# muonium-ai/Qwen3-TTS-C

Hardware: AMD Instinct MI355X
Metric: audio-sec/wall-sec (RTF^-1) + first-packet ms, Qwen3-TTS-1.7B @ 1 & 8 GPU (higher is better)
Workload: dtype fp32 activations x bf16 weights (fp32 accumulate); 1 GPU; Qwen3-TTS-1.7b synthetic, P128 prompt, fixed 128 frames (10.24 s audio), default sampling, batch 1 per GPU; global_batch=1, frames=128, parallelism=dp1 (independent replicas, no collective in the data path)

## Files before the change

### include/qtts_hip.h

```cpp
#ifndef QTTS_HIP_H
#define QTTS_HIP_H

#include <stddef.h>
#include <stdint.h>

#ifdef __cplusplus
extern "C" {
#endif

typedef struct qtts_dev qtts_dev_t;

typedef struct {
    int H, I, L, NH, KV, HD, TH, TV, V, G;
    int Hs, Is, Ls, NHs, KVs, HDs, Vs;
    float eps, theta;
    int cq, ccb, ccbdim, chid, clat, clayers, cheads, ckv, cinter, cwin, cdec;
    int rates[4], ratios[2];
    float ceps;
    int pad_id, bos_id, eos_id;
} qtts_dims_t;

typedef struct {
    int mel_dim, enc_dim, n_ch;
    int ch[8], ks[8], dil[8];
// ... 65 lines not shown
int qtts_dev_codec_stream_begin_ex(qtts_dev_t *dev, int max_frames, int chunk_frames);
int qtts_dev_codec_stream_prime(qtts_dev_t *dev, const int *codes, int T);
int qtts_dev_codec_stream_push_slot(qtts_dev_t *dev, int b, int frame0, int T, float *host_out);
int qtts_dev_codec_stream_push_host(qtts_dev_t *dev, const int *codes, int T, float *host_out);

int qtts_dev_codec_mstream_begin(qtts_dev_t *dev, int n_streams, int max_frames, int chunk_frames);
int qtts_dev_codec_mstream_push_slots(qtts_dev_t *dev, int n, const int *streams, const int *slots, int frame0, int T,
                                      float *const *host_out);
int qtts_dev_codec_mstream_push_host(qtts_dev_t *dev, int n, const int *streams, const int *codes, int T,
                                     float *const *host_out);
int qtts_dev_codec_mstream_pos(qtts_dev_t *dev, int stream);
int qtts_dev_codec_mstream_push_slots_at(qtts_dev_t *dev, int n, const int *streams, const int *slots,
                                         const int *frame0, int T, float *const *host_out);
int qtts_dev_codec_mstream_push_host_any(qtts_dev_t *dev, int n, const int *streams, const int *codes, int T,
                                         float *const *host_out);
int qtts_dev_codec_mstream_reset(qtts_dev_t *dev, int stream);
int qtts_dev_codec_mstream_push_host_ragged(qtts_dev_t *dev, int n, const int *streams, const int *codes,
                                            const int *counts, int ld_frames, float *const *host_out);
int qtts_dev_codec_mstream_push_slots_ragged(qtts_dev_t *dev, int n, const int *streams, const int *slots,
                                             const int *frame0, const int *count, float *const *host_out);
int qtts_dev_codec_mstream_prime(qtts_dev_t *dev, int n, const int *streams, const int *codes, const int *counts,
                                 int ld_frames);

int qtts_dev_codec_async_begin(qtts_dev_t *dev, int max_frames);
int qtts_dev_codec_async_push(qtts_dev_t *dev, int b, int frame0, int T);
int qtts_dev_codec_async_end(qtts_dev_t *dev, float *host_out, int frames);

int qtts_dev_enc_config(qtts_dev_t *dev, const qtts_enc_dims_t *dims);
int qtts_dev_enc_available(qtts_dev_t *dev);
int qtts_dev_speaker_embed(qtts_dev_t *dev, int nb, const float *const *wav, const int *n, float *out,
                           float *mel_out);
int qtts_dev_encode_audio(qtts_dev_t *dev, int nb, const float *const *wav, const int *n, int *codes,
                          int max_frames, int *frames, float *latent);

int qtts_dev_talker_prefill_host(qtts_dev_t *dev, const float *embeds, int n, float *hidden_out);
int qtts_dev_talker_forward_host(qtts_dev_t *dev, const float *embed, float *logits, float *hidden_out);
int qtts_dev_subtalker_host(qtts_dev_t *dev, const float *hidden, int first_code, int *out_codes);
float *qtts_dev_codec_decode_host(qtts_dev_t *dev, const int *codes, int T, int *out_samples);

int qtts_hip_matvec_bf16(float *out_dev, const uint16_t *A_dev, const float *x_dev, int rows, int cols,
                         int batch, void *stream);
int qtts_hip_rmsnorm_matvec_bf16(float *out_dev, const uint16_t *A_dev, const float *x_dev, const float *w_dev,
                                 float eps, int rows, int cols, int batch, void *stream);
int qtts_hip_decode_matvec_bf16(float *out_dev, const uint16_t *A_dev, const float *x_dev, const float *w_dev,
                                float eps, int rows, int cols, int batch, void *stream);
int qtts_hip_resident_matvec_bf16(float *out_dev, const uint16_t *A_dev, const float *x_dev, const float *w_dev,
                                  float eps, int rows, int cols, int epi, void *stream);
int qtts_hip_sample_top_k(int *out_dev, const float *logits_dev, int vocab, int top_k, float top_p,
                          float temperature, uint32_t *rng_bits_dev, int batch, void *stream);
int qtts_hip_sample_top_k_rows(int *out_dev, const float *logits_dev, int vocab, const int *top_k,
                               const float *top_p, const float *temperature, uint32_t *rng_bits_dev, int batch,
                               void *stream);
int qtts_hip_causal_conv1d(float *out_dev, const float *in_dev, const float *w_dev, const float *b_dev, int ci,
                           int co, int k, int L, int dilation, int groups, void *stream);
int qtts_hip_transposed_conv1d(float *out_dev, const float *in_dev, const float *w_dev, const float *b_dev,
                               int ci, int co, int k, int stride, int L, void *stream);
int qtts_hip_snake_beta(float *out_dev, const float *x_dev, const float *alpha_dev, const float *inv_beta_dev,
                        int channels, int length, void *stream);
int qtts_hip_attn_decode(float *out_dev, const float *qkv_dev, void *kc_dev, void *vc_dev,
                         const float *qn_w_dev, const float *kn_w_dev,
                         const float *rope_cos_dev, const float *rope_sin_dev,
                         const int *pos_dev, int NH, int KV, int HD, int S, int rows,
                         float eps, int kv_dtype, void *stream);
int qtts_hip_attn_decode_ex(float *out_dev, const float *qkv_dev, void *kc_dev, void *vc_dev,
                            const float *qn_w_dev, const float *kn_w_dev,
                            const float *rope_cos_dev, const float *rope_sin_dev,
                            const int *pos_dev, int NH, int KV, int HD, int S, int rows,
                            float eps, int kv_dtype, const int *skip_dev, void *stream);
int qtts_hip_attn_cached(float *out_dev, float *q_dev, int ld_q, void *kc_dev, void *vc_dev,
                         const float *qn_w_dev, const float *kn_w_dev,
                         const float *rope_cos_dev, const float *rope_sin_dev,
                         const int *row_b_dev, const int *pos_dev, int NH, int KV, int HD, int S, int slots,
                         int rows, float eps, int win, int kv_dtype, int prep, void *stream);
int qtts_hip_attn_o(float *part_dev, const float *qkv_dev, float *kc_dev, float *vc_dev,
                    const float *qn_w_dev, const float *kn_w_dev,
                    const float *rope_cos_dev, const float *rope_sin_dev, const int *pos_dev,
                    const uint16_t *Wo_dev, int R, int NH, int KV, int HD, int S, int rows, float eps,
                    void *stream);
int qtts_hip_attn_o_pair(float *part_dev, const float *qkv_dev, float *kc_dev, float *vc_dev,
                         const float *qn_w_dev, const float *kn_w_dev,
                         const float *rope_cos_dev, const float *rope_sin_dev, const int *skip_dev,
                         const uint16_t *Wo_dev, int R, int NH, int KV, int HD, int S, float eps,
                         void *stream);
int qtts_hip_resident_matvec_rows_bf16(float *out_dev, const uint16_t *A_dev, const float *x_dev, const float *w_dev,
                                       float eps, int rows, int cols, int epi, const float *part_dev, int n_part,
                                       float *x_new_dev, int nrows, void *stream);
typedef struct {
    int rows, cols, batch;
    const uint16_t *A;
    int src;
    const float *x; int ldx;
    const void *table;
    const int *ids; int ids_bstride, ids_rstride, ids_off;
    const int *row_sel;
    const float *part_in; int n_part_in;
    const float *norm_w; float eps;
    float *xcopy; int xcopy_normed;
    int epi;
    const float *bias;
    float *y; int ldy;
    int kz, self_reduce;
    float *part_out;
} qtts_bgemv_desc_t;
int qtts_hip_batch_matvec_case(const qtts_bgemv_desc_t *d, void *stream);
typedef struct {
    int kernel;
    int n_tmpl, tmpl[5];
    int src;
    int grid_x, grid_y, block;
    size_t lds_bytes;
    int tpw, cch;
} qtts_bgemv_plan_t;
int qtts_hip_batch_matvec_plan(const qtts_bgemv_desc_t *d, qtts_bgemv_plan_t *out);
typedef struct {
    int M, N, K;
    int amode, bmode, emode;
    const float *A; int lda;
    const float *B; int ldb;
    int Kw, dil, pad, L, stride, tmin, co;
    const float *sa, *sb;
    float *C; int ldc;
    const float *bias, *vec, *aux, *res;
    int ldaux, ldres;
    const float *ea, *eb;
} qtts_xgemm_desc_t;
enum {
    QTTS_XP_CONVB2 = 0,
    QTTS_XP_CONVB4 = 1,
    QTTS_XP_CONV = 2,
    QTTS_XP_XLIN = 3,
    QTTS_XP_XGEMV = 4,
    QTTS_XP_XGEMM = 5,
};
int qtts_hip_xgemm_plan(const qtts_xgemm_desc_t *d, size_t part_elems, int force_path, int *path_out,
                        int *splits_out);
int qtts_hip_xgemm_case(const qtts_xgemm_desc_t *d, size_t part_elems, int force_path, int *path_out,
                        int *splits_out, void *stream);
int qtts_hip_xgemm_seg_case(const qtts_xgemm_desc_t *d, int nseg, int seg_ldb, int seg_ldc, size_t part_elems,
                            int force_path, int *path_out, int *splits_out, void *stream);
int qtts_hip_xgemm_func(float *out_dev, const float *x_dev, const float *alpha_dev, const float *inv_beta_dev,
                        int channels, int length, int fn, void *stream);
int qtts_hip_expf_glibc(float *out_dev, const float *in_dev, int n, void *stream);
int qtts_hip_sync(void);
long long qtts_hip_tengine_layers(void);
long long qtts_hip_st_pair_passes(void);
long long qtts_hip_gemv_wide_launches(void);
long long qtts_hip_sample_slot_launches(void);

int qtts_dev_profile_frame(qtts_dev_t *dev, int step, int max, int *kind, double *bytes, float *ms, char *names);
int qtts_hip_hbm_bw(size_t bytes, int iters, double *read_gbs, double *copy_gbs);

#ifdef __cplusplus
}
#endif
#endif
```

### qwen3-tts-c_amd/csrc/hip/k_misc.hip

```cpp
#include "qtts_common.h"
#include "qtts_kernels.h"

namespace {

__global__ __launch_bounds__(256) void k_embed_sum(EmbedSumArgs a) {
#pragma clang fp contract(off)
    const int b = blockIdx.y;
    const int d = blockIdx.x * 256 + threadIdx.x;
    const int stop = a.stopped ? a.stopped[b] : 0;
    const int row = a.cur_row[b];
    const int ntr = a.n_trailing[b];
    if (stop) return;
    const int *cd = a.codes + (size_t)b * a.codes_bstride + (size_t)row * a.G;
    constexpr int GM = 16;
    int c[GM];
#pragma unroll
    for (int g = 0; g < GM; ++g) c[g] = cd[g < a.G ? g : a.G - 1];
    if (d < a.H) {
        const float *tt = row < ntr ? a.trailing + ((size_t)b * a.tr_cap + row) * a.H : a.pad;
        float e[GM];
        e[0] = bf2f(a.codec_emb[(size_t)c[0] * a.H + d]);
#pragma unroll
        for (int g = 1; g < GM; ++g) {
            const int gg = g < a.G ? g : a.G - 1;
            e[g] = bf2f(a.st_emb[((size_t)(gg - 1) * a.Vs + c[g]) * a.H + d]);
        }
        const float t = tt[d];
        float s = 0.0f;
        s += e[0];
#pragma unroll
        for (int g = 1; g < GM; ++g)
            if (g < a.G) s += e[g];
        s += t;
        a.out[(size_t)b * a.H + d] = s;
    }
    if (a.advance && blockIdx.x == 0 && threadIdx.x == 0) a.kv_len[b] += 1;
}

__global__ __launch_bounds__(256) void k_prompt(PromptArgs a) {
#pragma clang fp contract(off)
    const int e = blockIdx.y;
    const int *pl = a.plan + 5 * e;
    const int src = pl[0], cid = pl[1], kind = pl[2], b = pl[3], slot = pl[4];
    float *dst = kind == 0 ? a.prefill + ((size_t)b * a.p_cap + slot) * a.H
                           : a.trailing + ((size_t)b * a.tr_cap + slot) * a.H;
    const int f = -3 - cid;
    const int *fr = cid <= -3 && f < a.n_ref ? a.ref_codes + (size_t)f * a.G : nullptr;
    for (int d = blockIdx.x * 256 + threadIdx.x; d < a.H; d += gridDim.x * 256) {
        float v = a.proj[(size_t)src * a.H + d];
        if (cid >= 0) v += bf2f(a.codec_emb[(size_t)cid * a.H + d]);
        else if (cid == -2 && a.spk) v += a.spk[d];
        else if (fr) {
            float s = 0.0f;
            if (fr[0] >= 0 && fr[0] < a.V) s += bf2f(a.codec_emb[(size_t)fr[0] * a.H + d]);
            for (int g = 1; g < a.G; ++g)
                if (fr[g] >= 0 && fr[g] < a.Vs) s += bf2f(a.st_emb[((size_t)(g - 1) * a.Vs + fr[g]) * a.H + d]);
            v += s;
        }
        dst[d] = v;
    }
}

__global__ void k_copy_rows(float *dst, int ldd, const float *src, int lds, const int *rows, int ncols) {
    const int r = blockIdx.y;
    const int sr = rows ? rows[r] : r;
    for (int c = blockIdx.x * 256 + threadIdx.x; c < ncols; c += gridDim.x * 256)
        dst[(size_t)r * ldd + c] = src[(size_t)sr * lds + c];
}

__global__ __launch_bounds__(256) void k_slot_reset(SlotResetArgs a) {
    const int i = blockIdx.x * 256 + threadIdx.x;
    if (i < a.H) a.x[(size_t)a.b * a.H + i] = a.row[i];
    if (i < a.V) a.counts[(size_t)a.b * a.V + i] = 0;
    if (i == 0) {
        a.kv_len[a.b] = a.pos;
        a.n_gen[a.b] = 0;
        a.cur_row[a.b] = 0;
        a.stop_step[a.b] = 0;
        a.last_tok[a.b] = 0;
        a.rng[a.b] = a.seed_bits;
        a.st_rng[a.b] = a.seed_bits;
        a.stopped[a.b] = 0;
    }
}

}

int qtts_slot_reset(const SlotResetArgs &a, hipStream_t st) {
    const int n = a.H > a.V ? a.H : a.V;
    hipLaunchKernelGGL(k_slot_reset, dim3((n + 255) / 256), dim3(256), 0, st, a);
    return hipGetLastError() == hipSuccess ? 0 : -1;
}

int qtts_embed_sum(const EmbedSumArgs &a, hipStream_t st) {
// ... 23 lines not shown
```

### qwen3-tts-c_amd/csrc/hip/k_tengine.hip

```cpp
#include "qtts_common.h"
#include "qtts_kernels.h"

namespace {

constexpr int H = 2048, NH = 16, KVH = 8, HD = 128, IM = 6144, QKVR = (NH + 2 * KVH) * HD;
constexpr int GPH = NH / KVH;
constexpr int LPK = 8, CH = 256 / LPK, DPL = HD / LPK, D4 = HD / 4, KG = 256 / D4, NO = GPH * HD;
constexpr int NVC = CH / KG;
constexpr unsigned SPIN_MAX = 1u << 22;

struct TLds {
    float xs[H];
    float hs[IM];
    float hq[4 * HD];
    float qk[(GPH + 1) * HD];
    float vv[HD];
    float sc[GPH][CH];
    float ml[GPH][2];
    float red[KG * NO];
    float cred[4];
    float outq[16], outo[8], outh[24];
    int gflag;
    int ocnt;
    int cbar;
    int last;
    int full;
    int done[4];
};

__device__ __forceinline__ float dot8w(const v4u &w, const float *x) {
    const float4 x0 = *reinterpret_cast<const float4 *>(x);
    const float4 x1 = *reinterpret_cast<const float4 *>(x + 4);
    float s = 0.f;
    s = fmaf(__uint_as_float(w.x << 16), x0.x, s); s = fmaf(__uint_as_float(w.x & 0xFFFF0000u), x0.y, s);
    s = fmaf(__uint_as_float(w.y << 16), x0.z, s); s = fmaf(__uint_as_float(w.y & 0xFFFF0000u), x0.w, s);
    s = fmaf(__uint_as_float(w.z << 16), x1.x, s); s = fmaf(__uint_as_float(w.z & 0xFFFF0000u), x1.y, s);
    s = fmaf(__uint_as_float(w.w << 16), x1.z, s); s = fmaf(__uint_as_float(w.w & 0xFFFF0000u), x1.w, s);
    return s;
}

__device__ __forceinline__ int lds_ld(int *p) { return __hip_atomic_load(p, __ATOMIC_RELAXED, __HIP_MEMORY_SCOPE_WORKGROUP); }
__device__ __forceinline__ void give_up(int *err, int code) {
    __hip_atomic_store(err, code, __ATOMIC_RELAXED, __HIP_MEMORY_SCOPE_AGENT);
}

__device__ __forceinline__ bool gemv_wait(TLds &L, int k) {
    unsigned n = 0;
    bool ok = true;
    while (lds_ld(&L.gflag) < k) {
        __builtin_amdgcn_s_sleep(1);
        if (++n > SPIN_MAX) { ok = false; break; }
    }
    __builtin_amdgcn_fence(__ATOMIC_ACQUIRE, "workgroup");
    return ok;
}
__device__ __forceinline__ void gemv_done(TLds &L, int lane) {
    __builtin_amdgcn_fence(__ATOMIC_RELEASE, "workgroup");
    if (lane == 0) __hip_atomic_fetch_add(&L.ocnt, 1, __ATOMIC_RELAXED, __HIP_MEMORY_SCOPE_WORKGROUP);
}
__device__ __forceinline__ void cbarrier(TLds &L, int &gen, int lane, int *err) {
    gen += 4;
    __builtin_amdgcn_fence(__ATOMIC_RELEASE, "workgroup");
    if (lane == 0) __hip_atomic_fetch_add(&L.cbar, 1, __ATOMIC_RELAXED, __HIP_MEMORY_SCOPE_WORKGROUP);
    unsigned n = 0;
    while (lds_ld(&L.cbar) < gen) {
        __builtin_amdgcn_s_sleep(1);
        if (++n > SPIN_MAX) { give_up(err, 2); break; }
    }
    __builtin_amdgcn_fence(__ATOMIC_ACQUIRE, "workgroup");
}
__device__ __forceinline__ void comm_wait_out(TLds &L, int k, int *err) {
    unsigned n = 0;
    while (lds_ld(&L.ocnt) < 4 * k) {
        __builtin_amdgcn_s_sleep(1);
        if (++n > SPIN_MAX) { give_up(err, 20 + k); break; }
    }
    __builtin_amdgcn_fence(__ATOMIC_ACQUIRE, "workgroup");
}
__device__ __forceinline__ void comm_stage(TLds &L, int k, int &gen, int lane, int *err) {
    cbarrier(L, gen, lane, err);
    if (threadIdx.x == 256) __hip_atomic_store(&L.gflag, k, __ATOMIC_RELAXED, __HIP_MEMORY_SCOPE_WORKGROUP);
}

typedef unsigned long long u64;
__device__ __forceinline__ void te_stamp(const TLayerArgs &a, int k, bool who) {
#ifdef QTTS_STAMPS
    if (a.dbg && who) a.dbg[blockIdx.x * 16 + k] = __builtin_amdgcn_s_memrealtime();
#endif
}
__device__ __forceinline__ void put_granule(u64 *g, unsigned tag, float v) {
    __hip_atomic_store(g, ((u64)tag << 32) | __float_as_uint(v), __ATOMIC_RELAXED, __HIP_MEMORY_SCOPE_AGENT);
}
template <int N, typename Idx>
__device__ __forceinline__ void sweep(const u64 *g, unsigned tag, Idx idx, float (&v)[N], int *err, int code) {
    unsigned n = 0;
    for (;;) {
        bool ok = true;
#pragma unroll
        for (int j = 0; j < N; ++j) {
            const u64 x = __hip_atomic_load(const_cast<u64 *>(g) + idx(j), __ATOMIC_RELAXED, __HIP_MEMORY_SCOPE_AGENT);
            v[j] = __uint_as_float((unsigned)x);
            ok &= (unsigned)(x >> 32) == tag;
        }
        if (__all(ok)) return;
        __builtin_amdgcn_s_sleep(1);
        if (++n > SPIN_MAX) { give_up(err, code); return; }
    }
}

__device__ __forceinline__ void comm_norm_stage(TLds &L, float4 (&xv)[2], const float *nw, float eps, int ct, int lane,
                                                int cw, int &gen, int *err) {
    float ss = 0.f;
#pragma unroll
    for (int q = 0; q < 2; ++q) {
        const float4 v = xv[q];
        ss += v.x * v.x + v.y * v.y + v.z * v.z + v.w * v.w;
    }
    ss = wave_sum(ss);
    if (lane == 0) L.cred[cw] = ss;
    cbarrier(L, gen, lane, err);
    const float inv = rms_inv(L.cred[0] + L.cred[1] + L.cred[2] + L.cred[3], H, eps);
#pragma unroll
    for (int q = 0; q < 2; ++q) {
        const int c = 4 * (ct + 256 * q);
        const float4 n4 = *reinterpret_cast<const float4 *>(nw + c);
        float4 v = xv[q];
        v.x = v.x * inv * n4.x; v.y = v.y * inv * n4.y; v.z = v.z * inv * n4.z; v.w = v.w * inv * n4.w;
        *reinterpret_cast<float4 *>(L.xs + c) = v;
    }
}

__device__ __forceinline__ int qkv_row(int h, int i) {
    return i < NO ? GPH * HD * h + i : i < NO + HD ? NH * HD + HD * h + (i - NO) : (NH + KVH) * HD + HD * h + (i - NO - HD);
}

struct AttnPre {
    float4 kreg[DPL / 4];
    float4 vreg[NVC];
    float hw[2], rc[2], rs[2];
};
__device__ __forceinline__ void attn_preload(AttnPre &q, const TLayerArgs &a, int kvh, int split, int p, int ct,
                                             int lane, int cw) {
    const int t0 = split * CH, t1 = min(p + 1, t0 + CH);
    const int KVD = KVH * HD;
    const float *Kc = a.kc + kvh * HD;
    const float *Vc = a.vc + kvh * HD;
    const int hh0 = cw < GPH ? cw : GPH;
    const float *nw = hh0 < GPH ? a.qn_w : a.kn_w;
    const float *cs = a.rope_cos + (size_t)p * HD, *sn = a.rope_sin + (size_t)p * HD;
#pragma unroll
    for (int j = 0; j < 2; ++j) {
        q.hw[j] = nw[lane + 64 * j];
        q.rc[j] = cs[lane + 64 * j];
        q.rs[j] = sn[lane + 64 * j];
    }
    const int kl = ct / LPK, ksub = ct - kl * LPK;
    const int tk = t0 + kl;
    const float4 *kp = reinterpret_cast<const float4 *>(Kc + (size_t)(tk < t1 ? tk : t0) * KVD + ksub * DPL);
#pragma unroll
    for (int j = 0; j < DPL / 4; ++j) q.kreg[j] = kp[j];
    const int d4 = ct % D4, kg = ct / D4;
#pragma unroll
    for (int j = 0; j < NVC; ++j) {
        const int t = t0 + kg + j * KG;
        const bool ok = kg + j * KG < CH && t < t1;
        q.vreg[j] = reinterpret_cast<const float4 *>(Vc + (size_t)(ok ? t : t0) * KVD)[d4];
    }
}

__device__ void comm_attention(TLds &L, const TLayerArgs &a, int kvh, int split, int nact, int p, unsigned tag,
                               int ct, int lane, int cw, int &gen, const AttnPre &pre) {
    const int n = p + 1;
    const int t0 = split * CH, t1 = min(n, t0 + CH);
    const bool owner = (split == nact - 1);
    const int KVD = KVH * HD;
    const int hh0 = cw < GPH ? cw : GPH;
    float hv[2];
    {
        const float *src = L.hq + (hh0 < GPH ? hh0 * HD : NO);
#pragma unroll
        for (int j = 0; j < 2; ++j) hv[j] = src[lane + 64 * j];
    }
    const float *hw = pre.hw, *rc = pre.rc, *rs = pre.rs;
    const float4 *kreg = pre.kreg, *vreg = pre.vreg;
    const float vtok = L.hq[NO + HD + ct % HD];
    const int kl = ct / LPK, ksub = ct - kl * LPK;
    const int tk = t0 + kl;
    const int d4 = ct % D4, kg = ct / D4;
    if (cw <= GPH) {
        float ss = 0.f;
#pragma unroll
        for (int j = 0; j < 2; ++j) ss += hv[j] * hv[j];
// ... 564 lines not shown
```

### qwen3-tts-c_amd/csrc/hip/qtts_kernels.h

```cpp
#pragma once
#include <hip/hip_runtime.h>
#include <stdint.h>

typedef uint16_t bf16_t;

constexpr int QTTS_GM_TICKS = 1024;

enum { EPI_STORE = 0, EPI_BIAS = 1, EPI_BIAS_SILU = 2, EPI_RESID = 3, EPI_SWIGLU = 4 };

constexpr int QTTS_PF_LOADS = 4;
struct L2Prefetch {
    const unsigned char *base = nullptr;
    int pm = 1 << 30;
    long long pa = 0, pb = 0;
    int chunks = 0, lg = 30, ld = 0;
    int cs = 6;
    int nwg = 0;
    unsigned *sink = nullptr;
};

struct GemvArgs {
    const bf16_t *W = nullptr;
    int R = 0, C = 0;
    int ksplit = 0;
// ... 58 lines not shown
int qtts_bgemv(const GemvArgs &a, hipStream_t st, unsigned allowed = BG_ALL);
int qtts_gemvm_launch(const GemvArgs &a, const BgPlan &p, hipStream_t st);
int qtts_gemvb_launch(const GemvArgs &a, const BgPlan &p, hipStream_t st);
int qtts_gemvx_launch(const GemvArgs &a, const BgPlan &p, hipStream_t st);
bool qtts_gemvx_shape_ok(int R, int C);
int qtts_mgemm(const GemvArgs &a, float *inv_scratch, hipStream_t st, float *part = nullptr, size_t part_elems = 0);
size_t qtts_mgemm_part_elems(size_t rows, size_t widest);
int qtts_row_rms(const float *x, int ldx, int rows, int C, float eps, float *inv, hipStream_t st);
int qtts_mgemm_reduce(const GemvArgs &a, const float *part, int kz, hipStream_t st);
int qtts_pgemm(const GemvArgs &a, float *inv_scratch, unsigned short *planes, size_t plane_elems, hipStream_t st,
               float *part, size_t part_elems);
size_t qtts_pgemm_plane_elems(size_t rows, size_t K);

struct TLayerArgs {
    const float *x_in = nullptr;
    float *x_out = nullptr;
    const bf16_t *wqkv = nullptr, *wo = nullptr, *wgu = nullptr, *wdown = nullptr;
    const float *in_norm = nullptr, *post_norm = nullptr, *qn_w = nullptr, *kn_w = nullptr;
    const float *rope_cos = nullptr, *rope_sin = nullptr;
    float *kc = nullptr, *vc = nullptr;
    const int *pos = nullptr;
    const int *skip = nullptr;
    float eps = 1e-6f;
    float *part = nullptr;
    int *cnt = nullptr;
    int nsplit = 0;
    unsigned long long *g_qkv = nullptr, *g_att = nullptr, *g_x = nullptr, *g_h = nullptr;
    int *epoch = nullptr;
    int *err = nullptr;
    int layer = 0, last_layer = 0;
    unsigned long long *dbg = nullptr;
};
constexpr int QTTS_TE_GRANULES = 4096 + 2048 + 2048 + 6144;
bool qtts_tlayer_dims_ok(int H, int NH, int KV, int HD, int I);
size_t qtts_tlayer_lds();
int qtts_tlayer(const TLayerArgs &a, hipStream_t st, int mode);

struct AttnArgs {
    int mode = 0;
    const float *qkv = nullptr;
    int ld_qkv = 0;
    const float *qn_w = nullptr, *kn_w = nullptr;
    float eps = 1e-6f;
    const float *rope_cos = nullptr, *rope_sin = nullptr;
    float *kc = nullptr, *vc = nullptr;
    int S = 0;
    const int *pos = nullptr;
    int pos_const = 0;
    const int *row_b = nullptr;
    int NH = 0, KV = 0, HD = 0;
    float *out = nullptr;
    int ld_out = 0;
    int nrows = 0;
    const int *skip = nullptr;
    int win = 0;
    const float *qkv_tab = nullptr;
    const int *tab_ids = nullptr, *tab_row_sel = nullptr;
    int tab_bstride = 0, tab_rstride = 0, tab_off = 0;
    float *part = nullptr;
    int *cnt = nullptr;
    int nsplit = 0;
    int defer = 0;
    L2Prefetch pf;
#ifdef QTTS_STAMPS
    unsigned long long *dbg = nullptr;
#endif
    const float *xc_tab = nullptr;
    const bf16_t *xc_tab16 = nullptr;
    float *xc_dst = nullptr;
    int xc_n = 0;
    int lpk = 0;
    int kv_dtype = 0;
};
int qtts_attn_keys_per_split(int HD, bool defer, int lpk);
bool qtts_attn_defer_ok(const AttnArgs &a);
int qtts_attn_o(const AttnArgs &a, const bf16_t *Wo, int R, float *part, hipStream_t st);
bool qtts_attn_o_covers(const AttnArgs &a, const bf16_t *Wo);

bool qtts_gemvw_pair_covers(int R, int C, int epi);
int qtts_gemvw_pair(const GemvArgs &a, hipStream_t st);
bool qtts_attn_o_pair_covers(const AttnArgs &a, const bf16_t *Wo);
int qtts_attn_o_pair(const AttnArgs &a, const bf16_t *Wo, int R, float *part, hipStream_t st);

extern thread_local const char *qtts_last_kernel;
inline bool qtts_attn_head_ok(int HD) { return HD == 8 || HD == 16 || HD == 32 || HD == 64 || HD == 128; }
int qtts_attention(const AttnArgs &a, hipStream_t st);
int qtts_qk_prep(const AttnArgs &a, hipStream_t st);

struct SampArgs {
    const float *logits = nullptr;
    int ld = 0, n = 0, nb = 1;
    int top_k = 50;
    float top_p = 1.0f, temp = 0.9f;
    uint32_t *rng = nullptr;
    int mode = 0;
    int suppress_lo = 0, eos = -1;
    float rep = 1.0f;
    int *counts = nullptr;
    int fixed = 0;
    int *n_gen = nullptr, *stopped = nullptr, *cur_row = nullptr, *stop_step = nullptr;
    int *host_stopped = nullptr;
    uint32_t *st_rng = nullptr;
    uint32_t seed_bits = 0;
    int *codes = nullptr;
    int codes_bstride = 0, G = 16, g = 0;
    int *out_tok = nullptr;
};
int qtts_sample(const SampArgs &a, hipStream_t st);

constexpr int QTTS_MAX_TAPS = 8;
struct SampForce {
    const int *forced = nullptr;
    int *drawn = nullptr;
    const int *taps = nullptr;
    float *tap_logits = nullptr;
    int *tap_meta = nullptr;
    int tap_ld = 0;
};
int qtts_sample_forced(const SampArgs &a, const SampForce &f, hipStream_t st);

struct alignas(16) SampSlotRow {
    float temp, top_p, rep;
    int top_k;
    float st_temp, st_top_p;
    int st_top_k;
    uint32_t seed_bits;
};
static_assert(sizeof(SampSlotRow) == 32, "two dwordx4 loads cover a row");
bool qtts_sample_row_fast(const SampSlotRow &r, int mode, int n);
int qtts_sample_slots(const SampArgs &a, const SampSlotRow *tab, bool all_fast, hipStream_t st);
long long qtts_sample_slot_launches();
int qtts_slot_row_set(SampSlotRow *tab, int b, const SampSlotRow &r, uint32_t *rng, uint32_t *st_rng, hipStream_t st);

struct EmbedSumArgs {
    const int *codes = nullptr;
    int codes_bstride = 0, G = 16;
    const int *cur_row = nullptr, *stopped = nullptr;
    const bf16_t *codec_emb = nullptr;
    const bf16_t *st_emb = nullptr;
    int Vs = 0, H = 0, nb = 1;
    const float *trailing = nullptr;
    int tr_cap = 0;
    const int *n_trailing = nullptr;
    const float *pad = nullptr;
    float *out = nullptr;
    int *kv_len = nullptr;
    int advance = 0;
};
int qtts_embed_sum(const EmbedSumArgs &a, hipStream_t st);

struct PromptArgs {
    const float *proj = nullptr;
    const int *plan = nullptr;
    int nplan = 0, H = 0;
    const bf16_t *codec_emb = nullptr;
    const bf16_t *st_emb = nullptr;
    const float *spk = nullptr;
    const int *ref_codes = nullptr;
    int n_ref = 0, G = 0, V = 0, Vs = 0;
    float *prefill = nullptr;
    int p_cap = 0;
    float *trailing = nullptr;
    int tr_cap = 0;
};
int qtts_prompt_assemble(const PromptArgs &a, hipStream_t st);

int qtts_copy_rows(float *dst, int ldd, const float *src, int lds, const int *src_rows, int nrows, int ncols,
                   hipStream_t st);

struct SlotResetArgs {
    int b = 0, pos = 0, H = 0, V = 0;
    const float *row = nullptr;
    float *x = nullptr;
    int *kv_len = nullptr, *n_gen = nullptr, *cur_row = nullptr, *stopped = nullptr, *stop_step = nullptr;
    int *last_tok = nullptr, *counts = nullptr;
    uint32_t *rng = nullptr, *st_rng = nullptr;
    uint32_t seed_bits = 0;
};
int qtts_slot_reset(const SlotResetArgs &a, hipStream_t st);
```

### qwen3-tts-c_amd/csrc/hip/qtts_runtime.hip

```cpp
#include <math.h>
#include <stdlib.h>
#include <string.h>

#include <algorithm>
#include <map>
#include <set>
#include <string>
#include <atomic>
#include <vector>

#include "qtts_common.h"
#include "qtts_kernels.h"
#include "qtts_codec.h"
#include "qtts_enc.h"
#include "../../../include/qtts_hip.h"

#define CK(x)                                                                                              \
    do {                                                                                                   \
        hipError_t e_ = (x);                                                                               \
        if (e_ != hipSuccess) {                                                                            \
            fprintf(stderr, "HIP error %s at %s:%d: %s\n", hipGetErrorName(e_), __FILE__, __LINE__, #x);   \
            return -1;                                                                                     \
        }                                                                                                  \
    } while (0)
// ... 40 lines not shown
    size_t war_off = 0, war_cap = 0, sar_off = 0, sar_cap = 0;
    std::vector<Layer> tl, sl;
    bf16_t *codec_emb = nullptr, *text_emb = nullptr, *fc1w = nullptr, *fc2w = nullptr, *head = nullptr;
    float *fc1b = nullptr, *fc2b = nullptr, *tk_norm = nullptr;
    bf16_t *st_emb = nullptr, *lm = nullptr, *st_proj = nullptr;
    float *st_projb = nullptr, *st_norm = nullptr;
    float *codec_ptab = nullptr, *st_ptab = nullptr;
    float *qkv0_tab = nullptr;
    CodecModel codec;
    EncModel enc;
    float *rope_cos = nullptr, *rope_sin = nullptr, *rope_cos_s = nullptr, *rope_sin_s = nullptr;
    int rope_max = 0;
    std::set<std::string> got;
    int nb = 0, nrun = 0, max_frames = 0, S = 0, p_cap = 0, tr_cap = 0, rows_cap = 0;
    float *x_tk = nullptr, *qkv = nullptr, *att = nullptr, *hbuf = nullptr, *logits = nullptr, *tk_hid = nullptr;
    float *x_st2 = nullptr, *opart = nullptr;
    float *x_tk2 = nullptr, *bpo = nullptr, *bpd = nullptr;
    float *ppart = nullptr;
    float *tk_xfin = nullptr;
    const float *tk_pend = nullptr;
    int tk_npend = 0;
    bool bsplit = true;
    int bself_min = 9;
    int bkz_max = 0;
    int bkz_wide = 1;
    float *x_st = nullptr, *qkv_s = nullptr, *att_s = nullptr, *h_s = nullptr, *logits_s = nullptr;
    float *kc = nullptr, *vc = nullptr, *kcs = nullptr, *vcs = nullptr;
    int kv_dtype = 0, kv_want = 0;
    bool te_kv_said = false;
    bool att_own = false;
    int *codes = nullptr, *counts = nullptr, *n_gen = nullptr, *stopped = nullptr, *cur_row = nullptr;
    int *last_tok = nullptr;
    int *stop_step = nullptr, *kv_len = nullptr, *n_trailing = nullptr;
    float *att_part = nullptr;
    int *att_cnt = nullptr, att_nsplit = 0;
    int *btick = nullptr;
    uint32_t *rng = nullptr, *st_rng = nullptr;
    float *trailing = nullptr, *prefill = nullptr, *pad_emb = nullptr;
    float *px = nullptr, *pqkv = nullptr, *patt = nullptr, *ph = nullptr, *pt1 = nullptr, *pproj = nullptr;
    int *prow_b = nullptr, *ppos = nullptr, *psrc = nullptr, *pids = nullptr, *pplan = nullptr, *plast = nullptr;
    int ids_cap = 0;
    int *pref = nullptr;
    float *pspk = nullptr;
    int pref_cap = 0, n_pref = 0, has_spk = 0;
    std::vector<int> p_len_h, n_tr_h;
    qtts_gen_params_t par{};
    bool have_par = false;
    hipGraphExec_t g0 = nullptr, gN = nullptr;
    hipGraphExec_t gNr[QTTS_MAX_SLOTS + 1] = {};
    int graph_key = -1;
    int *f_forced = nullptr, *f_drawn = nullptr, *f_taps = nullptr, *f_tap_meta = nullptr;
    float *f_tap_logits = nullptr;
    int f_tap_ld = 0, f_ntaps = 0, f_phase = 0;
    int f_run_frames = 0;
    bool f_armed = false;
    size_t f_bytes = 0;
    SampSlotRow *sp_tab = nullptr;
    std::vector<SampSlotRow> sp_host;
    bool sp_armed = false, sp_general = false;
    int *hstop = nullptr;
    int hstop_cap = 0;
    hipEvent_t fev[2] = {nullptr, nullptr};
    hipStream_t cst = nullptr;
    hipEvent_t cev = nullptr;
    float *cwav = nullptr;
    size_t cwav_cap = 0;
    int *push_codes = nullptr;
    size_t push_cap = 0;
    bool prime_pending = false;
    float *pwav = nullptr;
    size_t pwav_cap = 0;
    std::vector<CodecModel *> clanes;
    std::vector<hipStream_t> clane_st;
    float *mwav = nullptr;
    size_t mwav_cap = 0;
    int *mcodes = nullptr;
    size_t mcodes_cap = 0;
    struct Prof { int kind; double bytes; hipEvent_t a, b; const char *name; };
    std::vector<Prof> prof;
    bool profiling = false;
    bool attn_o = true;
    bool tab0b = true;
    bool st_pair = true;
    int l2pf = 31;
    int l2pf_tk = 0;
    unsigned *pf_sink = nullptr;
    bool attn_defer = true;
    int attn_lpk = 0;
    int gm_dbg_layer = -1;
    unsigned long long *gm_dbg = nullptr;
    int tengine = 0;
    unsigned long long *te_g = nullptr;
    int *te_ctl = nullptr;
    float *pinv = nullptr;
    int pinv_cap = 0;
    float *mpart = nullptr;
    size_t mpart_elems = 0;
    unsigned short *pplanes = nullptr;
    size_t pplanes_elems = 0;
    bool pgemm = true;

    int QKV() const { return (d.NH + 2 * d.KV) * d.HD; }
    int QKVs() const { return (d.NHs + 2 * d.KVs) * d.HDs; }
    size_t kv_esz() const { return kv_dtype == 1 ? 2 : 4; }
    float *kv_layer(float *c, int l) const {
        return reinterpret_cast<float *>(reinterpret_cast<char *>(c) + (size_t)l * nb * S * d.KV * d.HD * kv_esz());
    }
};

static constexpr size_t QTTS_ARENA_SMALL = (size_t)1 << 20, QTTS_ARENA_BLOCK = (size_t)32 << 20;
static void *dalloc(qtts_dev *dv, size_t n, bool weight) {
    void *p = nullptr;
    if (n == 0) n = 16;
    const char *ae = getenv("QTTS_HIP_ARENA");
    const int arena = ae ? atoi(ae) : 0;
    if (arena && n <= QTTS_ARENA_SMALL) {
        unsigned char *&base = weight ? dv->war : dv->sar;
        size_t &off = weight ? dv->war_off : dv->sar_off, &cap = weight ? dv->war_cap : dv->sar_cap;
        const size_t need = (n + 255) & ~(size_t)255;
        if (!base || off + need > cap) {
            void *blk = dalloc(dv, QTTS_ARENA_BLOCK, weight);
            if (!blk) return nullptr;
            base = (unsigned char *)blk; off = 0; cap = QTTS_ARENA_BLOCK;
        }
        p = base + off;
        off += need;
        return p;
    }
    const hipError_t prior = hipPeekAtLastError();
    const hipError_t e = hipMalloc(&p, n);
    if (e != hipSuccess) {
        fprintf(stderr, "qtts: hipMalloc(%zu) failed: %s (last error before it: %s)\n", n, hipGetErrorName(e),
                hipGetErrorName(prior));
        return nullptr;
    }
    if (weight) { dv->wallocs.push_back(p); dv->wbytes += n; }
    else { dv->sallocs.push_back(p); dv->sbytes += n; }
    return p;
}

static void drop_row_graphs(qtts_dev *dv) {
    for (auto &g : dv->gNr)
        if (g) { hipGraphExecDestroy(g); g = nullptr; }
}

static void free_force(qtts_dev *dv) {
    if (!dv->f_armed) return;
    hipStreamSynchronize(dv->st);
    for (void *p : {(void *)dv->f_forced, (void *)dv->f_drawn, (void *)dv->f_taps, (void *)dv->f_tap_meta,
                    (void *)dv->f_tap_logits})
        if (p) hipFree(p);
    dv->f_forced = dv->f_drawn = dv->f_taps = dv->f_tap_meta = nullptr;
    dv->f_tap_logits = nullptr;
    dv->f_tap_ld = dv->f_ntaps = 0;
    dv->sbytes -= dv->f_bytes;
    dv->f_bytes = 0;
    dv->f_armed = false;
    dv->graph_key = -1;
}

static void free_slot_params(qtts_dev *dv) {
    if (!dv->sp_armed) return;
    hipStreamSynchronize(dv->st);
    if (dv->sp_tab) {
        hipFree(dv->sp_tab);
        dv->sbytes -= dv->sp_host.size() * sizeof(SampSlotRow);
// ... 137 lines not shown
    } else if (name == "talker.text_projection.linear_fc2.bias") {
        dv->fc2b = upload_f32(dv, host, dtype, n); rc = dv->fc2b ? 0 : -1;
    } else if (name == "talker.model.norm.weight") {
        dv->tk_norm = upload_f32(dv, host, dtype, n); rc = dv->tk_norm ? 0 : -1;
    } else if (name == "talker.codec_head.weight") {
        dv->head = upload_bf16(dv, host, dtype, n); rc = dv->head ? 0 : -1;
    } else if (name == "talker.code_predictor.small_to_mtp_projection.weight") {
        dv->st_proj = upload_bf16(dv, host, dtype, n); rc = dv->st_proj ? 0 : -1;
    } else if (name == "talker.code_predictor.small_to_mtp_projection.bias") {
        dv->st_projb = upload_f32(dv, host, dtype, n); rc = dv->st_projb ? 0 : -1;
    } else if (name == "talker.code_predictor.model.norm.weight") {
        dv->st_norm = upload_f32(dv, host, dtype, n); rc = dv->st_norm ? 0 : -1;
    } else if ((idx = parse_idx(name, "talker.code_predictor.model.codec_embedding.", &rest)) >= 0 && rest == "weight") {
        if (idx >= d.G - 1 || n != (size_t)d.Vs * d.H) { fprintf(stderr, "qtts: bad %s\n", cname); return -1; }
        if (!dv->st_emb) dv->st_emb = (bf16_t *)dalloc(dv, (size_t)(d.G - 1) * d.Vs * d.H * 2, true);
        rc = dv->st_emb ? upload_bf16_at(dv->st_emb + (size_t)idx * d.Vs * d.H, host, dtype, n) : -1;
    } else if ((idx = parse_idx(name, "talker.code_predictor.lm_head.", &rest)) >= 0 && rest == "weight") {
        if (idx >= d.G - 1 || n != (size_t)d.Vs * d.Hs) { fprintf(stderr, "qtts: bad %s\n", cname); return -1; }
        if (!dv->lm) dv->lm = (bf16_t *)dalloc(dv, (size_t)(d.G - 1) * d.Vs * d.Hs * 2, true);
        rc = dv->lm ? upload_bf16_at(dv->lm + (size_t)idx * d.Vs * d.Hs, host, dtype, n) : -1;
    } else if ((idx = parse_idx(name, "talker.code_predictor.model.layers.", &rest)) >= 0) {
        if (idx >= d.Ls) return 0;
        rc = put_layer(dv, dv->sl[idx], rest, host, dtype, n, d.Hs, d.NHs, d.KVs, d.HDs, d.Is);
    } else if ((idx = parse_idx(name, "talker.model.layers.", &rest)) >= 0) {
        if (idx >= d.L) return 0;
        rc = put_layer(dv, dv->tl[idx], rest, host, dtype, n, d.H, d.NH, d.KV, d.HD, d.I);
    } else {
        return 0;
    }
    if (rc) {
        fprintf(stderr, "qtts: failed to upload tensor %s\n", cname);
        return -1;
    }
    dv->got.insert(name);
    return 0;
}

extern "C" qtts_dev_t *qtts_dev_create(const qtts_dims_t *dims, int device) {
    if (hipSetDevice(device) != hipSuccess) {
        fprintf(stderr, "qtts: cannot select HIP device %d\n", device);
        return nullptr;
    }
    qtts_dev *dv = new qtts_dev();
    dv->d = *dims;
    dv->device = device;
    if (hipStreamCreateWithFlags(&dv->st, hipStreamNonBlocking) != hipSuccess) {
        delete dv;
        return nullptr;
    }
    dv->tl.resize(dims->L);
    dv->sl.resize(dims->Ls);
    const char *bs = getenv("QTTS_HIP_BSPLIT");
    dv->bsplit = !(bs && !atoi(bs));
    const char *bk = getenv("QTTS_HIP_BKZ_MAX");
    if (bk) dv->bkz_max = atoi(bk) < 1 ? 1 : atoi(bk) > 4 ? 4 : atoi(bk);
    const char *bw = getenv("QTTS_HIP_BKZ_WIDE");
    dv->bkz_wide = bw ? atoi(bw) : 1;
    const char *bm = getenv("QTTS_HIP_BSELF_MIN");
    if (bm) dv->bself_min = atoi(bm);
    const char *ad = getenv("QTTS_HIP_ATTN_DEFER");
    dv->attn_defer = !(ad && !atoi(ad));
    const char *lk = getenv("QTTS_HIP_ATTN_LPK");
    dv->attn_lpk = lk ? atoi(lk) : 0;
    const char *ao = getenv("QTTS_HIP_ATTN_O");
    dv->attn_o = !(ao && !atoi(ao));
    const char *pg = getenv("QTTS_HIP_PGEMM");
    dv->pgemm = !(pg && !atoi(pg));
    const char *te = getenv("QTTS_HIP_TENGINE");
    if (te && atoi(te)) {
        int dev = 0, ncu = 0;
        if (hipGetDevice(&dev) == hipSuccess &&
            hipDeviceGetAttribute(&ncu, hipDeviceAttributeMultiprocessorCount, dev) == hipSuccess && ncu >= 256)
            dv->tengine = std::min(3, std::max(1, atoi(te)));
    }
    const char *kvd = getenv("QTTS_HIP_KV");
    if (kvd && *kvd) {
        if (!strcmp(kvd, "bf16")) dv->kv_want = 1;
        else if (strcmp(kvd, "fp32")) fprintf(stderr, "qtts: QTTS_HIP_KV=%s ignored (bf16 or fp32)\n", kvd);
    }
    const char *tb = getenv("QTTS_HIP_TAB0B");
    dv->tab0b = !(tb && !atoi(tb));
    const char *sp = getenv("QTTS_HIP_ST_PAIR");
    dv->st_pair = !(sp && !atoi(sp));
    const char *pf = getenv("QTTS_HIP_L2PF");
    if (pf) dv->l2pf = atoi(pf);
    const char *pft = getenv("QTTS_HIP_L2PF_TK");
    if (pft) dv->l2pf_tk = atoi(pft);
    const char *gd = getenv("QTTS_HIP_GM_DBG");
    if (gd) dv->gm_dbg_layer = atoi(gd);
    codec_init(&dv->codec, dims, dv->st);
    dv->enc.st = dv->st;
    dv->enc.device = device;
    return dv;
}

extern "C" void qtts_dev_destroy(qtts_dev_t *dv) {
    if (!dv) return;
    hipSetDevice(dv->device);
    hipStreamSynchronize(dv->st);
    free_state(dv);
    codec_destroy(&dv->codec);
    enc_destroy(&dv->enc);
    if (dv->cst) hipStreamSynchronize(dv->cst);
    if (dv->hstop) hipHostFree(dv->hstop);
    for (hipEvent_t e : dv->fev)
        if (e) hipEventDestroy(e);
    for (CodecModel *ln : dv->clanes) codec_lane_delete(ln);
    for (hipStream_t st : dv->clane_st) hipStreamDestroy(st);
    if (dv->mwav) hipFree(dv->mwav);
    if (dv->mcodes) hipFree(dv->mcodes);
    if (dv->cwav) hipFree(dv->cwav);
    if (dv->pwav) hipFree(dv->pwav);
    if (dv->push_codes) hipFree(dv->push_codes);
    if (dv->cev) hipEventDestroy(dv->cev);
    if (dv->cst) hipStreamDestroy(dv->cst);
    for (void *p : dv->wallocs) hipFree(p);
    hipStreamDestroy(dv->st);
    delete dv;
}

extern "C" size_t qtts_dev_bytes(const qtts_dev_t *dv, int which) {
    if (!dv) return 0;
    return which == 0 ? dv->wbytes + codec_weight_bytes(&dv->codec) + enc_weight_bytes(&dv->enc) : dv->sbytes;
}

extern "C" int qtts_dev_set_kv_dtype(qtts_dev_t *dv, int dtype) {
    if (!dv || (dtype != 0 && dtype != 1)) return -1;
    dv->kv_want = dtype;
    return 0;
}

extern "C" int qtts_dev_kv_dtype(const qtts_dev_t *dv) { return dv ? dv->kv_want : -1; }

extern "C" int qtts_dev_get_kv(qtts_dev_t *dv, int layer, int b, int pos0, int n, float *k_host, float *v_host) {
    if (!dv || !dv->kc || !dv->vc || dv->nb < 1 || layer < 0 || layer >= dv->d.L || b < 0 || b >= dv->nb ||
        pos0 < 0 || n < 1 || pos0 > dv->S - n)
        return -1;
    hipSetDevice(dv->device);
    const size_t KVD = (size_t)dv->d.KV * dv->d.HD, cnt = (size_t)n * KVD, esz = dv->kv_esz();
    const size_t off = ((size_t)b * dv->S + pos0) * KVD * esz;
    CK(hipStreamSynchronize(dv->st));
    float *caches[2] = {dv->kc, dv->vc}, *outs[2] = {k_host, v_host};
    std::vector<uint16_t> tmp(dv->kv_dtype == 1 ? cnt : 0);
    for (int i = 0; i < 2; ++i) {
        if (!outs[i]) continue;
        const char *src = reinterpret_cast<const char *>(dv->kv_layer(caches[i], layer)) + off;
        if (dv->kv_dtype == 1) {
            CK(hipMemcpy(tmp.data(), src, cnt * 2, hipMemcpyDeviceToHost));
            for (size_t j = 0; j < cnt; ++j) outs[i][j] = host_bf16(tmp[j]);
        } else {
            CK(hipMemcpy(outs[i], src, cnt * 4, hipMemcpyDeviceToHost));
        }
    }
    return 0;
}

extern "C" int qtts_dev_get_attn(qtts_dev_t *dv, float *qkv_host, float *att_host) {
    if (!dv || dv->nb < 1 || !dv->qkv || !dv->att) return -1;
    if (att_host && !dv->att_own) {
        fprintf(stderr, "qtts_dev_get_attn: the last talker pass left no merged attention output "
                        "(batch 1 defers the merge to the O projection; QTTS_HIP_ATTN_DEFER=0 keeps it)\n");
        return -1;
    }
    hipSetDevice(dv->device);
    CK(hipStreamSynchronize(dv->st));
    if (qkv_host) CK(hipMemcpy(qkv_host, dv->qkv, (size_t)dv->nb * dv->QKV() * 4, hipMemcpyDeviceToHost));
// ... 120 lines not shown
        if (!dv->ptr) return -1;                                          \
    } while (0)
    A(x_tk, float, B * d.H);
    A(qkv, float, B * dv->QKV());
    A(att, float, B * d.NH * d.HD);
    A(hbuf, float, B * d.I);
    A(logits, float, B * d.V);
    A(tk_hid, float, B * d.H);
    const size_t B2 = B < 2 ? 2 : B;
    A(x_st, float, B2 * d.Hs);
    A(x_st2, float, B2 * d.Hs);
    A(x_tk2, float, B * d.H);
    A(bpo, float, (size_t)4 * B * (d.H > d.Hs ? d.H : d.Hs));
    A(bpd, float, (size_t)4 * B * (d.H > d.Hs ? d.H : d.Hs));
    A(ppart, float, (size_t)4 * 16 * (d.H > d.Hs ? d.H : d.Hs));
    A(opart, float, (size_t)B2 * ((size_t)d.KVs * d.Hs > (size_t)d.KV * d.H ? (size_t)d.KVs * d.Hs : (size_t)d.KV * d.H));
    A(qkv_s, float, B2 * dv->QKVs());
    A(att_s, float, B * d.NHs * d.HDs);
    A(h_s, float, B2 * d.Is);
    A(logits_s, float, B * d.Vs);
    {
        const size_t kv_floats = (size_t)d.L * B * dv->S * d.KV * d.HD * dv->kv_esz() / 4;
        A(kc, float, kv_floats);
        A(vc, float, kv_floats);
    }
    A(kcs, float, (size_t)d.Ls * B * d.G * d.KVs * d.HDs);
    A(vcs, float, (size_t)d.Ls * B * d.G * d.KVs * d.HDs);
    A(codes, int, B * (max_frames + 1) * d.G);
    A(counts, int, B * d.V);
    A(n_gen, int, B);
    A(stopped, int, B);
    A(cur_row, int, B);
    A(last_tok, int, B);
    CK(hipMemsetAsync(dv->last_tok, 0, B * sizeof(int), dv->st));
    A(stop_step, int, B);
    A(kv_len, int, B);
    A(n_trailing, int, B);
    A(rng, uint32_t, B);
    A(st_rng, uint32_t, B);
    A(trailing, float, B * 64 * d.H);
    dv->tr_cap = 64;
    A(prefill, float, B * max_prefill * d.H);
    A(pad_emb, float, d.H);
    const size_t R = dv->rows_cap;
    A(px, float, R * d.H);
    A(pqkv, float, R * dv->QKV());
    A(patt, float, R * d.NH * d.HD);
    A(ph, float, R * d.I);
    A(prow_b, int, R);
    A(ppos, int, R);
    A(psrc, int, R);
    A(plast, int, B);
    dv->pinv_cap = dv->rows_cap > 64 ? dv->rows_cap : 64;
    A(pinv, float, dv->pinv_cap);
    {
        const size_t wide = std::max<size_t>({(size_t)dv->QKV(), (size_t)2 * d.I, (size_t)d.H, (size_t)d.TH});
        const char *e = getenv("QTTS_HIP_MGEMM_KZ");
        dv->mpart_elems = e && !strcmp(e, "0") ? 0 : qtts_mgemm_part_elems(std::max<size_t>(R, 64), wide);
        if (dv->mpart_elems)
            dv->mpart_elems = std::max(dv->mpart_elems, std::min<size_t>((size_t)512 * 128 * 128, (size_t)8 * R * wide));
        if (dv->mpart_elems) A(mpart, float, dv->mpart_elems);
        const size_t kmax = std::max<size_t>({(size_t)d.H, (size_t)d.I, (size_t)d.NH * d.HD});
        dv->pplanes_elems = dv->pgemm ? qtts_pgemm_plane_elems(R, kmax) : 0;
        if (dv->pplanes_elems) A(pplanes, unsigned short, dv->pplanes_elems);
    }
    {
        const int gph = d.NH / d.KV;
        const int ch = std::min(qtts_attn_keys_per_split(d.HD, false, dv->attn_lpk),
                                qtts_attn_keys_per_split(d.HD, true, dv->attn_lpk));
        dv->att_nsplit = (dv->S + ch - 1) / ch;
        A(att_part, float, B * d.KV * dv->att_nsplit * (gph * d.HD + 2 * gph));
        const int kvmax = d.KV > d.KVs ? d.KV : d.KVs;
        A(att_cnt, int, B * kvmax);
        CK(hipMemsetAsync(dv->att_cnt, 0, B * kvmax * sizeof(int), dv->st));
        A(pf_sink, unsigned, 1);
        A(btick, int, QTTS_GM_TICKS);
        if (dv->tengine) {
            A(te_g, unsigned long long, QTTS_TE_GRANULES);
            CK(hipMemsetAsync(dv->te_g, 0, QTTS_TE_GRANULES * 8, dv->st));
            A(te_ctl, int, 2);
            CK(hipMemsetAsync(dv->te_ctl, 0, 2 * sizeof(int), dv->st));
        }
        CK(hipMemsetAsync(dv->btick, 0, QTTS_GM_TICKS * sizeof(int), dv->st));
        if (dv->gm_dbg_layer >= 0) {
            A(gm_dbg, unsigned long long, 4 * 2048 * 8);
            CK(hipMemsetAsync(dv->gm_dbg, 0, 4 * 2048 * 8 * 8, dv->st));
        }
    }
#undef A
    dv->p_len_h.assign(nb, 0);
    dv->n_tr_h.assign(nb, 0);
    CK(hipMemsetAsync(dv->codes, 0, B * (max_frames + 1) * d.G * sizeof(int), dv->st));
    CK(hipMemsetAsync(dv->kcs, 0, (size_t)d.Ls * B * d.G * d.KVs * d.HDs * 4, dv->st));
    CK(hipMemsetAsync(dv->vcs, 0, (size_t)d.Ls * B * d.G * d.KVs * d.HDs * 4, dv->st));
    if (dv->rope_max < dv->S) {
        dv->rope_max = dv->S;
        CKI(build_rope(dv, dv->S, d.HD, d.theta, &dv->rope_cos, &dv->rope_sin));
        if (d.HDs != d.HD) CKI(build_rope(dv, d.G + 2, d.HDs, d.theta, &dv->rope_cos_s, &dv->rope_sin_s));
        else { dv->rope_cos_s = dv->rope_cos; dv->rope_sin_s = dv->rope_sin; }
    }
    dv->graph_key = -1;
    return 0;
}

static uint32_t seed_bits(int seed) {
    float f = (float)seed;
    uint32_t u;
    memcpy(&u, &f, 4);
    return u;
}

static int reset_counters(qtts_dev *dv) {
    const size_t B = dv->nb;
    hipStream_t st = dv->st;
    if (dv->hstop_cap < (int)B) {
        if (dv->hstop) CK(hipHostFree(dv->hstop));
        dv->hstop = nullptr;
        CK(hipHostMalloc((void **)&dv->hstop, B * sizeof(int), hipHostMallocDefault));
        dv->hstop_cap = (int)B;
        dv->graph_key = -1;
    }
    if (!dv->fev[0]) {
        CK(hipEventCreateWithFlags(&dv->fev[0], hipEventDisableTiming));
        CK(hipEventCreateWithFlags(&dv->fev[1], hipEventDisableTiming));
    }
    CK(hipStreamSynchronize(st));
    memset(dv->hstop, 0, B * sizeof(int));
    CK(hipMemsetAsync(dv->counts, 0, B * dv->d.V * sizeof(int), st));
    CK(hipMemsetAsync(dv->n_gen, 0, B * sizeof(int), st));
    CK(hipMemsetAsync(dv->stopped, 0, B * sizeof(int), st));
    CK(hipMemsetAsync(dv->cur_row, 0, B * sizeof(int), st));
    CK(hipMemsetAsync(dv->stop_step, 0, B * sizeof(int), st));
    std::vector<uint32_t> r(B, seed_bits(dv->par.seed));
    CK(hipMemcpyAsync(dv->rng, r.data(), B * 4, hipMemcpyHostToDevice, st));
    CK(hipMemcpyAsync(dv->st_rng, r.data(), B * 4, hipMemcpyHostToDevice, st));
    CK(hipStreamSynchronize(st));
    return 0;
}

enum { PK_GEMV_TALKER = 0, PK_GEMV_SUB = 1, PK_ATTN = 2, PK_SAMPLE = 3, PK_EMBED = 4 };
struct ProfScope {
    qtts_dev *dv;
    size_t idx;
    ProfScope(qtts_dev *d, int kind, double bytes) : dv(d), idx((size_t)-1) {
        if (!dv->profiling) return;
        qtts_dev::Prof p{kind, bytes, nullptr, nullptr, ""};
        hipEventCreateWithFlags(&p.a, hipEventDisableSystemFence);
        hipEventCreateWithFlags(&p.b, hipEventDisableSystemFence);
        hipEventRecord(p.a, dv->st);
        dv->prof.push_back(p);
        idx = dv->prof.size() - 1;
    }
    void cancel() {
        if (idx == (size_t)-1) return;
        hipEventDestroy(dv->prof[idx].a);
        hipEventDestroy(dv->prof[idx].b);
        dv->prof.pop_back();
        idx = (size_t)-1;
    }
    ~ProfScope() {
        if (idx == (size_t)-1) return;
        hipEventRecord(dv->prof[idx].b, dv->st);
        dv->prof[idx].name = qtts_last_kernel;
    }
};
static double gemv_bytes(const GemvArgs &a) {
    return (double)a.R * a.C * 2 + (double)a.nb * a.C * 4 + (double)a.nb * a.R * 4 + (a.norm_w ? a.C * 4.0 : 0.0);
}
static int pgemv(qtts_dev *dv, const GemvArgs &a, int kind) {
    ProfScope ps(dv, kind, gemv_bytes(a));
    return qtts_gemv(a, dv->st);
}
static int rows_proj(qtts_dev *dv, GemvArgs a, int rows, bool prefill = false) {
    const int xs = a.ldx, ys = a.ldy;
    if (prefill && dv->pgemm && rows > 16 && (!a.norm_w || rows <= dv->pinv_cap)) {
        GemvArgs c = a;
        c.nb = rows;
        const int rc = qtts_pgemm(c, dv->pinv, dv->pplanes, dv->pplanes_elems, dv->st, dv->mpart, dv->mpart_elems);
        if (rc <= 0) return rc;
    }
    if (rows > 64 && (!a.norm_w || rows <= dv->pinv_cap)) {
        GemvArgs c = a;
        c.nb = rows;
        const int rc = qtts_mgemm(c, dv->pinv, dv->st, dv->mpart, dv->mpart_elems);
        if (rc <= 0) return rc;
    }
    for (int r0 = 0; r0 < rows;) {
        GemvArgs c = a;
        int nr = rows - r0 < 64 ? rows - r0 : 64;
        if (c.x) c.x = a.x + (size_t)r0 * xs;
        if (c.ids) c.ids = a.ids + (size_t)r0 * a.ids_bstride;
        c.y = a.y + (size_t)r0 * ys;
        c.nb = nr;
        int rc = 1;
        static const bool pgb = [] { const char *e = getenv("QTTS_HIP_PREFILL_GEMVB"); return !(e && !atoi(e)); }();
        static const int psk = [] { const char *e = getenv("QTTS_HIP_PREFILL_SPLIT");
                                    int v = e ? atoi(e) : 2; return v == 4 ? 4 : v ? 2 : 0; }();
        if (nr >= 2 && nr <= 16 && pgb && psk && c.epi == EPI_RESID && !c.norm_w && c.R / 16 < 256 &&
            c.C % (32 * psk) == 0 && c.R <= (dv->d.H > dv->d.Hs ? dv->d.H : dv->d.Hs)) {
            GemvArgs k = c;
            k.ypart = dv->ppart; k.kz = psk; k.ld_ypart = (size_t)nr * k.R; k.tick = dv->btick;
            rc = qtts_bgemv(k, dv->st, BG_GEMVB);
        }
        if (rc == 1) rc = qtts_bgemv(c, dv->st, pgb ? BG_GEMVB | BG_GEMVM : BG_GEMVM);
        if (rc == 1 && nr >= 2) rc = qtts_mgemm(c, dv->pinv, dv->st, dv->mpart, dv->mpart_elems);
        if (rc < 0) return -1;
        if (rc == 1) {
            nr = nr < 16 ? nr : 16;
            c.nb = nr;
            CKI(qtts_gemv(c, dv->st));
        }
        r0 += nr;
    }
    return 0;
}
// ... 45 lines not shown
    std::vector<int> io(nid);
    for (int i = 0; i < nid; ++i) io[i] = i;
    int *ids = (int *)dalloc(dv, (size_t)nid * 4, true);
    dv->qkv0_tab = (float *)dalloc(dv, rows * QKV * 4, true);
    if (!ids || !dv->qkv0_tab) return -1;
    CK(hipMemcpy(ids, io.data(), (size_t)nid * 4, hipMemcpyHostToDevice));
    const bool proj = dv->st_proj != nullptr;
    for (int g = 1; g < d.G; ++g) {
        GemvArgs a = gv(dv->sl[0].wqkv, QKV, d.Hs, nullptr, d.Hs, nullptr, QKV, 1, EPI_STORE);
        a.norm_w = dv->sl[0].in; a.eps = d.eps; a.nt = 0;
        if (proj) a.table_f32 = g == 1 ? dv->codec_ptab : dv->st_ptab + (size_t)(g - 2) * d.Vs * d.Hs;
        else a.table = g == 1 ? dv->codec_emb : dv->st_emb + (size_t)(g - 2) * d.Vs * d.H;
        a.ids = ids; a.ids_bstride = 1;
        a.reps = g == 1 ? d.V : d.Vs;
        a.ldy_rep = QKV;
        a.y = dv->qkv0_tab + (g == 1 ? 0 : (size_t)d.V + (size_t)(g - 2) * d.Vs) * QKV;
        const int rc = qtts_gemvw(a, dv->st);
        if (rc < 0) return -1;
        if (rc == 0) continue;
        const int n = a.reps;
        float *base = a.y;
        a.reps = 1;
        for (int r = 0; r < n; ++r) {
            a.ids_off = r;
            a.y = base + (size_t)r * QKV;
            CKI(qtts_gemv(a, dv->st));
        }
    }
    CK(hipStreamSynchronize(dv->st));
    return 0;
}


static int bsplit_kz(const qtts_dev *dv, int R, int C) {
    if (!dv->bsplit || dv->nrun < 2) return 0;
    int kz = R / 16 >= 256 ? 1 : 256 / (R / 16);
    const int cap = dv->bkz_max > 0 ? dv->bkz_max : dv->nrun <= 8 ? 2 : 4;
    if (kz > cap) kz = cap;
    if ((dv->nrun > 8 && dv->bkz_wide) || dv->bkz_wide == 2) {
        const int wcap = dv->bkz_wide == 2 ? 4 : cap;
        while (2 * kz <= wcap && C / kz > 2048 && C % (64 * kz) == 0) kz *= 2;
    }
    while (kz > 1 && C % (32 * kz)) kz /= 2;
    return kz > 1 ? kz : 0;
}
static bool split_out(qtts_dev *dv, GemvArgs &g, float *part, int kz, int self_min = 0) {
    g.ypart = part; g.kz = kz; g.ld_ypart = (size_t)dv->nrun * g.R;
    if (dv->nrun >= (self_min > 0 ? self_min : dv->bself_min)) { g.tick = dv->btick; return false; }
    g.y = nullptr;
    return true;
}
static void add_in(GemvArgs &g, const float *part, int n, int R, int nrun, float *xnew) {
    g.xadd = part; g.n_xadd = n; g.ld_xadd = nrun * R; g.ldb_xadd = R;
    if (xnew) { g.xcopy = xnew; g.ldxc = R; g.xcopy_normed = 0; }
}

static L2Prefetch pf_gemvw(const qtts_dev *dv, const bf16_t *W, int R, int C, int grid = 256, bool on = true) {
    L2Prefetch p;
    if (!on || R % grid) return p;
    long long bytes = (long long)(R / grid) * C * 2;
    if (bytes > 64LL * 256 * QTTS_PF_LOADS) bytes = 64LL * 256 * QTTS_PF_LOADS;
    if (bytes % 64) return p;
    p.base = reinterpret_cast<const unsigned char *>(W);
    p.pa = (long long)(R / grid) * C * 2; p.pb = 0; p.chunks = (int)(bytes / 64); p.lg = 30; p.ld = 0;
    p.nwg = grid;
    p.sink = dv->pf_sink;
    return p;
}
#ifdef QTTS_STAMPS
#define DBG_XFIRST(a) do { const char *e_ = getenv("QTTS_HIP_DBG_XFIRST"); (a).dbg_xfirst = e_ ? atoi(e_) : 0; } while (0)
#else
#define DBG_XFIRST(a) do { } while (0)
#endif
static L2Prefetch pf_attn_o(const qtts_dev *dv, const bf16_t *Wo, int R, int NH, int HD) {
    L2Prefetch p;
    const int W2 = 2 * HD, LPS = W2 / 8 < 8 ? W2 / 8 : 8, RPW = 256 / LPS;
    const int cpr = W2 * 2 / 64;
    if (R % RPW || (cpr & (cpr - 1)) || cpr < 1 || RPW * cpr > 256 * QTTS_PF_LOADS) return p;
    p.base = reinterpret_cast<const unsigned char *>(Wo);
    p.pm = R / RPW; p.pa = (long long)RPW * NH * HD * 2; p.pb = W2 * 2;
    p.chunks = RPW * cpr; p.lg = __builtin_ctz(cpr); p.ld = NH * HD * 2; p.sink = dv->pf_sink;
    p.nwg = (R / RPW) * (NH / 2);
    return p;
}

static bool tengine_ok(qtts_dev *dv, int kzo, int kzd) {
    const qtts_dims_t &d = dv->d;
    return dv->tengine && dv->te_g && dv->kv_dtype == 0 && dv->nrun == 1 && !kzo && !kzd && dv->attn_defer &&
           qtts_tlayer_dims_ok(d.H, d.NH, d.KV, d.HD, d.I) && dv->S > 16 && dv->att_nsplit * 32 >= dv->S;
}
static std::atomic<long long> g_tengine_layers{0};
extern "C" long long qtts_hip_tengine_layers(void) { return g_tengine_layers.load(); }
static int talker_layers_te(qtts_dev *dv) {
    const qtts_dims_t &d = dv->d;
    const int NBA = dv->nb, KVD = d.KV * d.HD;
    for (int l = 0; l < d.L; ++l) {
        Layer &ly = dv->tl[l];
        TLayerArgs a;
        a.x_in = dv->x_tk; a.x_out = dv->x_tk;
        a.wqkv = ly.wqkv; a.wo = ly.wo; a.wgu = ly.wgu; a.wdown = ly.wdown;
        a.in_norm = ly.in; a.post_norm = ly.post; a.qn_w = ly.qn; a.kn_w = ly.kn;
        a.rope_cos = dv->rope_cos; a.rope_sin = dv->rope_sin;
        a.kc = dv->kv_layer(dv->kc, l); a.vc = dv->kv_layer(dv->vc, l);
        a.pos = dv->kv_len; a.skip = dv->stopped; a.eps = d.eps;
        a.part = dv->att_part; a.cnt = dv->att_cnt; a.nsplit = dv->att_nsplit;
        a.g_qkv = dv->te_g; a.g_att = dv->te_g + 4096; a.g_x = a.g_att + 2048; a.g_h = a.g_x + 2048;
        a.epoch = dv->te_ctl; a.err = dv->te_ctl + 1;
        a.layer = l; a.last_layer = l == d.L - 1;
        if (dv->gm_dbg && (l == dv->gm_dbg_layer || l == dv->gm_dbg_layer + 1))
            a.dbg = dv->gm_dbg + (size_t)(l - dv->gm_dbg_layer) * 256 * 16;
        ProfScope ps(dv, PK_GEMV_TALKER, 2.0 * ((double)dv->QKV() * d.H + (double)d.H * d.NH * d.HD + 3.0 * d.I * d.H));
        CKI(qtts_tlayer(a, dv->st, dv->tengine));
        g_tengine_layers.fetch_add(1);
    }
    dv->tk_xfin = dv->x_tk; dv->tk_pend = nullptr; dv->tk_npend = 0;
    dv->att_own = false;
    return 0;
}

static int talker_layers(qtts_dev *dv) {
    const qtts_dims_t &d = dv->d;
    const int nb = dv->nrun, NBA = dv->nb, QKV = dv->QKV(), AD = d.NH * d.HD, KVD = d.KV * d.HD;
    hipStream_t st = dv->st;
    const int kzo = bsplit_kz(dv, d.H, AD), kzd = bsplit_kz(dv, d.H, d.I);
    if (tengine_ok(dv, kzo, kzd)) return talker_layers_te(dv);
    float *xa = dv->x_tk, *xb = dv->x_tk2;
    const float *pend = nullptr;
    int npend = 0;
    for (int l = 0; l < d.L; ++l) {
        Layer &ly = dv->tl[l];
        GemvArgs a = gv(ly.wqkv, QKV, d.H, xa, d.H, dv->qkv, QKV, nb, EPI_STORE);
        a.norm_w = ly.in; a.eps = d.eps;
        if (pend) add_in(a, pend, npend, d.H, nb, xb);
        AttnArgs t;
        t.mode = 0; t.qkv = dv->qkv; t.ld_qkv = QKV; t.qn_w = ly.qn; t.kn_w = ly.kn; t.eps = d.eps;
        t.rope_cos = dv->rope_cos; t.rope_sin = dv->rope_sin;
        t.kc = dv->kv_layer(dv->kc, l); t.vc = dv->kv_layer(dv->vc, l); t.S = dv->S; t.kv_dtype = dv->kv_dtype;
        t.pos = dv->kv_len; t.NH = d.NH; t.KV = d.KV; t.HD = d.HD; t.out = dv->att; t.ld_out = AD; t.nrows = nb;
        t.skip = dv->stopped;
        t.part = dv->att_part; t.cnt = dv->att_cnt; t.nsplit = dv->att_nsplit; t.lpk = dv->attn_lpk;
        const bool defer = dv->attn_defer && nb == 1 && qtts_attn_defer_ok(t) && qtts_gemvw_amerge_ok(d.H, AD);
        t.defer = defer;
        dv->att_own = !defer;
        const bool dbg = dv->gm_dbg && l == dv->gm_dbg_layer;
        if (dbg) a.dbg = dv->gm_dbg;
        if (nb == 1 && (dv->l2pf_tk & 1)) a.pf = pf_gemvw(dv, ly.wo, d.H, AD);
        CKI(qkv_attn(dv, a, t, PK_GEMV_TALKER));
        if (pend) { std::swap(xa, xb); pend = nullptr; }
        GemvArgs o = gv(ly.wo, d.H, AD, dv->att, AD, xa, d.H, nb, EPI_RESID);
        if (dbg) o.dbg = dv->gm_dbg + 2048 * 8;
        if (defer) {
            o.amerge = dv->att_part; o.am_pos = dv->kv_len; o.am_nsplit = dv->att_nsplit;
            o.am_ch = qtts_attn_keys_per_split(d.HD, true, dv->attn_lpk); o.am_hd = d.HD; o.am_gph = d.NH / d.KV;
        }
        const int tk_self = 2;
        const bool opend = kzo && split_out(dv, o, dv->bpo, kzo, tk_self);
        if (nb == 1 && (dv->l2pf_tk & 2)) o.pf = pf_gemvw(dv, ly.wgu, 2 * d.I, d.H, 512);
        CKI(pgemv(dv, o, PK_GEMV_TALKER));
        a = gv(ly.wgu, 2 * d.I, d.H, xa, d.H, dv->hbuf, d.I, nb, EPI_SWIGLU);
        a.norm_w = ly.post; a.eps = d.eps;
        if (dbg) a.dbg = dv->gm_dbg + 2 * 2048 * 8;
        if (opend) add_in(a, dv->bpo, kzo, d.H, nb, xb);
        CKI(pgemv(dv, a, PK_GEMV_TALKER));
        if (opend) std::swap(xa, xb);
        GemvArgs dn = gv(ly.wdown, d.H, d.I, dv->hbuf, d.I, xa, d.H, nb, EPI_RESID);
        if (dbg) dn.dbg = dv->gm_dbg + 3 * 2048 * 8;
// ... 65 lines not shown
}
static bool st_pair_ok(const qtts_dev *dv) {
    const qtts_dims_t &d = dv->d;
    if (!dv->st_pair || dv->nrun != 1 || !dv->attn_o || !dv->qkv0_tab || d.G < 2 || d.Ls < 1) return false;
    if (dv->st_proj && !(dv->st_ptab && dv->codec_ptab)) return false;
    if (!dv->st_proj && d.H != d.Hs) return false;
    if (!qtts_gemvw_pair_covers(dv->QKVs(), d.Hs, EPI_STORE) || !qtts_gemvw_pair_covers(2 * d.Is, d.Hs, EPI_SWIGLU) ||
        !qtts_gemvw_pair_covers(d.Hs, d.Is, EPI_RESID))
        return false;
    for (int l = 0; l < d.Ls; ++l)
        if (!qtts_attn_o_pair_covers(st_pair_attn_args(dv, l), dv->sl[l].wo)) return false;
    return true;
}
static int pgemv_pair(qtts_dev *dv, const GemvArgs &a) {
    ProfScope ps(dv, PK_GEMV_SUB, gemv_bytes(a));
    if (qtts_gemvw_pair(a, dv->st) != 0) {
        fprintf(stderr, "qtts: pair GEMV launch failed (R=%d C=%d)\n", a.R, a.C);
        return -1;
    }
    return 0;
}
static int subtalker_pair_layers(qtts_dev *dv, int pfm, float **xfin) {
    const qtts_dims_t &d = dv->d;
    const int QKV = dv->QKVs(), AD = d.NHs * d.HDs;
    const bool proj = dv->st_proj != nullptr;
    float *xa = dv->x_st, *xb = dv->x_st2;
    if (proj) {
        GemvArgs a = gv(dv->st_proj, d.Hs, d.H, dv->tk_hid, d.H, dv->x_st, d.Hs, 1, dv->st_projb ? EPI_BIAS : EPI_STORE);
        a.bias = dv->st_projb;
        a.nt = 0;
        CKI(pgemv(dv, a, PK_GEMV_SUB));
    }
    {
        Layer &ly = dv->sl[0];
        GemvArgs a = gv(ly.wqkv, QKV, d.Hs, xa, d.Hs, dv->qkv_s, QKV, 1, EPI_STORE);
        a.norm_w = ly.in; a.eps = d.eps; a.nt = 0;
        if (!proj) { a.x = dv->tk_hid; a.ldx = d.H; a.xcopy = dv->x_st; a.ldxc = d.Hs; a.xcopy_normed = 0; }
        if (pfm & 1) a.pf = pf_attn_o(dv, ly.wo, d.Hs, d.NHs, d.HDs);
        CKI(pgemv(dv, a, PK_GEMV_SUB));
    }
    for (int l = 0; l < d.Ls; ++l) {
        Layer &ly = dv->sl[l];
        const bool sdbg = dv->gm_dbg && dv->gm_dbg_layer == 98 && l == 2;
        if (l > 0) {
            GemvArgs a = gv(ly.wqkv, QKV, d.Hs, xa, d.Hs, dv->qkv_s, QKV, 2, EPI_STORE);
            a.norm_w = ly.in; a.eps = d.eps; a.nt = 0;
            if (sdbg) a.dbg = dv->gm_dbg;
            if (pfm & 1) a.pf = pf_attn_o(dv, ly.wo, d.Hs, d.NHs, d.HDs);
            CKI(pgemv_pair(dv, a));
        }
        AttnArgs t = st_pair_attn_args(dv, l);
        if (pfm & 2) t.pf = pf_gemvw(dv, ly.wgu, 2 * d.Is, d.Hs);
#ifdef QTTS_STAMPS
        if (sdbg) t.dbg = dv->gm_dbg + 2048 * 8;
#endif
        {
            ProfScope ps(dv, PK_ATTN, (double)d.Hs * AD * 2);
            if (qtts_attn_o_pair(t, ly.wo, d.Hs, dv->opart, dv->st) != 0) {
                fprintf(stderr, "qtts: pair attention + O launch failed (layer %d)\n", l);
                return -1;
            }
        }
        GemvArgs a = gv(ly.wgu, 2 * d.Is, d.Hs, xa, d.Hs, dv->h_s, d.Is, 2, EPI_SWIGLU);
        a.norm_w = ly.post; a.eps = d.eps; a.nt = 0;
        if (pfm & 4) a.pf = pf_gemvw(dv, ly.wdown, d.Hs, d.Is);
        add_in(a, dv->opart, d.KVs, d.Hs, 2, xb);
        if (sdbg) a.dbg = dv->gm_dbg + 2 * 2048 * 8;
        CKI(pgemv_pair(dv, a));
        std::swap(xa, xb);
        a = gv(ly.wdown, d.Hs, d.Is, dv->h_s, d.Is, xa, d.Hs, 2, EPI_RESID);
        a.nt = 0;
        if (pfm & 8) {
            if (l + 1 < d.Ls) a.pf = pf_gemvw(dv, dv->sl[l + 1].wqkv, QKV, d.Hs);
            else a.pf = pf_gemvw(dv, dv->lm, d.Vs, d.Hs);
        }
        if (sdbg) a.dbg = dv->gm_dbg + 3 * 2048 * 8;
        CKI(pgemv_pair(dv, a));
    }
    *xfin = xa;
    g_st_pair_passes.fetch_add(1);
    return 0;
}

static int subtalker(qtts_dev *dv) {
    const qtts_dims_t &d = dv->d;
    const int nb = dv->nrun, NBA = dv->nb, QKV = dv->QKVs(), AD = d.NHs * d.HDs, KVD = d.KVs * d.HDs;
    const int cstride = (dv->max_frames + 1) * d.G;
    hipStream_t st = dv->st;
    const bool proj = dv->st_proj != nullptr;
    const bool pfon = nb == 1 && dv->attn_o && dv->l2pf;
    const int pfm = pfon ? dv->l2pf : 0;
    const bool tab0_ok = nb == 1 && dv->attn_o && dv->qkv0_tab && (!proj || dv->st_ptab);
    auto first_op_pf = [&](int gn) {
        if (gn >= d.G) return L2Prefetch();
        if (gn >= 1 && tab0_ok) return pf_attn_o(dv, dv->sl[0].wo, d.Hs, d.NHs, d.HDs);
        return pf_gemvw(dv, dv->sl[0].wqkv, QKV, d.Hs);
    };
    auto pass_head = [&](int g, const float *x, const float *pend, int npend) -> int {
        GemvArgs a = gv(dv->lm + (size_t)(g - 1) * d.Vs * d.Hs, d.Vs, d.Hs, x, d.Hs, dv->logits_s, d.Vs, nb,
                        EPI_STORE);
        a.norm_w = dv->st_norm; a.eps = d.eps; a.nt = 0;
        if (pend) add_in(a, pend, npend, d.Hs, nb, nullptr);
        if (pfm & 16) a.pf = first_op_pf(g + 1);
        SampArgs s;
        s.logits = dv->logits_s; s.ld = d.Vs; s.n = d.Vs; s.nb = nb;
        s.top_k = dv->par.st_top_k; s.top_p = dv->par.st_top_p; s.temp = dv->par.st_temperature;
        s.mode = 0; s.st_rng = dv->st_rng; s.stopped = dv->stopped; s.cur_row = dv->cur_row;
        s.codes = dv->codes; s.codes_bstride = cstride; s.G = d.G; s.g = g; s.out_tok = dv->last_tok;
        return head_sample(dv, a, s, PK_GEMV_SUB);
    };
    int g0 = 0;
    if (st_pair_ok(dv)) {
        float *xfin = nullptr;
        CKI(subtalker_pair_layers(dv, pfm, &xfin));
        CKI(pass_head(1, xfin + d.Hs, nullptr, 0));
        g0 = 2;
    }
    for (int g = g0; g < d.G; ++g) {
        GemvArgs src;
        src.nb = nb;
        const bool ptab = proj && g >= 1 && dv->st_ptab;
        if (g == 0) { src.x = dv->tk_hid; src.ldx = d.H; }
        else {
            if (ptab) src.table_f32 = g == 1 ? dv->codec_ptab : dv->st_ptab + (size_t)(g - 2) * d.Vs * d.Hs;
            else src.table = g == 1 ? dv->codec_emb : dv->st_emb + (size_t)(g - 2) * d.Vs * d.H;
            src.ids = dv->last_tok; src.ids_bstride = 1; src.row_sel = nullptr; src.ids_rstride = 0;
            src.ids_off = 0;
        }
        auto set_src = [&](GemvArgs &a) {
            a.x = src.x; a.ldx = src.ldx; a.table = src.table; a.table_f32 = src.table_f32; a.ids = src.ids;
            a.ids_bstride = src.ids_bstride; a.row_sel = src.row_sel; a.ids_rstride = src.ids_rstride;
            a.ids_off = src.ids_off;
        };
        if (proj && !ptab) {
            GemvArgs a = gv(dv->st_proj, d.Hs, d.H, nullptr, 0, dv->x_st, d.Hs, nb, dv->st_projb ? EPI_BIAS : EPI_STORE);
            set_src(a);
            a.bias = dv->st_projb;
            a.nt = 0;
            CKI(pgemv(dv, a, PK_GEMV_SUB));
        }
        float *xa = dv->x_st, *xb = dv->x_st2;
        const int kzo = bsplit_kz(dv, d.Hs, AD), kzd = bsplit_kz(dv, d.Hs, d.Is);
        const float *pend = nullptr;
        int npend = 0;
        for (int l = 0; l < d.Ls; ++l) {
            Layer &ly = dv->sl[l];
            const bool kv_only = g == 0 && l == d.Ls - 1;
            GemvArgs a = gv(ly.wqkv, QKV, d.Hs, xa, d.Hs, dv->qkv_s, QKV, nb, EPI_STORE);
            a.norm_w = ly.in; a.eps = d.eps; a.nt = 0;
            const bool sdbg = dv->gm_dbg && dv->gm_dbg_layer == 99 && g == 5 && l == 2;
            if (sdbg) { a.dbg = dv->gm_dbg; DBG_XFIRST(a); }
            if (l == 0 && (!proj || ptab)) { set_src(a); a.xcopy = dv->x_st; a.ldxc = d.Hs; a.xcopy_normed = 0; }
            else if (pend) add_in(a, pend, npend, d.Hs, nb, xb);
            AttnArgs t;
            t.mode = 0; t.qkv = dv->qkv_s; t.ld_qkv = QKV; t.qn_w = ly.qn; t.kn_w = ly.kn; t.eps = d.eps;
            t.rope_cos = dv->rope_cos_s; t.rope_sin = dv->rope_sin_s;
            t.kc = dv->kcs + (size_t)l * NBA * d.G * KVD; t.vc = dv->vcs + (size_t)l * NBA * d.G * KVD; t.S = d.G;
            t.pos = nullptr; t.pos_const = g; t.NH = d.NHs; t.KV = d.KVs; t.HD = d.HDs; t.out = dv->att_s;
            t.ld_out = AD; t.nrows = nb; t.skip = dv->stopped;
            t.cnt = dv->att_cnt;
            const bool tab0 = l == 0 && g >= 1 && nb == 1 && dv->attn_o && dv->qkv0_tab && (!proj || ptab) &&
                              qtts_attn_o_covers(t, ly.wo);
            GemvArgs o = gv(ly.wo, d.Hs, AD, dv->att_s, AD, xa, d.Hs, nb, EPI_RESID);
            o.nt = 0;
            bool fused_o = false, opend = false;
            const bool hd_ok = d.HDs == 128 || d.HDs == 64 || d.HDs == 32 || d.HDs == 16;
            const bool tab0b = l == 0 && g >= 1 && nb >= 2 && dv->tab0b && dv->qkv0_tab && (!proj || ptab) &&
                               d.NHs == 2 * d.KVs && d.G <= 16 && hd_ok;
            if (tab0 || tab0b) {
                t.qkv_tab = dv->qkv0_tab + (g == 1 ? 0 : (size_t)d.V + (size_t)(g - 2) * d.Vs) * QKV;
                t.tab_ids = src.ids; t.tab_bstride = src.ids_bstride; t.tab_row_sel = src.row_sel;
                t.tab_rstride = src.ids_rstride; t.tab_off = src.ids_off;
            }
            if (tab0b) { t.xc_tab = src.table_f32; t.xc_tab16 = src.table; t.xc_dst = xa; t.xc_n = d.Hs; }
            if (pfm & 1) a.pf = pf_attn_o(dv, ly.wo, d.Hs, d.NHs, d.HDs);
            if (pfm & 2) t.pf = kv_only ? first_op_pf(g + 1) : pf_gemvw(dv, ly.wgu, 2 * d.Is, d.Hs);
#ifdef QTTS_STAMPS
            if (sdbg) t.dbg = dv->gm_dbg + 2048 * 8;
#endif
            if (dv->attn_o && nb == 1) {
                if (!tab0) CKI(pgemv(dv, a, PK_GEMV_SUB));
                if (pend) { std::swap(xa, xb); pend = nullptr; }
                ProfScope ps(dv, PK_ATTN, (double)d.Hs * AD * 2);
                const int rc = qtts_attn_o(t, ly.wo, d.Hs, dv->opart, st);
                if (rc < 0) return -1;
                if (rc == 1) {
                    ps.cancel();
                    { ProfScope pa(dv, PK_ATTN, 0); CKI(qtts_attention(t, st)); }
                    o.y = xa;
                    if (kzo) opend = split_out(dv, o, dv->bpo, kzo);
                    if (!kv_only) CKI(pgemv(dv, o, PK_GEMV_SUB));
                } else {
                    fused_o = true;
                }
            } else {
                if (tab0b) {
                    ProfScope pa(dv, PK_ATTN, 0);
                    CKI(qtts_attention(t, st));
                } else {
                    CKI(qkv_attn(dv, a, t, PK_GEMV_SUB));
                }
                if (pend) { std::swap(xa, xb); pend = nullptr; }
                o.y = xa;
                if (kzo) opend = split_out(dv, o, dv->bpo, kzo);
                if (sdbg) o.dbg = dv->gm_dbg + 2048 * 8;
                if (!kv_only) CKI(pgemv(dv, o, PK_GEMV_SUB));
            }
            if (kv_only) break;
            a = gv(ly.wgu, 2 * d.Is, d.Hs, xa, d.Hs, dv->h_s, d.Is, nb, EPI_SWIGLU);
            a.norm_w = ly.post; a.eps = d.eps; a.nt = 0;
            if (pfm & 4) a.pf = pf_gemvw(dv, ly.wdown, d.Hs, d.Is);
            if (sdbg) { a.dbg = dv->gm_dbg + 2 * 2048 * 8; DBG_XFIRST(a); }
            if (tab0) set_src(a);
            if (fused_o) {
                add_in(a, dv->opart, d.KVs, d.Hs, nb, xb);
            } else if (opend) {
                add_in(a, dv->bpo, kzo, d.Hs, nb, xb);
            }
            CKI(pgemv(dv, a, PK_GEMV_SUB));
            if (fused_o || opend) std::swap(xa, xb);
            a = gv(ly.wdown, d.Hs, d.Is, dv->h_s, d.Is, xa, d.Hs, nb, EPI_RESID);
            a.nt = 0;
            if (pfm & 8) {
                if (l + 1 < d.Ls) a.pf = pf_gemvw(dv, dv->sl[l + 1].wqkv, QKV, d.Hs);
                else if (g >= 1) a.pf = pf_gemvw(dv, dv->lm + (size_t)(g - 1) * d.Vs * d.Hs, d.Vs, d.Hs);
            }
            if (sdbg) { a.dbg = dv->gm_dbg + 3 * 2048 * 8; DBG_XFIRST(a); }
            if (kzd && split_out(dv, a, dv->bpd, kzd)) { pend = dv->bpd; npend = kzd; }
            CKI(pgemv(dv, a, PK_GEMV_SUB));
        }
        if (g == 0) continue;
        CKI(pass_head(g, xa, pend, npend));
    }
    return 0;
}

static int embed_sum(qtts_dev *dv, int advance) {
    const qtts_dims_t &d = dv->d;
    EmbedSumArgs e;
    e.codes = dv->codes; e.codes_bstride = (dv->max_frames + 1) * d.G; e.G = d.G;
    e.cur_row = dv->cur_row; e.stopped = dv->stopped; e.codec_emb = dv->codec_emb; e.st_emb = dv->st_emb;
    e.Vs = d.Vs; e.H = d.H; e.nb = dv->nrun; e.trailing = dv->trailing; e.tr_cap = dv->tr_cap;
    e.n_trailing = dv->n_trailing; e.pad = dv->pad_emb; e.out = dv->x_tk; e.kv_len = dv->kv_len; e.advance = advance;
    ProfScope ps(dv, PK_EMBED, 0);
    return qtts_embed_sum(e, dv->st);
}

static int record_frame(qtts_dev *dv, bool with_talker) {
    dv->tk_xfin = dv->x_tk; dv->tk_pend = nullptr; dv->tk_npend = 0;
    if (with_talker) CKI(talker_layers(dv));
    CKI(talker_head_sample(dv));
    CKI(subtalker(dv));
    CKI(embed_sum(dv, with_talker ? 1 : 0));
    return 0;
}

static int capture(qtts_dev *dv, bool with_talker, hipGraphExec_t *out) {
    hipGraph_t g = nullptr;
    CK(hipStreamBeginCapture(dv->st, hipStreamCaptureModeThreadLocal));
    int rc = record_frame(dv, with_talker);
    hipError_t e = hipStreamEndCapture(dv->st, &g);
    if (rc || e != hipSuccess) {
        fprintf(stderr, "qtts: frame graph capture failed\n");
        if (g) hipGraphDestroy(g);
        return -1;
    }
    e = hipGraphInstantiate(out, g, nullptr, nullptr, 0);
    hipGraphDestroy(g);
    CK(e);
    return 0;
}

static int ensure_graphs(qtts_dev *dv) {
    const int want = dv->f_armed ? 2 : dv->sp_armed ? (dv->sp_general ? 4 : 3) : 1;
    if (dv->g0 && dv->gN && dv->graph_key == want) return 0;
    if (dv->f_phase == 2 && (dv->g0 || dv->gN)) CK(hipStreamSynchronize(dv->st));
    if (dv->g0) { hipGraphExecDestroy(dv->g0); dv->g0 = nullptr; }
    if (dv->gN) { hipGraphExecDestroy(dv->gN); dv->gN = nullptr; }
    drop_row_graphs(dv);
    if (getenv("QTTS_HIP_NO_GRAPH")) { dv->graph_key = 0; return 0; }
    const int nrun = dv->nrun;
    dv->nrun = dv->nb;
    int rc = capture(dv, false, &dv->g0);
    if (!rc) rc = capture(dv, true, &dv->gN);
    dv->nrun = nrun;
    CKI(rc);
    dv->graph_key = want;
    return 0;
}

static bool force_refuses(const qtts_dev *dv, const char *what) {
    if (!dv->f_armed) return false;
    fprintf(stderr, "qtts: %s refused: forced codes / taps are armed (not defined for the work queue)\n", what);
    return true;
}

static bool same_params(const qtts_gen_params_t &a, const qtts_gen_params_t &b) {
    return memcmp(&a, &b, sizeof a) == 0;
}

static bool wide_shapes_ok(const qtts_dev *dv) {
    const qtts_dims_t &d = dv->d;
    const struct { const char *name; int R, C; bool used; } sh[] = {
        {"talker q|k|v", dv->QKV(), d.H, true},
        {"talker O", d.H, d.NH * d.HD, true},
        {"talker gate|up", 2 * d.I, d.H, true},
        {"talker down", d.H, d.I, true},
        {"codec head", d.V, d.H, true},
        {"sub-talker input projection", d.Hs, d.H, dv->st_proj != nullptr},
        {"sub-talker q|k|v", dv->QKVs(), d.Hs, true},
        {"sub-talker O", d.Hs, d.NHs * d.HDs, true},
        {"sub-talker gate|up", 2 * d.Is, d.Hs, true},
        {"sub-talker down", d.Hs, d.Is, true},
        {"sub-talker lm head", d.Vs, d.Hs, true},
    };
    for (const auto &s : sh)
        if (s.used && !qtts_gemvx_shape_ok(s.R, s.C)) {
            fprintf(stderr, "qtts_dev_begin: more than 16 slots refused: the wide batch GEMV does not take the %s "
                            "weights [%d][%d] (rows %% 16, columns %% 32)\n", s.name, s.R, s.C);
            return false;
        }
    return true;
}

extern "C" int qtts_dev_begin(qtts_dev_t *dv, int nb, int max_frames, int max_prefill, const qtts_gen_params_t *p) {
    if (!dv || nb < 1 || max_frames < 1) return -1;
// ... 242 lines not shown
    for (int *p : {dv->kv_len, dv->n_gen, dv->cur_row, dv->stopped, dv->stop_step, dv->last_tok, dv->n_trailing})
        CK(row(p, 4));
    CK(row(dv->rng, 4));
    CK(row(dv->st_rng, 4));
    if (dv->sp_armed) {
        CK(row(dv->sp_tab, sizeof(SampSlotRow)));
        dv->sp_host[to] = dv->sp_host[from];
    }
    CK(hipStreamSynchronize(st));
    dv->p_len_h[to] = dv->p_len_h[from];
    dv->n_tr_h[to] = dv->n_tr_h[from];
    if (dv->hstop && from < dv->hstop_cap && to < dv->hstop_cap)
        ((volatile int *)dv->hstop)[to] = ((volatile int *)dv->hstop)[from];
    return 0;
}

extern "C" int qtts_dev_set_rows(qtts_dev_t *dv, int rows) {
    if (!dv || rows < 1 || rows > dv->nb || (rows < dv->nb && rows > QTTS_MAX_SLOTS)) return -1;
    if (force_refuses(dv, "qtts_dev_set_rows")) return -1;
    dv->nrun = rows;
    return 0;
}

extern "C" int qtts_dev_reserve(qtts_dev_t *dv, int max_trailing) {
    if (!dv || max_trailing < 0) return -1;
    hipSetDevice(dv->device);
    return ensure_trailing(dv, max_trailing);
}

extern "C" int qtts_dev_frame(qtts_dev_t *dv, int step) {
    if (!dv) return -1;
    hipSetDevice(dv->device);
    CKI(ensure_graphs(dv));
    if (dv->nrun < dv->nb && step == 0) return -1;
    dv->f_phase = 2;
    if (dv->graph_key == 0) return record_frame(dv, step > 0);
    hipGraphExec_t g = step == 0 ? dv->g0 : dv->gN;
    if (dv->nrun < dv->nb) {
        hipGraphExec_t &gr = dv->gNr[dv->nrun];
        if (!gr) CKI(capture(dv, true, &gr));
        g = gr;
    }
    CK(hipGraphLaunch(g, dv->st));
    CK(hipEventRecord(dv->fev[step & 1], dv->st));
    return 0;
}

extern "C" int qtts_dev_frame_done(qtts_dev_t *dv, int step, int *all_stopped) {
    if (!dv || !all_stopped || !dv->hstop) return -1;
    hipSetDevice(dv->device);
    if (dv->graph_key >= 1) CK(hipEventSynchronize(dv->fev[step & 1]));
    else CK(hipStreamSynchronize(dv->st));
    int all = 1;
    for (int b = 0; b < dv->nrun; ++b) all &= ((volatile int *)dv->hstop)[b] != 0;
    *all_stopped = all;
    return 0;
}

extern "C" int qtts_dev_poll(qtts_dev_t *dv, int *stopped, int *n_gen, int *stop_step) {
    if (!dv) return -1;
    hipSetDevice(dv->device);
    const size_t B = dv->nb;
    if (stopped) CK(hipMemcpyAsync(stopped, dv->stopped, B * 4, hipMemcpyDeviceToHost, dv->st));
    if (n_gen) CK(hipMemcpyAsync(n_gen, dv->n_gen, B * 4, hipMemcpyDeviceToHost, dv->st));
    if (stop_step) CK(hipMemcpyAsync(stop_step, dv->stop_step, B * 4, hipMemcpyDeviceToHost, dv->st));
    CK(hipStreamSynchronize(dv->st));
    return 0;
}

extern "C" int qtts_dev_get_codes(qtts_dev_t *dv, int b, int *host_codes, int max_frames) {
    if (!dv || b < 0 || b >= dv->nb) return -1;
    hipSetDevice(dv->device);
    int n = 0;
    CK(hipMemcpyAsync(&n, dv->n_gen + b, 4, hipMemcpyDeviceToHost, dv->st));
    CK(hipStreamSynchronize(dv->st));
    if (dv->te_ctl) {
        int ctl[2] = {0, 0};
        CK(hipMemcpy(ctl, dv->te_ctl, sizeof(ctl), hipMemcpyDeviceToHost));
        if (ctl[1]) {
            fprintf(stderr, "qtts: talker layer engine hand-off timed out (code %d, epoch %d)\n", ctl[1], ctl[0]);
            return -1;
        }
    }
    if (dv->gm_dbg && dv->te_g) {
        std::vector<unsigned long long> h(2 * 256 * 16);
        CK(hipMemcpy(h.data(), dv->gm_dbg, h.size() * 8, hipMemcpyDeviceToHost));
        static const char *ph[15] = {"start", "x staged", "qkv dot", "qkv put", "head got", "attn done", "att staged",
                                     "O dot", "x' got", "x' staged", "gu dot", "h staged", "down dot", "ld issued",
                                     "ld landed"};
        unsigned long long t00 = ~0ull;
        for (int i = 0; i < 256; ++i) if (h[i * 16] && h[i * 16] < t00) t00 = h[i * 16];
        for (int g = 0; g < 2; ++g) {
            const unsigned long long *b = h.data() + (size_t)g * 256 * 16;
            unsigned long long t0 = ~0ull;
            for (int i = 0; i < 256; ++i) if (b[i * 16] && b[i * 16] < t0) t0 = b[i * 16];
            if (t0 == ~0ull) continue;
            fprintf(stderr, "[te_dbg] layer +%d starts %7.2f us after layer +0\n", g, (t0 - t00) * 0.01);
            for (int k = 0; k < 15; ++k) {
                std::vector<double> v;
                for (int i = 0; i < 256; ++i) if (b[i * 16 + k]) v.push_back((b[i * 16 + k] - t0) * 0.01);
                if (v.empty()) continue;
                std::sort(v.begin(), v.end());
                fprintf(stderr, "[te_dbg] +%d %-10s n %3zu  min %6.2f  med %6.2f  max %6.2f us\n", g, ph[k], v.size(), v[0],
                        v[v.size() / 2], v.back());
            }
        }
        hipMemsetAsync(dv->gm_dbg, 0, h.size() * 8, dv->st);
    } else if (dv->gm_dbg) {
        std::vector<unsigned long long> h(4 * 2048 * 8);
        CK(hipMemcpy(h.data(), dv->gm_dbg, h.size() * 8, hipMemcpyDeviceToHost));
        static const char *op[4] = {"q|k|v", "O / -", "gate|up", "down"};
        static const char *ph[7] = {"start", "x staged", "dot done", "epilogue", "pf landed", "w issued", "merged"};
        unsigned long long tq = 0;
        for (int g = 0; g < 4; ++g) {
            const unsigned long long *b = h.data() + (size_t)g * 2048 * 8;
            unsigned long long t0 = ~0ull, tend = 0;
            for (int i = 0; i < 2048; ++i) if (b[i * 8] && b[i * 8] < t0) t0 = b[i * 8];
            for (int i = 0; i < 2048 * 8; ++i) if (b[i] > tend) tend = b[i];
            if (t0 != ~0ull) {
                if (!tq) tq = t0;
                fprintf(stderr, "[gm_dbg] %-8s launch at %7.2f us after the first, last stamp %6.2f us into it\n", op[g],
                        (t0 - tq) * 0.01, (tend - t0) * 0.01);
            }
            for (int k = 0; k < 7; ++k) {
                std::vector<double> v;
                for (int i = 0; i < 2048; ++i) if (b[i * 8 + k]) v.push_back((b[i * 8 + k] - t0) * 0.01);
                if (v.empty()) continue;
                std::sort(v.begin(), v.end());
                fprintf(stderr, "[gm_dbg] %-8s %-10s n %4zu  min %6.2f  med %6.2f  max %6.2f us\n", op[g], ph[k], v.size(),
                        v[0], v[v.size() / 2], v.back());
            }
        }
        hipMemsetAsync(dv->gm_dbg, 0, h.size() * 8, dv->st);
    }
    if (n > max_frames) n = max_frames;
    CK(hipMemcpyAsync(host_codes, dv->codes + (size_t)b * (dv->max_frames + 1) * dv->d.G, (size_t)n * dv->d.G * 4,
                      hipMemcpyDeviceToHost, dv->st));
    CK(hipStreamSynchronize(dv->st));
    return n;
}

static int arm_force(qtts_dev *dv) {
    if (dv->f_phase != 1) {
        fprintf(stderr, "qtts: forced codes / taps are armed after qtts_dev_begin and before frame 0\n");
        return -1;
    }
    if (dv->f_armed) return 0;
    if (dv->sp_armed) {
        fprintf(stderr, "qtts: forced codes / taps refused: per-slot sampling parameters are armed for this run\n");
        return -1;
    }
    const qtts_dims_t &d = dv->d;
    const size_t tab = (size_t)dv->nb * (dv->max_frames + 1) * d.G * sizeof(int);
    const int ld = d.V > d.Vs ? d.V : d.Vs;
    const size_t taps = QTTS_MAX_TAPS * 3 * sizeof(int), meta = QTTS_MAX_TAPS * 4 * sizeof(int);
    const size_t lg = (size_t)QTTS_MAX_TAPS * ld * sizeof(float);
    dv->f_armed = true;
    CK(hipMalloc((void **)&dv->f_forced, tab));
    CK(hipMalloc((void **)&dv->f_drawn, tab));
    CK(hipMalloc((void **)&dv->f_taps, taps));
    CK(hipMalloc((void **)&dv->f_tap_meta, meta));
    CK(hipMalloc((void **)&dv->f_tap_logits, lg));
    dv->f_bytes = 2 * tab + taps + meta + lg;
    dv->sbytes += dv->f_bytes;
    dv->f_tap_ld = ld;
    dv->f_ntaps = 0;
    CK(hipMemsetAsync(dv->f_forced, 0xFF, tab, dv->st));
    CK(hipMemsetAsync(dv->f_drawn, 0xFF, tab, dv->st));
    CK(hipMemsetAsync(dv->f_taps, 0xFF, taps, dv->st));
    CK(hipMemsetAsync(dv->f_tap_meta, 0, meta, dv->st));
    CK(hipMemsetAsync(dv->f_tap_logits, 0, lg, dv->st));
    CK(hipStreamSynchronize(dv->st));
    dv->graph_key = -1;
    return 0;
}

extern "C" int qtts_dev_force(qtts_dev_t *dv, int b, const int *codes, int n_frames) {
    if (!dv) return -1;
    hipSetDevice(dv->device);
    const qtts_dims_t &d = dv->d;
    if (dv->f_phase != 1) return arm_force(dv);
    if (b < 0 || b >= dv->nb) {
        fprintf(stderr, "qtts_dev_force: slot %d out of range (%d slots)\n", b, dv->nb);
        return -1;
    }
    if (n_frames < 0 || n_frames > dv->f_run_frames || (n_frames > 0 && !codes)) {
        fprintf(stderr, "qtts_dev_force: %d frames outside [0, %d]\n", n_frames, dv->f_run_frames);
        return -1;
    }
    std::vector<int> h((size_t)n_frames * d.G);
    for (int f = 0; f < n_frames; ++f)
        for (int g = 0; g < d.G; ++g) {
            const int id = codes[(size_t)f * d.G + g];
            const bool ok = id < 0 || (g == 0 ? (id < d.V - 1024 || id == d.eos_id) && id < d.V : id < d.Vs);
            if (!ok) {
                fprintf(stderr, "qtts_dev_force: id %d at frame %d, group %d out of range\n", id, f, g);
                return -1;
            }
            h[(size_t)f * d.G + g] = id < 0 ? -1 : id;
        }
    CKI(arm_force(dv));
    int *row = dv->f_forced + (size_t)b * (dv->max_frames + 1) * d.G;
    CK(hipMemset(row, 0xFF, (size_t)(dv->max_frames + 1) * d.G * sizeof(int)));
    if (n_frames > 0) CK(hipMemcpy(row, h.data(), h.size() * sizeof(int), hipMemcpyHostToDevice));
    return 0;
}

extern "C" int qtts_dev_tap(qtts_dev_t *dv, int b, int frame, int group) {
    if (!dv) return -1;
    hipSetDevice(dv->device);
    if (dv->f_phase != 1) return arm_force(dv);
    if (b < 0 || b >= dv->nb || frame < 0 || frame >= dv->f_run_frames || group < 0 || group >= dv->d.G) {
        fprintf(stderr, "qtts_dev_tap: (slot %d, frame %d, group %d) out of range\n", b, frame, group);
// ... 408 lines not shown
        dv->graph_key = -1;
    }
    const SampSlotRow r = slot_row_of(*p);
    if (!slot_row_fast(dv, r)) dv->sp_general = true;
    const bool fresh = dv->f_phase == 1;
    CKI(qtts_slot_row_set(dv->sp_tab, b, r, fresh ? dv->rng : nullptr, fresh ? dv->st_rng : nullptr, dv->st));
    dv->sp_host[b] = r;
    return 0;
}

extern "C" long long qtts_hip_sample_slot_launches(void) { return qtts_sample_slot_launches(); }

static int ensure_slot0(qtts_dev *dv) {
    if (dv->nb >= 1) return 0;
    qtts_gen_params_t p{0.9f, 1.0f, 1.05f, 50, 0.9f, 1.0f, 50, 0, 42};
    return qtts_dev_begin(dv, 1, 4096, 256, &p);
}

extern "C" int qtts_dev_talker_prefill_host(qtts_dev_t *dv, const float *embeds, int n, float *hidden_out) {
    if (!dv) return -1;
    hipSetDevice(dv->device);
    CKI(ensure_slot0(dv));
    if (n > dv->p_cap) {
        qtts_gen_params_t p = dv->par;
        CKI(qtts_dev_begin(dv, dv->nb, dv->max_frames > 4096 ? dv->max_frames : 4096, n, &p));
    } else if (dv->kv_want != dv->kv_dtype) {
        qtts_gen_params_t p = dv->par;
        CKI(qtts_dev_begin(dv, dv->nb, dv->max_frames, dv->p_cap, &p));
    }
    const qtts_dims_t &d = dv->d;
    for (int b = 0; b < dv->nb; ++b) dv->p_len_h[b] = b == 0 ? n : 0;
    CK(hipMemcpy(dv->prefill, embeds, (size_t)n * d.H * 4, hipMemcpyHostToDevice));
    CKI(qtts_dev_prefill(dv));
    if (hidden_out) {
        GemvArgs a = gv(dv->head, d.V, d.H, dv->x_tk, d.H, dv->logits, d.V, 1, EPI_STORE);
        a.norm_w = dv->tk_norm; a.eps = d.eps; a.xcopy = dv->tk_hid; a.ldxc = d.H; a.xcopy_normed = 1;
        CKI(qtts_gemv(a, dv->st));
        CK(hipMemcpyAsync(hidden_out, dv->tk_hid, (size_t)d.H * 4, hipMemcpyDeviceToHost, dv->st));
        CK(hipStreamSynchronize(dv->st));
    }
    return 0;
}

extern "C" int qtts_dev_talker_forward_host(qtts_dev_t *dv, const float *embed, float *logits, float *hidden_out) {
    if (!dv) return -1;
    hipSetDevice(dv->device);
    CKI(ensure_slot0(dv));
    const qtts_dims_t &d = dv->d;
    dv->nrun = 1;
    int rc = 0;
    if (hipMemcpy(dv->x_tk, embed, (size_t)d.H * 4, hipMemcpyHostToDevice) != hipSuccess) rc = -1;
    if (!rc) rc = talker_layers(dv);
    if (!rc) rc = talker_tail(dv);
    dv->nrun = dv->nb;
    CKI(rc);
    int kl = 0;
    CK(hipMemcpyAsync(&kl, dv->kv_len, 4, hipMemcpyDeviceToHost, dv->st));
    CK(hipStreamSynchronize(dv->st));
    kl += 1;
    CK(hipMemcpy(dv->kv_len, &kl, 4, hipMemcpyHostToDevice));
    if (logits) CK(hipMemcpy(logits, dv->logits, (size_t)d.V * 4, hipMemcpyDeviceToHost));
    if (hidden_out) CK(hipMemcpy(hidden_out, dv->tk_hid, (size_t)d.H * 4, hipMemcpyDeviceToHost));
    return 0;
}

extern "C" int qtts_dev_subtalker_host(qtts_dev_t *dv, const float *hidden, int first_code, int *out_codes) {
    if (!dv) return -1;
    hipSetDevice(dv->device);
    CKI(ensure_slot0(dv));
    const qtts_dims_t &d = dv->d;
    CK(hipStreamSynchronize(dv->st));
    CK(hipMemcpy(dv->tk_hid, hidden, (size_t)d.H * 4, hipMemcpyHostToDevice));
    int zero = 0;
    uint32_t sb = seed_bits(dv->par.seed);
    CK(hipMemcpy(dv->cur_row, &zero, 4, hipMemcpyHostToDevice));
    CK(hipMemcpy(dv->stopped, &zero, 4, hipMemcpyHostToDevice));
    CK(hipMemcpy(dv->st_rng, &sb, 4, hipMemcpyHostToDevice));
    CK(hipMemcpy(dv->codes, &first_code, 4, hipMemcpyHostToDevice));
    CK(hipMemcpy(dv->last_tok, &first_code, 4, hipMemcpyHostToDevice));
    dv->nrun = 1;
    int rc = subtalker(dv);
    dv->nrun = dv->nb;
    CKI(rc);
    CK(hipMemcpyAsync(out_codes, dv->codes, (size_t)d.G * 4, hipMemcpyDeviceToHost, dv->st));
    CK(hipStreamSynchronize(dv->st));
    return 0;
}

extern "C" float *qtts_dev_codec_decode_host(qtts_dev_t *dv, const int *codes, int T, int *out_samples) {
    if (out_samples) *out_samples = 0;
    if (!dv || T < 1) return nullptr;
    hipSetDevice(dv->device);
    if (join_prime(dv)) return nullptr;
    int *dc = nullptr;
    if (hipMalloc(&dc, (size_t)T * dv->d.cq * 4) != hipSuccess) return nullptr;
    float *r = nullptr;
    if (hipMemcpy(dc, codes, (size_t)T * dv->d.cq * 4, hipMemcpyHostToDevice) == hipSuccess)
        r = codec_decode(&dv->codec, dc, T, out_samples);
    hipFree(dc);
    return r;
}

extern "C" int qtts_dev_codec_multi(qtts_dev_t *dv, int n, const int *const *host_codes, const int *slot, const int *T,
                                    float **audio, int *samples) {
    if (!dv || n < 1 || !T || !audio || !samples) return -1;
    for (int i = 0; i < n; ++i) {
        audio[i] = nullptr;
        samples[i] = 0;
        const bool host = host_codes && host_codes[i];
        if (T[i] < 1 || (!host && (!slot || slot[i] < 0 || slot[i] >= dv->nb || T[i] > dv->max_frames + 1)))
            return -1;
    }
    hipSetDevice(dv->device);
    CKI(join_prime(dv));
    const int cq = dv->d.cq;
    size_t nh = 0;
    for (int i = 0; i < n; ++i)
        if (host_codes && host_codes[i]) nh += (size_t)T[i] * cq;
    if (nh > dv->mcodes_cap) {
        CK(hipDeviceSynchronize());
        if (dv->mcodes) CK(hipFree(dv->mcodes));
        dv->mcodes = nullptr;
        dv->mcodes_cap = 0;
        CK(hipMalloc(&dv->mcodes, nh * 4));
        dv->mcodes_cap = nh;
    }
    std::vector<const int *> dcodes(n);
    size_t ho = 0;
    for (int i = 0; i < n; ++i) {
        if (host_codes && host_codes[i]) {
            CK(hipMemcpyAsync(dv->mcodes + ho, host_codes[i], (size_t)T[i] * cq * 4, hipMemcpyHostToDevice, dv->st));
            dcodes[i] = dv->mcodes + ho;
            ho += (size_t)T[i] * cq;
        } else {
            dcodes[i] = dv->codes + (size_t)slot[i] * (dv->max_frames + 1) * dv->d.G;
        }
    }
    const char *e = getenv("QTTS_HIP_CODEC_LANES");
    int nl = e ? atoi(e) : 8;
    if (nl < 1) nl = 1;
    if (nl > 16) nl = 16;
    if (nl > n) nl = n;
    int tmax = 1;
    for (int i = 0; i < n; ++i) tmax = T[i] > tmax ? T[i] : tmax;
    const size_t per_lane = codec_state_bytes(&dv->codec, tmax);
    while (nl > 1 && (size_t)(nl - 1) * per_lane > ((size_t)16 << 30)) --nl;
    auto fail = [&]() {
        for (int i = 0; i < n; ++i) {
            free(audio[i]);
            audio[i] = nullptr;
            samples[i] = 0;
        }
        return -1;
    };
    if (nl == 1) {
        for (int i = 0; i < n; ++i) {
            audio[i] = codec_decode(&dv->codec, dcodes[i], T[i], &samples[i]);
            if (!audio[i]) return fail();
        }
        return 0;
    }
    while ((int)dv->clanes.size() < nl - 1) {
        hipStream_t st = nullptr;
        CK(hipStreamCreateWithFlags(&st, hipStreamNonBlocking));
        dv->clane_st.push_back(st);
        dv->clanes.push_back(codec_lane_new(&dv->codec, st));
// ... 144 lines not shown
    t.skip = skip;
    const int gph = NH % KV ? 1 : NH / KV, ch = qtts_attn_keys_per_split(HD, false, 0);
    t.nsplit = (S + ch - 1) / ch;
    const size_t part_n = (size_t)rows * KV * t.nsplit * (gph * HD + 2 * gph), cnt_n = (size_t)rows * KV;
    void *scratch = nullptr;
    CK(hipMalloc(&scratch, part_n * 4 + cnt_n * 4));
    t.part = (float *)scratch;
    t.cnt = (int *)(t.part + part_n);
    int rc = hipMemsetAsync(scratch, 0, part_n * 4 + cnt_n * 4, st) == hipSuccess ? 0 : -1;
    if (!rc) rc = qtts_attention(t, st);
    if (hipStreamSynchronize(st) != hipSuccess) rc = -1;
    hipFree(scratch);
    return rc;
}

extern "C" int qtts_hip_attn_decode(float *out, const float *qkv, void *kc, void *vc, const float *qn_w,
                                    const float *kn_w, const float *rope_cos, const float *rope_sin, const int *pos,
                                    int NH, int KV, int HD, int S, int rows, float eps, int kv_dtype, void *stream) {
    return qtts_hip_attn_decode_ex(out, qkv, kc, vc, qn_w, kn_w, rope_cos, rope_sin, pos, NH, KV, HD, S, rows, eps,
                                   kv_dtype, nullptr, stream);
}

extern "C" int qtts_hip_attn_cached(float *out, float *q, int ld_q, void *kc, void *vc, const float *qn_w,
                                    const float *kn_w, const float *rope_cos, const float *rope_sin,
                                    const int *row_b, const int *pos, int NH, int KV, int HD, int S, int slots,
                                    int rows, float eps, int win, int kv_dtype, int prep, void *stream) {
    if (!out || !q || !kc || !vc || !row_b || !pos) return -1;
    if (prep != 0 && prep != 1) return -1;
    if (prep && (!qn_w || !kn_w || !rope_cos || !rope_sin)) return -1;
    if (!attn_dims_ok(NH, KV, HD, S, rows, kv_dtype) || slots < 1 || win < 0) return -1;
    if (HD < 8 || HD > 128 || (HD & 7) || NH % KV || !qtts_attn_head_ok(HD)) return -1;
    if (ld_q < (prep ? NH + 2 * KV : NH) * HD) return -1;
    if (kv_dtype == 1 && win != 0) return -1;
    hipStream_t st = (hipStream_t)stream;
    CKI(attn_ints_ok("qtts_hip_attn_cached", "position", pos, rows, S, st));
    CKI(attn_ints_ok("qtts_hip_attn_cached", "slot", row_b, rows, slots, st));
    AttnArgs t;
    t.mode = 1; t.qkv = q; t.ld_qkv = ld_q; t.qn_w = qn_w; t.kn_w = kn_w; t.eps = eps;
    t.rope_cos = rope_cos; t.rope_sin = rope_sin;
    t.kc = (float *)kc; t.vc = (float *)vc; t.S = S; t.kv_dtype = kv_dtype;
    t.pos = pos; t.row_b = row_b; t.NH = NH; t.KV = KV; t.HD = HD; t.out = out; t.ld_out = NH * HD; t.nrows = rows;
    t.win = win;
    int rc = prep ? qtts_qk_prep(t, st) : 0;
    if (!rc) rc = qtts_attention(t, st);
    if (hipStreamSynchronize(st) != hipSuccess) rc = -1;
    return rc;
}

extern "C" int qtts_hip_attn_o(float *part, const float *qkv, float *kc, float *vc, const float *qn_w,
                               const float *kn_w, const float *rope_cos, const float *rope_sin, const int *pos,
                               const uint16_t *Wo, int R, int NH, int KV, int HD, int S, int rows, float eps,
                               void *stream) {
    if (!part || !qkv || !kc || !vc || !qn_w || !kn_w || !rope_cos || !rope_sin || !pos || !Wo) return -1;
    if (!attn_dims_ok(NH, KV, HD, S, rows, 0) || R < 1) return -1;
    AttnArgs t;
    t.mode = 0; t.qkv = qkv; t.ld_qkv = (NH + 2 * KV) * HD; t.qn_w = qn_w; t.kn_w = kn_w; t.eps = eps;
    t.rope_cos = rope_cos; t.rope_sin = rope_sin; t.kc = kc; t.vc = vc; t.S = S;
    t.pos = pos; t.NH = NH; t.KV = KV; t.HD = HD; t.ld_out = NH * HD; t.nrows = rows;
    if (!qtts_attn_o_covers(t, Wo)) return 1;
    hipStream_t st = (hipStream_t)stream;
    CKI(attn_ints_ok("qtts_hip_attn_o", "position", pos, rows, S, st));
    int rc = qtts_attn_o(t, Wo, R, part, st);
    if (hipStreamSynchronize(st) != hipSuccess) rc = -1;
    return rc;
}

extern "C" int qtts_hip_attn_o_pair(float *part, const float *qkv, float *kc, float *vc, const float *qn_w,
                                    const float *kn_w, const float *rope_cos, const float *rope_sin, const int *skip,
                                    const uint16_t *Wo, int R, int NH, int KV, int HD, int S, float eps,
                                    void *stream) {
    if (!part || !qkv || !kc || !vc || !qn_w || !kn_w || !rope_cos || !rope_sin || !Wo) return -1;
    if (!attn_dims_ok(NH, KV, HD, S, 2, 0) || R < 1) return -1;
    AttnArgs t;
    t.mode = 0; t.qkv = qkv; t.ld_qkv = (NH + 2 * KV) * HD; t.qn_w = qn_w; t.kn_w = kn_w; t.eps = eps;
    t.rope_cos = rope_cos; t.rope_sin = rope_sin; t.kc = kc; t.vc = vc; t.S = S;
    t.pos = nullptr; t.NH = NH; t.KV = KV; t.HD = HD; t.ld_out = NH * HD; t.nrows = 2; t.skip = skip;
    if (!qtts_attn_o_pair_covers(t, Wo)) return 1;
    hipStream_t st = (hipStream_t)stream;
    int rc = qtts_attn_o_pair(t, Wo, R, part, st);
    if (hipStreamSynchronize(st) != hipSuccess) rc = -1;
    return rc;
}

extern "C" int qtts_hip_resident_matvec_rows_bf16(float *out, const uint16_t *A, const float *x, const float *w,
                                                  float eps, int rows, int cols, int epi, const float *part,
                                                  int n_part, float *x_new, int nrows, void *stream) {
    if (!out || !A || !x || rows < 1 || cols < 1 || (nrows != 1 && nrows != 2)) return -1;
    if (epi != EPI_STORE && epi != EPI_RESID && epi != EPI_SWIGLU) return -1;
    if (part && n_part < 1) return -1;
    if (part && cols > 1024) return 1;
    GemvArgs a = gv(A, rows, cols, x, cols, out, epi == EPI_SWIGLU ? rows / 2 : rows, nrows, epi);
    a.norm_w = w; a.eps = eps; a.nt = 0;
    if (part) { a.xadd = part; a.n_xadd = n_part; a.ld_xadd = nrows * cols; a.ldb_xadd = cols; }
    if (x_new) { a.xcopy = x_new; a.ldxc = cols; a.xcopy_normed = 0; }
    return nrows == 2 ? qtts_gemvw_pair(a, (hipStream_t)stream) : qtts_gemvw(a, (hipStream_t)stream);
}

static int bgemv_desc_args(const qtts_bgemv_desc_t *d, GemvArgs &a) {
    if (!d || !d->A || d->rows < 1 || d->cols < 1 || d->batch < 2 || d->batch > QTTS_HIP_MAX_BATCH) return -1;
    if (d->epi < EPI_STORE || d->epi > EPI_SWIGLU || d->src < 0 || d->src > 2) return -1;
    if ((d->epi == EPI_BIAS || d->epi == EPI_BIAS_SILU) && !d->bias) return -1;
    if (d->src == 0 ? !d->x : (!d->table || !d->ids)) return -1;
    if (d->part_in && (d->src != 0 || d->n_part_in < 1 || d->n_part_in > 4)) return -1;
    if (d->kz < 0 || d->kz == 1 || d->kz > 4) return -1;
    if (d->kz >= 2 && (d->self_reduce ? !d->y : !d->part_out)) return -1;
    if (d->kz < 2 && !d->y) return -1;
    a = gv(d->A, d->rows, d->cols, d->src == 0 ? d->x : nullptr, d->ldx, d->y, d->ldy, d->batch, d->epi);
    if (d->src == 1) a.table = (const bf16_t *)d->table;
    if (d->src == 2) a.table_f32 = (const float *)d->table;
    a.ids = d->ids; a.ids_bstride = d->ids_bstride; a.ids_rstride = d->ids_rstride; a.ids_off = d->ids_off;
    a.row_sel = d->row_sel;
    if (d->part_in) {
        a.xadd = d->part_in; a.n_xadd = d->n_part_in; a.ld_xadd = d->batch * d->cols; a.ldb_xadd = d->cols;
    }
    a.norm_w = d->norm_w; a.eps = d->eps;
    if (d->xcopy) { a.xcopy = d->xcopy; a.ldxc = d->cols; a.xcopy_normed = d->xcopy_normed; }
    a.bias = d->bias;
    if (d->kz >= 2) {
        a.kz = d->kz; a.ld_ypart = (size_t)d->batch * d->rows;
        if (!d->self_reduce) { a.ypart = d->part_out; a.y = nullptr; }
    }
    return 0;
}

extern "C" int qtts_hip_batch_matvec_case(const qtts_bgemv_desc_t *d, void *stream) {
    GemvArgs a;
    if (bgemv_desc_args(d, a)) return -1;
    hipStream_t st = (hipStream_t)stream;
    float *scratch = nullptr;
    static int *ticks = nullptr;
    if (d->kz >= 2 && d->self_reduce) {
        if (!ticks) {
            CK(hipMalloc((void **)&ticks, QTTS_GM_TICKS * sizeof(int)));
            CK(hipMemset(ticks, 0, QTTS_GM_TICKS * sizeof(int)));
        }
        CK(hipMalloc((void **)&scratch, (size_t)d->kz * a.ld_ypart * 4));
        a.ypart = scratch; a.tick = ticks;
    }
    int rc = qtts_bgemv(a, st);
    if (hipStreamSynchronize(st) != hipSuccess) rc = -1;
    if (scratch) hipFree(scratch);
    return rc;
}

extern "C" int qtts_hip_batch_matvec_plan(const qtts_bgemv_desc_t *d, qtts_bgemv_plan_t *out) {
    GemvArgs a;
    if (!out || bgemv_desc_args(d, a)) return -1;
    if (d->kz >= 2 && d->self_reduce) { a.ypart = (float *)(uintptr_t)256; a.tick = (int *)(uintptr_t)256; }
    BgPlan p;
    const int rc = qtts_bgemv_plan(a, p);
    *out = qtts_bgemv_plan_t();
    if (rc) return rc;
    out->kernel = p.kernel; out->n_tmpl = p.nt;
    for (int i = 0; i < p.nt; ++i) out->tmpl[i] = p.t[i];
    out->src = p.src; out->grid_x = (int)p.grid.x; out->grid_y = (int)p.grid.y; out->block = (int)p.block.x;
    out->lds_bytes = p.smem; out->tpw = p.tpw; out->cch = p.cch;
    return 0;
}

extern "C" int qtts_dev_profile_frame(qtts_dev_t *dv, int step, int max, int *kind, double *bytes, float *ms,
                                      char *names) {
    if (!dv || dv->nb < 1) return -1;
    hipSetDevice(dv->device);
    CK(hipStreamSynchronize(dv->st));
    dv->prof.clear();
    dv->profiling = true;
// ... 19 lines not shown
```

### qwen3-tts-c_amd/qtts.py

```python
import ctypes as C
import os

import numpy as np

HERE = os.path.dirname(os.path.abspath(__file__))
LIB_PATH = os.environ.get("QTTS_LIB") or os.path.join(HERE, "lib", "libqwen_tts_amd.so")
CLI_PATH = os.path.join(HERE, "bin", "qwen-tts")

_fp = C.POINTER(C.c_float)
_ip = C.POINTER(C.c_int)

PROGRESS_CB = C.CFUNCTYPE(None, C.c_int, C.c_int, C.c_void_p)
QUEUE_NEXT_CB = C.CFUNCTYPE(C.c_int, C.c_void_p)
AUDIO_CB = C.CFUNCTYPE(None, C.POINTER(C.c_float), C.c_int, C.c_void_p)
BATCH_AUDIO_CB = C.CFUNCTYPE(None, C.c_int, C.POINTER(C.c_float), C.c_int, C.c_void_p)


class Config(C.Structure):
    _fields_ = [(n, C.c_int) for n in (
        "talker_vocab_size", "talker_hidden", "talker_intermediate", "talker_layers", "talker_heads",
        "talker_kv_heads", "talker_head_dim", "talker_text_hidden", "talker_text_vocab", "num_code_groups")] + [
        ("talker_rms_norm_eps", C.c_float), ("talker_rope_theta", C.c_float), ("mrope_section", C.c_int * 3)] + [
        (n, C.c_int) for n in (
            "subtalker_vocab_size", "subtalker_hidden", "subtalker_intermediate", "subtalker_layers",
# ... 1 lines not shown
            "codec_num_quantizers", "codec_codebook_size", "codec_codebook_dim", "codec_hidden", "codec_latent",
            "codec_layers", "codec_heads", "codec_kv_heads", "codec_intermediate", "codec_sliding_window",
            "codec_decoder_dim")] + [
        ("codec_rms_norm_eps", C.c_float), ("codec_layer_scale", C.c_float),
        ("codec_upsample_rates", C.c_int * 4), ("codec_upsampling_ratios", C.c_int * 2),
        ("n_speakers", C.c_int), ("speaker_names", C.POINTER(C.c_char_p)), ("speaker_ids", _ip),
        ("n_languages", C.c_int), ("language_names", C.POINTER(C.c_char_p)), ("language_ids", _ip)] + [
        (n, C.c_int) for n in ("codec_pad_id", "codec_bos_id", "codec_eos_id", "codec_nothink_id", "codec_think_id",
                               "codec_think_bos_id", "codec_think_eos_id")]


class Ctx(C.Structure):
    _fields_ = [
        ("config", Config), ("model_dir", C.c_char * 512), ("hip", C.c_void_p), ("hip_device", C.c_int),
        ("talker_kv_len", C.c_int), ("tk_x", _fp),
        ("temperature", C.c_float), ("subtalker_temperature", C.c_float), ("top_k", C.c_int),
        ("subtalker_top_k", C.c_int), ("top_p", C.c_float), ("subtalker_top_p", C.c_float),
        ("repetition_penalty", C.c_float), ("max_new_tokens", C.c_int), ("fixed_codec_tokens", C.c_int),
        ("sample_seed", C.c_int), ("progress_cb", C.c_void_p), ("progress_cb_userdata", C.c_void_p),
        ("perf_total_ms", C.c_double), ("perf_talker_ms", C.c_double), ("perf_codec_ms", C.c_double),
        ("perf_codec_tokens", C.c_int), ("perf_prefill_ms", C.c_double), ("perf_first_frame_ms", C.c_double),
        ("last_codes", _ip), ("last_frames", C.c_int), ("last_stop_reason", C.c_int), ("last_stop_step", C.c_int),
        ("perf_first_packet_ms", C.c_double),
        ("tokenizer", C.c_void_p),
        ("queue_n", C.c_int), ("queue_codes", C.POINTER(_ip)), ("queue_frames", _ip), ("queue_stop_reason", _ip),
        ("queue_slot", _ip), ("queue_slots", C.c_int), ("queue_frames_launched", C.c_int),
        ("queue_refills", C.c_int), ("queue_slot_frames_used", C.c_longlong), ("queue_rows_launched", C.c_longlong),
        ("sampling", C.c_void_p), ("force", C.c_void_p),
    ]


class Sampling(C.Structure):
    _fields_ = [("temperature", C.c_float), ("top_p", C.c_float), ("repetition_penalty", C.c_float),
                ("top_k", C.c_int), ("subtalker_temperature", C.c_float), ("subtalker_top_p", C.c_float),
                ("subtalker_top_k", C.c_int), ("sample_seed", C.c_int)]


class SlotParams(C.Structure):
    _fields_ = [("temperature", C.c_float), ("top_p", C.c_float), ("repetition_penalty", C.c_float),
                ("top_k", C.c_int), ("st_temperature", C.c_float), ("st_top_p", C.c_float), ("st_top_k", C.c_int),
                ("seed", C.c_int)]


EXPORTS = [
    "qwen_tts_load", "qwen_tts_free", "qwen_tts_set_progress_callback", "qwen_tts_generate", "qwen_tts_write_wav",
    "qwen_tts_talker_prefill", "qwen_tts_talker_forward", "qwen_tts_subtalker_generate", "qwen_tts_codec_decode",
    "qwen_tts_talker_hidden", "qwen_tts_load_on", "qwen_tts_generate_batch", "qwen_tts_last_codes", "qwen_tts_last_codes_slot",
    "qwen_tts_abi_sizeof_ctx", "qwen_tts_verbose", "qwen_tts_generate_stream", "qwen_tts_codec_stream_begin",
    "qwen_tts_codec_stream_push", "qwen_tts_generate_voice_clone",
    "qwen_tts_generate_voice_clone_batch", "qwen_tts_generate_voice_clone_stream", "qwen_tts_tokenize",
    "qwen_tts_text_prompt", "qwen_tts_speaker_embedding", "qwen_tts_encode_audio",
    "qwen_tts_generate_voice_clone_audio", "qwen_tts_generate_voice_clone_audio_batch",
    "qwen_tts_generate_voice_clone_audio_stream", "qtts_dev_codec_timing", "qtts_dev_codec_stage_ms", "qwen_tts_resample",
    "qtts_hip_device_count", "qtts_dev_create", "qtts_dev_destroy", "qtts_dev_put_tensor", "qtts_dev_finalize",
    "qtts_dev_bytes", "qtts_dev_begin", "qtts_dev_prompt", "qtts_dev_prompt_ref", "qtts_dev_prefill", "qtts_dev_frame", "qtts_dev_poll", "qtts_dev_frame_done",
    "qtts_dev_get_codes", "qtts_dev_codec_slot", "qtts_dev_talker_prefill_host", "qtts_dev_talker_forward_host",
    "qtts_dev_subtalker_host", "qtts_dev_codec_decode_host", "qtts_hip_matvec_bf16",
    "qtts_hip_rmsnorm_matvec_bf16", "qtts_hip_decode_matvec_bf16", "qtts_hip_resident_matvec_bf16", "qtts_hip_sample_top_k", "qtts_hip_causal_conv1d",
    "qtts_hip_transposed_conv1d", "qtts_hip_snake_beta", "qtts_hip_expf_glibc", "qtts_hip_sync",
    "qtts_dev_profile_frame", "qtts_hip_hbm_bw", "qtts_dev_codec_stream_begin", "qtts_dev_codec_stream_begin_ex",
    "qtts_dev_codec_stream_prime", "qtts_dev_codec_stream_push_slot",
    "qtts_dev_codec_stream_push_host", "qtts_dev_codec_async_begin", "qtts_dev_codec_async_push",
    "qtts_dev_codec_async_end", "qtts_dev_codec_multi", "qtts_dev_enc_config", "qtts_dev_enc_available", "qtts_dev_speaker_embed",
    "qtts_dev_encode_audio", "qwen_tts_generate_queue", "qwen_tts_queue_codes", "qtts_dev_reserve", "qtts_dev_refill",
    "qtts_dev_retire", "qtts_dev_frame_stops", "qtts_dev_move_slot", "qtts_dev_set_rows", "qtts_hip_tengine_layers",
    "qwen_tts_set_kv_cache_dtype", "qwen_tts_kv_cache_dtype", "qtts_dev_set_kv_dtype", "qtts_dev_kv_dtype",
    "qtts_dev_get_kv", "qtts_dev_get_attn", "qtts_hip_attn_decode",
    "qtts_hip_attn_decode_ex", "qtts_hip_attn_cached", "qtts_hip_attn_o",
    "qtts_hip_attn_o_pair", "qtts_hip_resident_matvec_rows_bf16", "qtts_hip_st_pair_passes",
    "qwen_tts_force_codes", "qwen_tts_tap_draw", "qwen_tts_last_drawn", "qwen_tts_tap_result",
    "qtts_dev_force", "qtts_dev_tap", "qtts_dev_get_drawn", "qtts_dev_get_tap",
    "qtts_hip_xgemm_plan", "qtts_hip_xgemm_case", "qtts_hip_xgemm_func",
    "qtts_hip_batch_matvec_case", "qtts_hip_gemv_wide_launches", "qtts_hip_batch_matvec_plan",
    "qwen_tts_sampling_defaults", "qwen_tts_set_utterance_sampling", "qtts_dev_slot_params",
    "qtts_hip_sample_slot_launches", "qtts_hip_sample_top_k_rows",
    "qwen_tts_generate_batch_stream", "qwen_tts_codec_mstream_begin", "qwen_tts_codec_mstream_push",
    "qtts_dev_codec_mstream_begin", "qtts_dev_codec_mstream_push_slots", "qtts_dev_codec_mstream_push_host",
    "qtts_dev_codec_mstream_pos", "qtts_hip_xgemm_seg_case",
    "qwen_tts_generate_queue_stream", "qwen_tts_codec_mstream_push_any", "qwen_tts_codec_mstream_reset",
    "qtts_dev_codec_mstream_push_host_any", "qtts_dev_codec_mstream_push_slots_at", "qtts_dev_codec_mstream_reset",
    "qwen_tts_codec_mstream_push_ragged", "qtts_dev_codec_mstream_push_host_ragged",
    "qtts_dev_codec_mstream_push_slots_ragged", "qtts_dev_codec_mstream_prime",
    "qwen_tts_generate_voice_clone_batch_stream", "qwen_tts_generate_voice_clone_audio_batch_stream",
]

MAX_BATCH = 64


class BGemvDesc(C.Structure):
    _fields_ = [
        ("rows", C.c_int), ("cols", C.c_int), ("batch", C.c_int),
        ("A", C.c_void_p),
        ("src", C.c_int),
        ("x", C.c_void_p), ("ldx", C.c_int),
        ("table", C.c_void_p),
        ("ids", C.c_void_p), ("ids_bstride", C.c_int), ("ids_rstride", C.c_int), ("ids_off", C.c_int),
        ("row_sel", C.c_void_p),
        ("part_in", C.c_void_p), ("n_part_in", C.c_int),
        ("norm_w", C.c_void_p), ("eps", C.c_float),
        ("xcopy", C.c_void_p), ("xcopy_normed", C.c_int),
        ("epi", C.c_int),
        ("bias", C.c_void_p),
        ("y", C.c_void_p), ("ldy", C.c_int),
        ("kz", C.c_int), ("self_reduce", C.c_int),
        ("part_out", C.c_void_p),
    ]


class BGemvPlan(C.Structure):
    _fields_ = [
        ("kernel", C.c_int),
        ("n_tmpl", C.c_int), ("tmpl", C.c_int * 5),
        ("src", C.c_int),
        ("grid_x", C.c_int), ("grid_y", C.c_int), ("block", C.c_int),
        ("lds_bytes", C.c_size_t),
        ("tpw", C.c_int), ("cch", C.c_int),
    ]


BGEMV_KERNELS = {1: "k_gemvm", 2: "k_gemvb", 4: "k_gemvx"}


class XGemmDesc(C.Structure):
    _fields_ = [
        ("M", C.c_int), ("N", C.c_int), ("K", C.c_int),
        ("amode", C.c_int), ("bmode", C.c_int), ("emode", C.c_int),
        ("A", C.c_void_p), ("lda", C.c_int),
        ("B", C.c_void_p), ("ldb", C.c_int),
        ("Kw", C.c_int), ("dil", C.c_int), ("pad", C.c_int), ("L", C.c_int), ("stride", C.c_int),
        ("tmin", C.c_int), ("co", C.c_int),
        ("sa", C.c_void_p), ("sb", C.c_void_p),
        ("C", C.c_void_p), ("ldc", C.c_int),
        ("bias", C.c_void_p), ("vec", C.c_void_p), ("aux", C.c_void_p), ("res", C.c_void_p),
        ("ldaux", C.c_int), ("ldres", C.c_int),
        ("ea", C.c_void_p), ("eb", C.c_void_p),
    ]


XA_ROWS, XA_TRANS, XA_TCONV_W = 0, 1, 2
XB_WT, XB_CONV, XB_TCONV = 0, 1, 2
(XE_STORE, XE_BIAS_N, XE_BIAS_N_GELU, XE_SILU_MUL, XE_SCALE_RESID_N, XE_BIAS_T, XE_BIAS_GAMMA_RES_T, XE_BIAS_M,
 XE_BIAS_M_RES, XE_BIAS_M_SNAKE) = range(10)
XP_CONVB2, XP_CONVB4, XP_CONV, XP_XLIN, XP_XGEMV, XP_XGEMM = range(6)
XP_NAMES = ["k_convb<Kw,2>", "k_convb<Kw,4>", "k_conv<Kw>", "k_xlin", "k_xgemv", "k_xgemm"]

MAX_TAPS = 8

KV_F32, KV_BF16 = 0, 1

_LIB = None


def tokenize(model_dir, text):
    n = C.c_int(0)
    p = lib().qwen_tts_tokenize(model_dir.encode(), text.encode("utf-8"), C.byref(n))
    if not p:
        return None
    ids = np.ctypeslib.as_array(C.cast(p, _ip), shape=(n.value,)).tolist() if n.value else []
    _libc.free(C.c_void_p(p))
    return ids


def resample(wav, sr_in, sr_out=24000):
    w = np.ascontiguousarray(wav, np.float32)
    n = C.c_int(0)
    p = lib().qwen_tts_resample(w.ctypes.data_as(_fp), w.shape[0], int(sr_in), int(sr_out), C.byref(n))
# ... 101 lines not shown
        L.qtts_dev_codec_mstream_prime.argtypes = [C.c_void_p, C.c_int, _ip, _ip, _ip, C.c_int]
        L.qwen_tts_generate_voice_clone_batch_stream.restype = C.c_int
        L.qwen_tts_generate_voice_clone_batch_stream.argtypes = [
            C.POINTER(Ctx), C.c_int, C.POINTER(C.c_char_p), C.POINTER(C.c_char_p), C.POINTER(_ip), _ip,
            C.POINTER(_fp), C.POINTER(C.c_char_p), C.c_int, C.c_int, BATCH_AUDIO_CB, C.c_void_p,
            C.POINTER(C.c_void_p), _ip]
        L.qwen_tts_generate_voice_clone_audio_batch_stream.restype = C.c_int
        L.qwen_tts_generate_voice_clone_audio_batch_stream.argtypes = [
            C.POINTER(Ctx), C.c_int, C.POINTER(C.c_char_p), C.POINTER(C.c_char_p), C.POINTER(_fp), _ip,
            C.POINTER(C.c_char_p), _ip, C.c_int, C.c_int, BATCH_AUDIO_CB, C.c_void_p, C.POINTER(C.c_void_p), _ip]
    L.qwen_tts_speaker_embedding.restype = C.c_void_p
    L.qwen_tts_speaker_embedding.argtypes = [C.POINTER(Ctx), _fp, C.c_int, _ip]
    L.qwen_tts_encode_audio.restype = C.c_void_p
    L.qwen_tts_encode_audio.argtypes = [C.POINTER(Ctx), _fp, C.c_int, _ip]
    L.qwen_tts_generate_voice_clone_audio.restype = C.c_void_p
    L.qwen_tts_generate_voice_clone_audio.argtypes = [C.POINTER(Ctx), C.c_char_p, C.c_char_p, _fp, C.c_int,
                                                      C.c_char_p, C.c_int, C.c_int, _ip]
    L.qwen_tts_generate_voice_clone_audio_batch.restype = C.c_int
    L.qwen_tts_generate_voice_clone_audio_batch.argtypes = [C.POINTER(Ctx), C.c_int, C.POINTER(C.c_char_p),
                                                            C.POINTER(C.c_char_p), C.POINTER(_fp), _ip,
                                                            C.POINTER(C.c_char_p), _ip, C.c_int,
                                                            C.POINTER(C.c_void_p), _ip]
    L.qwen_tts_generate_voice_clone_audio_stream.restype = C.c_void_p
    L.qwen_tts_generate_voice_clone_audio_stream.argtypes = [C.POINTER(Ctx), C.c_char_p, C.c_char_p, _fp, C.c_int,
                                                             C.c_char_p, C.c_int, C.c_int, C.c_int, AUDIO_CB,
                                                             C.c_void_p, _ip]
    L.qtts_dev_enc_available.restype = C.c_int
    L.qtts_dev_enc_available.argtypes = [C.c_void_p]
    L.qtts_dev_speaker_embed.restype = C.c_int
    L.qtts_dev_speaker_embed.argtypes = [C.c_void_p, C.c_int, C.POINTER(_fp), _ip, _fp, _fp]
    L.qtts_dev_encode_audio.restype = C.c_int
    L.qtts_dev_encode_audio.argtypes = [C.c_void_p, C.c_int, C.POINTER(_fp), _ip, _ip, C.c_int, _ip, _fp]
    L.qwen_tts_set_kv_cache_dtype.restype = C.c_int
    L.qwen_tts_set_kv_cache_dtype.argtypes = [C.POINTER(Ctx), C.c_int]
    L.qwen_tts_kv_cache_dtype.restype = C.c_int
    L.qwen_tts_kv_cache_dtype.argtypes = [C.POINTER(Ctx)]
    L.qtts_dev_set_kv_dtype.restype = C.c_int
    L.qtts_dev_set_kv_dtype.argtypes = [C.c_void_p, C.c_int]
    L.qtts_dev_kv_dtype.restype = C.c_int
    L.qtts_dev_kv_dtype.argtypes = [C.c_void_p]
    L.qtts_dev_get_kv.restype = C.c_int
    L.qtts_dev_get_kv.argtypes = [C.c_void_p, C.c_int, C.c_int, C.c_int, C.c_int, _fp, _fp]
    L.qtts_dev_get_attn.restype = C.c_int
    L.qtts_dev_get_attn.argtypes = [C.c_void_p, _fp, _fp]
    L.qtts_dev_bytes.restype = C.c_size_t
    L.qtts_dev_bytes.argtypes = [C.c_void_p, C.c_int]
    _up = C.POINTER(C.c_uint)
    L.qwen_tts_force_codes.restype = C.c_int
    L.qwen_tts_force_codes.argtypes = [C.POINTER(Ctx), C.c_int, _ip, C.c_int]
    L.qwen_tts_tap_draw.restype = C.c_int
    L.qwen_tts_tap_draw.argtypes = [C.POINTER(Ctx), C.c_int, C.c_int, C.c_int]
    L.qwen_tts_last_drawn.restype = C.c_int
    L.qwen_tts_last_drawn.argtypes = [C.POINTER(Ctx), C.c_int, _ip, C.c_int]
    L.qwen_tts_tap_result.restype = C.c_int
    L.qwen_tts_tap_result.argtypes = [C.POINTER(Ctx), C.c_int, _fp, C.c_int, _up, _ip]
    L.qtts_dev_force.restype = C.c_int
    L.qtts_dev_force.argtypes = [C.c_void_p, C.c_int, _ip, C.c_int]
    L.qtts_dev_tap.restype = C.c_int
    L.qtts_dev_tap.argtypes = [C.c_void_p, C.c_int, C.c_int, C.c_int]
    L.qtts_dev_get_drawn.restype = C.c_int
    L.qtts_dev_get_drawn.argtypes = [C.c_void_p, C.c_int, _ip, C.c_int]
    L.qtts_dev_get_tap.restype = C.c_int
    L.qtts_dev_get_tap.argtypes = [C.c_void_p, C.c_int, _fp, C.c_int, _up, _ip]
    L.qtts_hip_device_count.restype = C.c_int
    L.qtts_hip_tengine_layers.restype = C.c_longlong
    vp = C.c_void_p
    L.qtts_hip_matvec_bf16.argtypes = [vp, vp, vp, C.c_int, C.c_int, C.c_int, vp]
    L.qtts_hip_rmsnorm_matvec_bf16.argtypes = [vp, vp, vp, vp, C.c_float, C.c_int, C.c_int, C.c_int, vp]
    L.qtts_hip_decode_matvec_bf16.argtypes = [vp, vp, vp, vp, C.c_float, C.c_int, C.c_int, C.c_int, vp]
    L.qtts_hip_resident_matvec_bf16.argtypes = [vp, vp, vp, vp, C.c_float, C.c_int, C.c_int, C.c_int, vp]
    L.qtts_hip_sample_top_k.argtypes = [vp, vp, C.c_int, C.c_int, C.c_float, C.c_float, vp, C.c_int, vp]
    L.qtts_hip_causal_conv1d.argtypes = [vp, vp, vp, vp, C.c_int, C.c_int, C.c_int, C.c_int, C.c_int, C.c_int, vp]
    L.qtts_hip_transposed_conv1d.argtypes = [vp, vp, vp, vp, C.c_int, C.c_int, C.c_int, C.c_int, C.c_int, vp]
    L.qtts_hip_snake_beta.argtypes = [vp, vp, vp, vp, C.c_int, C.c_int, vp]
    L.qtts_hip_expf_glibc.argtypes = [vp, vp, C.c_int, vp]
    L.qtts_hip_attn_decode.restype = C.c_int
    L.qtts_hip_attn_decode.argtypes = [vp] * 9 + [C.c_int] * 5 + [C.c_float, C.c_int, vp]
    L.qtts_hip_attn_decode_ex.restype = C.c_int
    L.qtts_hip_attn_decode_ex.argtypes = [vp] * 9 + [C.c_int] * 5 + [C.c_float, C.c_int, vp, vp]
    L.qtts_hip_attn_cached.restype = C.c_int
    L.qtts_hip_attn_cached.argtypes = [vp, vp, C.c_int] + [vp] * 8 + [C.c_int] * 6 + [C.c_float] + [C.c_int] * 3 + [vp]
    L.qtts_hip_attn_o.restype = C.c_int
    L.qtts_hip_attn_o.argtypes = [vp] * 10 + [C.c_int] * 6 + [C.c_float, vp]
    if hasattr(L, "qtts_hip_st_pair_passes"):
        L.qtts_hip_st_pair_passes.restype = C.c_longlong
        L.qtts_hip_attn_o_pair.restype = C.c_int
        L.qtts_hip_attn_o_pair.argtypes = [vp] * 10 + [C.c_int] * 5 + [C.c_float, vp]
        L.qtts_hip_resident_matvec_rows_bf16.restype = C.c_int
        L.qtts_hip_resident_matvec_rows_bf16.argtypes = ([vp] * 4 + [C.c_float] + [C.c_int] * 3 + [vp, C.c_int, vp,
                                                                                                C.c_int, vp])
    if hasattr(L, "qtts_hip_xgemm_case"):
        L.qtts_hip_xgemm_plan.restype = C.c_int
        L.qtts_hip_xgemm_plan.argtypes = [C.POINTER(XGemmDesc), C.c_size_t, C.c_int, _ip, _ip]
        L.qtts_hip_xgemm_case.restype = C.c_int
        L.qtts_hip_xgemm_case.argtypes = [C.POINTER(XGemmDesc), C.c_size_t, C.c_int, _ip, _ip, vp]
        L.qtts_hip_xgemm_func.restype = C.c_int
        L.qtts_hip_xgemm_func.argtypes = [vp] * 4 + [C.c_int] * 3 + [vp]
    if hasattr(L, "qtts_hip_batch_matvec_case"):
        L.qtts_hip_batch_matvec_case.restype = C.c_int
        L.qtts_hip_batch_matvec_case.argtypes = [C.POINTER(BGemvDesc), vp]
        L.qtts_hip_gemv_wide_launches.restype = C.c_longlong
        L.qtts_hip_gemv_wide_launches.argtypes = []
    if hasattr(L, "qtts_dev_slot_params"):
        L.qwen_tts_sampling_defaults.restype = C.c_int
        L.qwen_tts_sampling_defaults.argtypes = [C.POINTER(Ctx), C.POINTER(Sampling)]
        L.qwen_tts_set_utterance_sampling.restype = C.c_int
        L.qwen_tts_set_utterance_sampling.argtypes = [C.POINTER(Ctx), C.c_int, C.POINTER(Sampling)]
        L.qtts_dev_slot_params.restype = C.c_int
        L.qtts_dev_slot_params.argtypes = [C.c_void_p, C.c_int, C.POINTER(SlotParams)]
        L.qtts_hip_sample_slot_launches.restype = C.c_longlong
        L.qtts_hip_sample_slot_launches.argtypes = []
        L.qtts_hip_sample_top_k_rows.restype = C.c_int
        L.qtts_hip_sample_top_k_rows.argtypes = [vp, vp, C.c_int, _ip, _fp, _fp, vp, C.c_int, vp]
    if hasattr(L, "qtts_hip_batch_matvec_plan"):
        L.qtts_hip_batch_matvec_plan.restype = C.c_int
        L.qtts_hip_batch_matvec_plan.argtypes = [C.POINTER(BGemvDesc), C.POINTER(BGemvPlan)]
    _LIB = L
    return L


_libc = C.CDLL("libc.so.6")
_libc.free.argtypes = [C.c_void_p]


def _take_audio(ptr, n):
    if not ptr or n <= 0:
        return None
    a = np.ctypeslib.as_array(C.cast(ptr, _fp), shape=(n,)).copy()
    _libc.free(ptr)
    return a


def set_verbose(v):
    C.c_int.in_dll(lib(), "qwen_tts_verbose").value = int(v)


class QwenTTS:

    def __init__(self, model_dir, device=0):
        L = lib()
        self.ctx = L.qwen_tts_load_on(model_dir.encode(), int(device))
        if not self.ctx:
            raise RuntimeError(f"qwen_tts_load({model_dir}) failed")
        self.c = self.ctx.contents
        self.cfg = self.c.config
        self._last_nb = 1

    def close(self):
        if self.ctx:
            lib().qwen_tts_free(self.ctx)
            self.ctx = None

    def __del__(self):
        try:
            self.close()
        except Exception:
            pass

    def set_params(self, max_tokens=4096, fixed=0, seed=42, temperature=0.9, top_k=50, top_p=1.0, rep=1.05,
                   st_temperature=0.9, st_top_k=50, st_top_p=1.0):
        c = self.c
        c.temperature, c.top_k, c.top_p, c.repetition_penalty = temperature, top_k, top_p, rep
        c.subtalker_temperature, c.subtalker_top_k, c.subtalker_top_p = st_temperature, st_top_k, st_top_p
        c.max_new_tokens, c.fixed_codec_tokens, c.sample_seed = max_tokens, fixed, seed

    def set_kv_cache(self, dtype):
# ... 503 lines not shown
    import torch
    return C.c_void_p(torch.cuda.current_stream().cuda_stream)


def _ok(rc, what):
    if rc != 0:
        raise RuntimeError(f"{what} failed (rc={rc})")


class Kernels:

    @staticmethod
    def matvec_bf16(out, A_u16, x, rows, cols, batch=1):
        _ok(lib().qtts_hip_matvec_bf16(_ptr(out), _ptr(A_u16), _ptr(x), rows, cols, batch, _stream()), "matvec")

    @staticmethod
    def rmsnorm_matvec_bf16(out, A_u16, x, w, eps, rows, cols, batch=1):
        _ok(lib().qtts_hip_rmsnorm_matvec_bf16(_ptr(out), _ptr(A_u16), _ptr(x), _ptr(w), eps, rows, cols, batch,
                                               _stream()), "rmsnorm_matvec")

    @staticmethod
    def decode_matvec_bf16(out, A_u16, x, w, eps, rows, cols, batch=1):
        _ok(lib().qtts_hip_decode_matvec_bf16(_ptr(out), _ptr(A_u16), _ptr(x), _ptr(w) if w is not None else None,
                                              eps, rows, cols, batch, _stream()), "decode_matvec")

    @staticmethod
    def resident_matvec_bf16(out, A_u16, x, w, eps, rows, cols, epi=0):
        _ok(lib().qtts_hip_resident_matvec_bf16(_ptr(out), _ptr(A_u16), _ptr(x), _ptr(w) if w is not None else None,
                                                eps, rows, cols, epi, _stream()), "resident_matvec")

    @staticmethod
    def sample_top_k(out_i32, logits, vocab, top_k, top_p, temperature, rng_u32, batch=1):
        _ok(lib().qtts_hip_sample_top_k(_ptr(out_i32), _ptr(logits), vocab, top_k, top_p, temperature,
                                        _ptr(rng_u32), batch, _stream()), "sample")

    @staticmethod
    def causal_conv1d(out, x, w, b, ci, co, k, L, dil=1, groups=1):
        _ok(lib().qtts_hip_causal_conv1d(_ptr(out), _ptr(x), _ptr(w), _ptr(b), ci, co, k, L, dil, groups,
                                         _stream()), "conv1d")

    @staticmethod
    def transposed_conv1d(out, x, w, b, ci, co, k, stride, L):
        _ok(lib().qtts_hip_transposed_conv1d(_ptr(out), _ptr(x), _ptr(w), _ptr(b), ci, co, k, stride, L,
                                             _stream()), "tconv1d")

    @staticmethod
    def snake_beta(out, x, alpha, inv_beta, C_, L):
        _ok(lib().qtts_hip_snake_beta(_ptr(out), _ptr(x), _ptr(alpha), _ptr(inv_beta), C_, L, _stream()), "snake")

    @staticmethod
    def expf_glibc(out, x, n):
        _ok(lib().qtts_hip_expf_glibc(_ptr(out), _ptr(x), n, _stream()), "expf")

    @staticmethod
    def attn_decode(out, qkv, kc, vc, qn_w, kn_w, rope_cos, rope_sin, pos_i32, NH, KV, HD, S, rows, eps, kv_dtype=0):
        _ok(lib().qtts_hip_attn_decode(_ptr(out), _ptr(qkv), _ptr(kc), _ptr(vc), _ptr(qn_w), _ptr(kn_w),
                                       _ptr(rope_cos), _ptr(rope_sin), _ptr(pos_i32), NH, KV, HD, S, rows, eps,
                                       kv_dtype, _stream()), "attn_decode")

    @staticmethod
    def attn_decode_ex(out, qkv, kc, vc, qn_w, kn_w, rope_cos, rope_sin, pos_i32, NH, KV, HD, S, rows, eps,
                       kv_dtype=0, skip_i32=None):
        _ok(lib().qtts_hip_attn_decode_ex(_ptr(out), _ptr(qkv), _ptr(kc), _ptr(vc), _ptr(qn_w), _ptr(kn_w),
                                          _ptr(rope_cos), _ptr(rope_sin), _ptr(pos_i32), NH, KV, HD, S, rows, eps,
                                          kv_dtype, _ptr(skip_i32), _stream()), "attn_decode_ex")

    @staticmethod
    def attn_cached(out, q, ld_q, kc, vc, qn_w, kn_w, rope_cos, rope_sin, row_b_i32, pos_i32, NH, KV, HD, S, slots,
                    rows, eps, win=0, kv_dtype=0, prep=0):
        _ok(lib().qtts_hip_attn_cached(_ptr(out), _ptr(q), ld_q, _ptr(kc), _ptr(vc), _ptr(qn_w), _ptr(kn_w),
                                       _ptr(rope_cos), _ptr(rope_sin), _ptr(row_b_i32), _ptr(pos_i32), NH, KV, HD, S,
                                       slots, rows, eps, win, kv_dtype, prep, _stream()), "attn_cached")

    @staticmethod
    def attn_o(part, qkv, kc, vc, qn_w, kn_w, rope_cos, rope_sin, pos_i32, Wo_u16, R, NH, KV, HD, S, rows, eps):
        rc = lib().qtts_hip_attn_o(_ptr(part), _ptr(qkv), _ptr(kc), _ptr(vc), _ptr(qn_w), _ptr(kn_w), _ptr(rope_cos),
                                   _ptr(rope_sin), _ptr(pos_i32), _ptr(Wo_u16), R, NH, KV, HD, S, rows, eps, _stream())
        if rc == 1:
            return False
        _ok(rc, "attn_o")
        return True

    @staticmethod
    def attn_o_pair(part, qkv, kc, vc, qn_w, kn_w, rope_cos, rope_sin, Wo_u16, R, NH, KV, HD, S, eps, skip_i32=None):
        rc = lib().qtts_hip_attn_o_pair(_ptr(part), _ptr(qkv), _ptr(kc), _ptr(vc), _ptr(qn_w), _ptr(kn_w),
                                        _ptr(rope_cos), _ptr(rope_sin), _ptr(skip_i32), _ptr(Wo_u16), R, NH, KV, HD,
                                        S, eps, _stream())
        if rc == 1:
            return False
        _ok(rc, "attn_o_pair")
        return True

    @staticmethod
    def resident_matvec_rows_bf16(out, A_u16, x, w, eps, rows, cols, epi=0, part=None, x_new=None, nrows=1):
        rc = lib().qtts_hip_resident_matvec_rows_bf16(_ptr(out), _ptr(A_u16), _ptr(x), _ptr(w), eps, rows, cols, epi,
                                                      _ptr(part), 0 if part is None else int(part.shape[0]),
                                                      _ptr(x_new), nrows, _stream())
        if rc == 1:
            return False
        _ok(rc, "resident_matvec_rows")
        return True

    @staticmethod
    def bgemv_desc(A_u16, batch, y, x=None, table=None, ids_i32=None, ids_bstride=1, ids_rstride=0, ids_off=0,
                   row_sel_i32=None, part_in=None, norm_w=None, eps=1e-6, xcopy=None, xcopy_normed=False,
                   epi=0, bias=None, kz=0, self_reduce=True, part_out=None):
        d = BGemvDesc()
        d.rows, d.cols, d.batch = int(A_u16.shape[0]), int(A_u16.shape[1]), int(batch)
        d.A = _ptr(A_u16)
        if table is not None:
            d.src = 1 if table.element_size() == 2 else 2
            d.table, d.ids = _ptr(table), _ptr(ids_i32)
            d.ids_bstride, d.ids_rstride, d.ids_off = ids_bstride, ids_rstride, ids_off
            d.row_sel = _ptr(row_sel_i32)
        else:
            d.src, d.x, d.ldx = 0, _ptr(x), int(x.stride(0))
        if part_in is not None:
            d.part_in, d.n_part_in = _ptr(part_in), int(part_in.shape[0])
        d.norm_w, d.eps = _ptr(norm_w), eps
        d.xcopy, d.xcopy_normed = _ptr(xcopy), int(bool(xcopy_normed))
        d.epi, d.bias = epi, _ptr(bias)
        d.y, d.ldy = _ptr(y), (int(y.stride(0)) if y is not None else 0)
        d.kz, d.self_reduce, d.part_out = kz, int(bool(self_reduce)), _ptr(part_out)
        return d

    @staticmethod
    def batch_matvec_case(A_u16, batch, y, **kw):
        d = Kernels.bgemv_desc(A_u16, batch, y, **kw)
        rc = lib().qtts_hip_batch_matvec_case(C.byref(d), _stream())
        if rc == 1:
            return False
        _ok(rc, "batch_matvec_case")
        return True

    @staticmethod
    def batch_matvec_plan(desc):
        p = BGemvPlan()
        rc = lib().qtts_hip_batch_matvec_plan(C.byref(desc), C.byref(p))
        if rc == 1:
            return None
        _ok(rc, "batch_matvec_plan")
        return dict(kernel=BGEMV_KERNELS[p.kernel], tmpl=list(p.tmpl[:p.n_tmpl]), grid=[p.grid_x, p.grid_y],
                    block=p.block, lds=int(p.lds_bytes), tpw=p.tpw, cch=p.cch)

    @staticmethod
    def sample_top_k_rows(out_i32, logits, vocab, top_k, top_p, temperature, rng_u32, batch=1):
        k = np.ascontiguousarray(top_k, np.int32)
        p = np.ascontiguousarray(top_p, np.float32)
        t = np.ascontiguousarray(temperature, np.float32)
        assert k.shape == p.shape == t.shape == (batch,)
        _ok(lib().qtts_hip_sample_top_k_rows(_ptr(out_i32), _ptr(logits), vocab, k.ctypes.data_as(_ip),
                                             p.ctypes.data_as(_fp), t.ctypes.data_as(_fp), _ptr(rng_u32), batch,
                                             _stream()), "sample_top_k_rows")

    @staticmethod
    def sample_slot_launches():
        return int(lib().qtts_hip_sample_slot_launches())

    @staticmethod
    def gemv_wide_launches():
        return int(lib().qtts_hip_gemv_wide_launches())

    @staticmethod
    def xgemm_plan(desc, part_elems=0, force_path=-1):
        path, splits = C.c_int(-1), C.c_int(0)
        rc = lib().qtts_hip_xgemm_plan(C.byref(desc), part_elems, force_path, C.byref(path), C.byref(splits))
# ... 31 lines not shown
```

Measured before the change: 35.28 audio-s/s.

## Fuse sub-talker RMSNorm, QKV projection, attention and O-projection into one kernel

Adds a kernel for the sub-talker decode step that does input RMSNorm, the QKV GEMV, q/k norm, RoPE, a short-context attention and the O-projection GEMV in a single launch. Workgroups exchange their q/k/v slices through epoch-tagged 64-bit granules in global memory and spin until every slice arrives. This removes separate launches and the intermediate qkv round trip to memory. In exchange it depends on all workgroups being co-resident, adds a spin timeout with an error flag checked on the host, and adds a per-step epoch bump kernel.

New measurement: 35.88 audio-s/s, median of 5. 1.02x the previous value.

```diff
diff --git a/include/qtts_hip.h b/include/qtts_hip.h
--- a/include/qtts_hip.h
+++ b/include/qtts_hip.h
@@ -171,6 +171,13 @@
                          const float *rope_cos_dev, const float *rope_sin_dev, const int *skip_dev,
                          const uint16_t *Wo_dev, int R, int NH, int KV, int HD, int S, float eps,
                          void *stream);
+int qtts_hip_qkv_attn_o(float *part_dev, const float *x_dev, const float *in_w_dev, const uint16_t *Wqkv_dev,
+                        float *kc_dev, float *vc_dev, const float *qn_w_dev, const float *kn_w_dev,
+                        const float *rope_cos_dev, const float *rope_sin_dev, const int *skip_dev,
+                        const uint16_t *Wo_dev, unsigned long long *g_dev, int *ctl_dev, int idx, int pos, int R,
+                        int cols, int NH, int KV, int HD, int S, float eps, int bump, int sync, void *stream);
+int qtts_hip_st_fuse_row(int NH, int KV, int HD, int b, int m);
+int qtts_hip_st_fuse_pf_rows(int NH, int KV, int HD, int cols, int b, int *rows, int max);
 int qtts_hip_resident_matvec_rows_bf16(float *out_dev, const uint16_t *A_dev, const float *x_dev, const float *w_dev,
                                        float eps, int rows, int cols, int epi, const float *part_dev, int n_part,
                                        float *x_new_dev, int nrows, void *stream);
@@ -233,6 +240,8 @@
 int qtts_hip_sync(void);
 long long qtts_hip_tengine_layers(void);
 long long qtts_hip_st_pair_passes(void);
+long long qtts_hip_st_fused_launches(void);
+int qtts_dev_debug_set_handoff_err(qtts_dev_t *dv, int which, int code);
 long long qtts_hip_gemv_wide_launches(void);
 long long qtts_hip_sample_slot_launches(void);
 
diff --git a/qwen3-tts-c_amd/csrc/hip/k_misc.hip b/qwen3-tts-c_amd/csrc/hip/k_misc.hip
--- a/qwen3-tts-c_amd/csrc/hip/k_misc.hip
+++ b/qwen3-tts-c_amd/csrc/hip/k_misc.hip
@@ -10,6 +10,7 @@
     const int stop = a.stopped ? a.stopped[b] : 0;
     const int row = a.cur_row[b];
     const int ntr = a.n_trailing[b];
+    if (a.epoch && blockIdx.x == 0 && b == 0 && threadIdx.x == 0) a.epoch[0] += 1;
     if (stop) return;
     const int *cd = a.codes + (size_t)b * a.codes_bstride + (size_t)row * a.G;
     constexpr int GM = 16;
diff --git a/qwen3-tts-c_amd/csrc/hip/k_stfuse.hip b/qwen3-tts-c_amd/csrc/hip/k_stfuse.hip
--- /dev/null
+++ b/qwen3-tts-c_amd/csrc/hip/k_stfuse.hip
@@ -0,0 +1,295 @@
+#include "qtts_common.h"
+#include "qtts_kernels.h"
+#include "qtts_handoff_dev.h"
+#include "qtts_l2pf.h"
+
+int qtts_stfuse_row(int NH, int KV, int HD, int b, int m) {
+    const int kvh = b % KV, rb = b / KV, nq = HD / 8;
+    if (rb < nq) return 2 * kvh * HD + 16 * rb + m;
+    const int j = rb - nq;
+    return (m < 8 ? NH * HD : (NH + KV) * HD) + kvh * HD + 8 * j + (m & 7);
+}
+
+namespace {
+
+__device__ __forceinline__ float dot8w(const v4u &w, const float *x) {
+    const float4 x0 = *reinterpret_cast<const float4 *>(x);
+    const float4 x1 = *reinterpret_cast<const float4 *>(x + 4);
+    float s = 0.f;
+    s = fmaf(__uint_as_float(w.x << 16), x0.x, s); s = fmaf(__uint_as_float(w.x & 0xFFFF0000u), x0.y, s);
+    s = fmaf(__uint_as_float(w.y << 16), x0.z, s); s = fmaf(__uint_as_float(w.y & 0xFFFF0000u), x0.w, s);
+    s = fmaf(__uint_as_float(w.z << 16), x1.x, s); s = fmaf(__uint_as_float(w.z & 0xFFFF0000u), x1.y, s);
+    s = fmaf(__uint_as_float(w.w << 16), x1.z, s); s = fmaf(__uint_as_float(w.w & 0xFFFF0000u), x1.w, s);
+    return s;
+}
+
+__device__ __forceinline__ float sumsq4(const float4 &v) {
+    return __fadd_rn(__fadd_rn(__fadd_rn(__fmul_rn(v.x, v.x), __fmul_rn(v.y, v.y)), __fmul_rn(v.z, v.z)),
+                     __fmul_rn(v.w, v.w));
+}
+__device__ __forceinline__ float dot4_fused(const float4 &q, const float4 &k) {
+    return fmaf(q.w, k.w, fmaf(q.z, k.z, fmaf(q.x, k.x, __fmul_rn(q.y, k.y))));
+}
+__device__ __forceinline__ float dot4_rounded(const float4 &q, const float4 &k) {
+    return __fadd_rn(__fadd_rn(__fadd_rn(__fmul_rn(q.x, k.x), __fmul_rn(q.y, k.y)), __fmul_rn(q.z, k.z)),
+                     __fmul_rn(q.w, k.w));
+}
+__device__ __forceinline__ float rot_sub(float a, float c, float b, float s) {
+    return __fsub_rn(__fmul_rn(a, c), __fmul_rn(b, s));
+}
+__device__ __forceinline__ float rot_add(float a, float c, float b, float s) {
+    return __fadd_rn(__fmul_rn(a, c), __fmul_rn(b, s));
+}
+
+__device__ __forceinline__ void sf_stamp(const StFuseArgs &f, int k) {
+#ifdef QTTS_STAMPS
+    if (f.dbg && threadIdx.x == 0) f.dbg[blockIdx.x * 8 + k] = __builtin_amdgcn_s_memrealtime();
+#endif
+}
+
+template <int HD>
+__global__ __launch_bounds__(256) void k_qkv_attn_o(const float *x, const bf16_t *Wqkv, int NH, int KV,
+                                                    const float *norm_w, int *ctl, StFuseArgs f, AttnArgs t,
+                                                    const bf16_t *Wo, int R, float *part) {
+    constexpr int C = QTTS_SF_C, NV = C / 512, RW = 4;
+    constexpr int W2 = 2 * HD, LPS = W2 / 8 < 8 ? W2 / 8 : 8, NJ = W2 / (8 * LPS), RPW = 256 / LPS;
+    constexpr int D4 = HD / 4, LPK = HD / 16, NK = 16, NG = 4 * HD / 64;
+    static_assert(HD == 128, "threads < 4 HD / 4 stage one float4 each; 16 rows x HD / 4 workgroups = 4 HD");
+    __shared__ __attribute__((aligned(16))) float xs[C];
+    __shared__ __attribute__((aligned(16))) float raw[4 * HD];
+    __shared__ __attribute__((aligned(16))) float lq[4 * HD];
+    __shared__ __attribute__((aligned(16))) float att[W2];
+    __shared__ __attribute__((aligned(16))) float red[4];
+    __shared__ float sc[2][NK];
+    sf_stamp(f, 0);
+    const int tid = threadIdx.x, lane = tid & 63, w = tid >> 6;
+    const int b = blockIdx.x, kvh = b % KV, rb = b / KV;
+    const float4 zero4 = make_float4(0.f, 0.f, 0.f, 0.f);
+
+    const float4 xv = reinterpret_cast<const float4 *>(x)[tid];
+    const float4 nwv = reinterpret_cast<const float4 *>(norm_w)[tid];
+    __builtin_amdgcn_sched_barrier(0);
+
+    const int nq = HD / 8, jkv = rb - nq;
+    v4u wv[RW][NV];
+#pragma unroll
+    for (int i = 0; i < RW; ++i) {
+        const int m = w + 4 * i;
+        const int r = rb < nq ? 2 * kvh * HD + 16 * rb + m
+                              : (m < 8 ? NH * HD : (NH + KV) * HD) + kvh * HD + 8 * jkv + (m & 7);
+        const v4u *p = reinterpret_cast<const v4u *>(Wqkv + (size_t)r * C) + lane;
+#pragma unroll
+        for (int k = 0; k < NV; ++k) wv[i][k] = p[64 * k];
+    }
+    asm volatile("" ::"s"(ctl), "s"(t.skip), "s"(t.pos_const), "s"(t.S), "s"(t.qn_w), "s"(t.kn_w), "s"(t.rope_cos),
+                 "s"(t.rope_sin), "s"(t.kc), "s"(t.vc), "s"(Wo), "s"(R), "s"(t.pf.base), "s"(t.pf.pm), "s"(t.pf.pa),
+                 "s"(t.pf.pb), "s"(t.pf.chunks), "s"(t.pf.lg), "s"(t.pf.ld), "s"(t.pf.cs), "s"(t.pf.nwg));
+    __builtin_amdgcn_sched_barrier(0);
+
+    const unsigned epoch = (unsigned)__hip_atomic_load(ctl, __ATOMIC_RELAXED, __HIP_MEMORY_SCOPE_AGENT);
+    const int err0 = __hip_atomic_load(ctl + 1, __ATOMIC_RELAXED, __HIP_MEMORY_SCOPE_AGENT);
+    int skipv = *(t.skip ? t.skip : ctl);
+    if (!t.skip) skipv = 0;
+    const int p = t.pos_const, n = p + 1, KVD = KV * HD, AD = NH * HD;
+    const int seg = tid / D4, l = tid - seg * D4;
+    float4 nwq = zero4, c4 = zero4, s4 = zero4;
+    if (seg < 3) {
+        nwq = reinterpret_cast<const float4 *>(seg < 2 ? t.qn_w : t.kn_w)[l];
+        c4 = reinterpret_cast<const float4 *>(t.rope_cos + (size_t)p * HD)[l];
+        s4 = reinterpret_cast<const float4 *>(t.rope_sin + (size_t)p * HD)[l];
+    }
+    const float *Kc = t.kc + kvh * HD, *Vc = t.vc + kvh * HD;
+    const int dI = tid / LPK, sub = tid - dI * LPK, gs = dI / NK, ts = dI - gs * NK;
+    float4 kr[4];
+    {
+        const int tr = gs < 2 && ts < t.S ? ts : 0;
+        const float4 *kp = reinterpret_cast<const float4 *>(Kc + (size_t)tr * KVD + 16 * sub);
+#pragma unroll
+        for (int c = 0; c < 4; ++c) kr[c] = kp[c];
+    }
+    const int go = tid / HD, dd = tid - go * HD;
+    float vr[NK];
+#pragma unroll
+    for (int k = 0; k < NK; ++k) vr[k] = Vc[(size_t)(k < t.S ? k : t.S - 1) * KVD + dd];
+    const int slot = tid / LPS, so = tid - slot * LPS;
+    const int row = rb * RPW + slot, rowc = row < R ? row : R - 1;
+    v4u wo[NJ];
+    const bf16_t *wr = Wo + (size_t)rowc * AD + W2 * kvh + 8 * so;
+#pragma unroll
+    for (int j = 0; j < NJ; ++j) wo[j] = *reinterpret_cast<const v4u *>(wr + 8 * LPS * j);
+    const int wu = __builtin_amdgcn_readfirstlane(w);
+    L2PfRegs pfr;
+    qtts_l2pf_issue<QTTS_SF_PF_THREADS>(t.pf, wu < 3 ? b : t.pf.nwg, pfr, Wo);
+    __builtin_amdgcn_sched_barrier(0);
+
+    float ss = sumsq4(xv);
+    ss = wave_sum(ss);
+    if (lane == 0) red[w] = ss;
+    __syncthreads();
+    const float inv = rms_inv(red[0] + red[1] + red[2] + red[3], C, f.eps);
+    {
+        float4 v = xv;
+        v.x = v.x * inv * nwv.x; v.y = v.y * inv * nwv.y; v.z = v.z * inv * nwv.z; v.w = v.w * inv * nwv.w;
+        reinterpret_cast<float4 *>(xs)[tid] = v;
+    }
+    __syncthreads();
+    sf_stamp(f, 1);
+
+    float acc[RW];
+#pragma unroll
+    for (int i = 0; i < RW; ++i) {
+        float s = 0.f;
+#pragma unroll
+        for (int k = 0; k < NV; ++k) s += dot8w(wv[i][k], xs + 8 * (lane + 64 * k));
+        acc[i] = wave_sum(s);
+    }
+    sf_stamp(f, 2);
+    if (skipv) return;
+
+    const unsigned tag = epoch * (unsigned)QTTS_SF_MAX_IDX + (unsigned)f.idx + 1u;
+    u64 *gh = f.g + (size_t)kvh * 4 * HD;
+    {
+        float v = acc[0];
+#pragma unroll
+        for (int i = 1; i < RW; ++i)
+            if (lane == i) v = acc[i];
+        const int m = w + 4 * (lane & 3);
+        const int tl = rb < nq ? 16 * rb + m : (m < 8 ? 2 * HD : 3 * HD) + 8 * jkv + (m & 7);
+        if (lane < RW) put_granule(gh + tl, tag, v);
+    }
+    sf_stamp(f, 3);
+    if (wu == 3) {
+        float v[NG];
+#pragma unroll
+        for (int j = 0; j < NG; ++j) v[j] = 0.f;
+        if (!err0) sweep<NG>(gh, tag, [&](int j) { return lane + 64 * j; }, v, ctl + 1, 30);
+#pragma unroll
+        for (int j = 0; j < NG; ++j) raw[lane + 64 * j] = v[j];
+    }
+    __syncthreads();
+    sf_stamp(f, 4);
+
+    float4 q = zero4;
+    if (seg < 4) q = reinterpret_cast<const float4 *>(raw)[tid];
+    float s2 = sumsq4(q);
+    s2 = group_sum<D4>(s2);
+    if (seg < 3) {
+        const float iv = rms_inv(s2, HD, t.eps);
+        q.x = q.x * iv * nwq.x; q.y = q.y * iv * nwq.y; q.z = q.z * iv * nwq.z; q.w = q.w * iv * nwq.w;
+    }
+    float4 o4;
+    if constexpr (D4 / 2 == 16) {
+        o4.x = xor16_get(q.x); o4.y = xor16_get(q.y); o4.z = xor16_get(q.z); o4.w = xor16_get(q.w);
+    } else {
+        o4.x = __shfl_xor(q.x, D4 / 2, 64); o4.y = __shfl_xor(q.y, D4 / 2, 64);
+        o4.z = __shfl_xor(q.z, D4 / 2, 64); o4.w = __shfl_xor(q.w, D4 / 2, 64);
+    }
+    if (seg < 4) {
+        float4 y = q;
+        if (seg < 3) {
+            if (l < D4 / 2) {
+                y.x = rot_sub(q.x, c4.x, o4.x, s4.x); y.y = rot_sub(q.y, c4.y, o4.y, s4.y);
+                y.z = rot_sub(q.z, c4.z, o4.z, s4.z); y.w = rot_sub(q.w, c4.w, o4.w, s4.w);
+            } else {
+                y.x = rot_add(q.x, c4.x, o4.x, s4.x); y.y = rot_add(q.y, c4.y, o4.y, s4.y);
+                y.z = rot_add(q.z, c4.z, o4.z, s4.z); y.w = rot_add(q.w, c4.w, o4.w, s4.w);
+            }
+        }
+        reinterpret_cast<float4 *>(lq)[tid] = y;
+        if (seg >= 2 && rb == 0) {
+            float *dst = (seg == 2 ? t.kc : t.vc) + (size_t)p * KVD + kvh * HD;
+            reinterpret_cast<float4 *>(dst)[l] = y;
+        }
+    }
+    __syncthreads();
+
+    {
+        float d = 0.f;
+        if (gs < 2 && ts < n) {
+            const float4 *q4 = reinterpret_cast<const float4 *>(lq + gs * HD + 16 * sub);
+            const float4 *k4 = reinterpret_cast<const float4 *>(lq + 2 * HD + 16 * sub);
+#pragma unroll
+            for (int c = 0; c < 4; ++c) {
+                const float4 k = ts == p ? k4[c] : kr[c], qq = q4[c];
+                d = __fadd_rn(d, c == 3 ? dot4_rounded(qq, k) : dot4_fused(qq, k));
+            }
+        }
+        d = group_sum<LPK>(d);
+        if (sub == 0 && gs < 2) sc[gs][ts] = ts < n ? d * div_rn(1.0f, sqrt_rn((float)HD)) : -INFINITY;
+    }
+    __syncthreads();
+
+    if (tid < 2 * NK) {
+        const int g = tid / NK, k = tid - g * NK;
+        const float s = sc[g][k];
+        float mx = s;
+        mx = group_max<NK>(mx);
+        const float e = k < n ? expf(s - mx) : 0.f;
+        float sum = e;
+        sum = group_sum<NK>(sum);
+        sc[g][k] = e * div_rn(1.0f, sum);
+    }
+    __syncthreads();
+
+    if (go < 2) {
+        float a = 0.f;
+#pragma unroll
+        for (int k = 0; k < NK; ++k)
+            if (k < n) a = fmaf(sc[go][k], k == p ? lq[3 * HD + dd] : vr[k], a);
+        att[go * HD + dd] = a;
+    }
+    __syncthreads();
+    sf_stamp(f, 5);
+
+    float o = 0.f;
+#pragma unroll
+    for (int j = 0; j < NJ; ++j) {
+        float fw[8];
+        unpack8(wo[j], fw);
+        const float *xp = att + 8 * (so + LPS * j);
+        const float4 x0 = *reinterpret_cast<const float4 *>(xp);
+        const float4 x1 = *reinterpret_cast<const float4 *>(xp + 4);
+        o = fmaf(fw[0], x0.x, o); o = fmaf(fw[1], x0.y, o);
+        o = fmaf(fw[2], x0.z, o); o = fmaf(fw[3], x0.w, o);
+        o = fmaf(fw[4], x1.x, o); o = fmaf(fw[5], x1.y, o);
+        o = fmaf(fw[6], x1.z, o); o = fmaf(fw[7], x1.w, o);
+    }
+    o = group_sum<LPS>(o);
+    sf_stamp(f, 6);
+    if (so == 0 && row < R) part[(size_t)kvh * R + row] = o;
+    qtts_l2pf_sink(t.pf, pfr);
+    sf_stamp(f, 7);
+}
+
+__global__ void k_stfuse_epoch(int *ctl) { ctl[0] += 1; }
+
+}
+
+bool qtts_qkv_attn_o_covers(const StFuseArgs &f, const AttnArgs &a, const bf16_t *Wo, int R) {
+    if (!qtts_attn_o_covers(a, Wo) || a.nrows != 1 || a.pos || a.qkv_tab || a.xc_dst) return false;
+    if (a.HD != 128 || R != 8 * a.HD || f.C != QTTS_SF_C || a.pos_const < 0 || a.pos_const >= a.S) return false;
+    if (!f.x || !f.norm_w || !f.Wqkv || !f.g || !f.ctl || f.idx < 0 || f.idx >= QTTS_SF_MAX_IDX) return false;
+    return (((uintptr_t)f.x | (uintptr_t)f.norm_w | (uintptr_t)f.Wqkv) & 15) == 0 && ((uintptr_t)f.g & 7) == 0;
+}
+
+int qtts_qkv_attn_o(const StFuseArgs &f, const AttnArgs &a0, const bf16_t *Wo, int R, float *part, hipStream_t st) {
+    if (!qtts_qkv_attn_o_covers(f, a0, Wo, R)) return 1;
+    AttnArgs a = a0;
+    if (a.pf.chunks > QTTS_SF_PF_THREADS * QTTS_PF_LOADS) a.pf.chunks = QTTS_SF_PF_THREADS * QTTS_PF_LOADS;
+    const dim3 grid((a.HD / 4) * a.KV);
+    hipLaunchKernelGGL((k_qkv_attn_o<128>), grid, dim3(256), 0, st, f.x, f.Wqkv, a.NH, a.KV, f.norm_w, f.ctl, f, a, Wo, R,
+                       part);
+    qtts_last_kernel = "k_qkv_attn_o<128>";
+    return hipGetLastError() == hipSuccess ? 0 : -1;
+}
+
+int qtts_qkv_attn_o_blocks_per_cu() {
+    int n = 0;
+    if (hipOccupancyMaxActiveBlocksPerMultiprocessor(&n, k_qkv_attn_o<128>, 256, 0) != hipSuccess) return 0;
+    return n;
+}
+
+int qtts_stfuse_epoch_bump(int *ctl, hipStream_t st) {
+    hipLaunchKernelGGL(k_stfuse_epoch, dim3(1), dim3(1), 0, st, ctl);
+    return hipGetLastError() == hipSuccess ? 0 : -1;
+}
diff --git a/qwen3-tts-c_amd/csrc/hip/k_tengine.hip b/qwen3-tts-c_amd/csrc/hip/k_tengine.hip
--- a/qwen3-tts-c_amd/csrc/hip/k_tengine.hip
+++ b/qwen3-tts-c_amd/csrc/hip/k_tengine.hip
@@ -1,5 +1,6 @@
 #include "qtts_common.h"
 #include "qtts_kernels.h"
+#include "qtts_handoff_dev.h"
 
 namespace {
 
@@ -7,7 +8,7 @@
 constexpr int GPH = NH / KVH;
 constexpr int LPK = 8, CH = 256 / LPK, DPL = HD / LPK, D4 = HD / 4, KG = 256 / D4, NO = GPH * HD;
 constexpr int NVC = CH / KG;
-constexpr unsigned SPIN_MAX = 1u << 22;
+constexpr unsigned SPIN_MAX = QTTS_SPIN_MAX;
 
 struct TLds {
     float xs[H];
@@ -40,9 +41,6 @@
 }
 
 __device__ __forceinline__ int lds_ld(int *p) { return __hip_atomic_load(p, __ATOMIC_RELAXED, __HIP_MEMORY_SCOPE_WORKGROUP); }
-__device__ __forceinline__ void give_up(int *err, int code) {
-    __hip_atomic_store(err, code, __ATOMIC_RELAXED, __HIP_MEMORY_SCOPE_AGENT);
-}
 
 __device__ __forceinline__ bool gemv_wait(TLds &L, int k) {
     unsigned n = 0;
@@ -82,32 +80,11 @@
     if (threadIdx.x == 256) __hip_atomic_store(&L.gflag, k, __ATOMIC_RELAXED, __HIP_MEMORY_SCOPE_WORKGROUP);
 }
 
-typedef unsigned long long u64;
 __device__ __forceinline__ void te_stamp(const TLayerArgs &a, int k, bool who) {
 #ifdef QTTS_STAMPS
     if (a.dbg && who) a.dbg[blockIdx.x * 16 + k] = __builtin_amdgcn_s_memrealtime();
 #endif
 }
-__device__ __forceinline__ void put_granule(u64 *g, unsigned tag, float v) {
-    __hip_atomic_store(g, ((u64)tag << 32) | __float_as_uint(v), __ATOMIC_RELAXED, __HIP_MEMORY_SCOPE_AGENT);
-}
-template <int N, typename Idx>
-__device__ __forceinline__ void sweep(const u64 *g, unsigned tag, Idx idx, float (&v)[N], int *err, int code) {
-    unsigned n = 0;
-    for (;;) {
-        bool ok = true;
-#pragma unroll
-        for (int j = 0; j < N; ++j) {
-            const u64 x = __hip_atomic_load(const_cast<u64 *>(g) + idx(j), __ATOMIC_RELAXED, __HIP_MEMORY_SCOPE_AGENT);
-            v[j] = __uint_as_float((unsigned)x);
-            ok &= (unsigned)(x >> 32) == tag;
-        }
-        if (__all(ok)) return;
-        __builtin_amdgcn_s_sleep(1);
-        if (++n > SPIN_MAX) { give_up(err, code); return; }
-    }
-}
-
 __device__ __forceinline__ void comm_norm_stage(TLds &L, float4 (&xv)[2], const float *nw, float eps, int ct, int lane,
                                                 int cw, int &gen, int *err) {
     float ss = 0.f;
diff --git a/qwen3-tts-c_amd/csrc/hip/qtts_handoff_dev.h b/qwen3-tts-c_amd/csrc/hip/qtts_handoff_dev.h
--- /dev/null
+++ b/qwen3-tts-c_amd/csrc/hip/qtts_handoff_dev.h
@@ -0,0 +1,36 @@
+#pragma once
+#include "qtts_common.h"
+
+typedef unsigned long long u64;
+
+constexpr unsigned QTTS_SPIN_MAX = 1u << 22;
+
+__device__ __forceinline__ void give_up(int *err, int code) {
+    __hip_atomic_store(err, code, __ATOMIC_RELAXED, __HIP_MEMORY_SCOPE_AGENT);
+}
+__device__ __forceinline__ void put_granule(u64 *g, unsigned tag, float v) {
+    __hip_atomic_store(g, ((u64)tag << 32) | __float_as_uint(v), __ATOMIC_RELAXED, __HIP_MEMORY_SCOPE_AGENT);
+}
+template <int N, typename Idx>
+__device__ __forceinline__ bool sweep(const u64 *g, unsigned tag, Idx idx, float (&v)[N], int *err, int code) {
+    unsigned n = 0;
+    bool mine = false;
+    for (;;) {
+        if (!mine) {
+            u64 x[N];
+#pragma unroll
+            for (int j = 0; j < N; ++j)
+                x[j] = __hip_atomic_load(const_cast<u64 *>(g) + idx(j), __ATOMIC_RELAXED, __HIP_MEMORY_SCOPE_AGENT);
+            bool ok = true;
+#pragma unroll
+            for (int j = 0; j < N; ++j) {
+                v[j] = __uint_as_float((unsigned)x[j]);
+                ok &= (unsigned)(x[j] >> 32) == tag;
+            }
+            mine = ok;
+        }
+        if (__all(mine)) return true;
+        __builtin_amdgcn_s_sleep(1);
+        if (++n > QTTS_SPIN_MAX) { give_up(err, code); return false; }
+    }
+}
diff --git a/qwen3-tts-c_amd/csrc/hip/qtts_kernels.h b/qwen3-tts-c_amd/csrc/hip/qtts_kernels.h
--- a/qwen3-tts-c_amd/csrc/hip/qtts_kernels.h
+++ b/qwen3-tts-c_amd/csrc/hip/qtts_kernels.h
@@ -164,6 +164,26 @@
 bool qtts_attn_o_pair_covers(const AttnArgs &a, const bf16_t *Wo);
 int qtts_attn_o_pair(const AttnArgs &a, const bf16_t *Wo, int R, float *part, hipStream_t st);
 
+constexpr int QTTS_SF_C = 1024;
+constexpr int QTTS_SF_MAX_IDX = 128;
+constexpr int QTTS_SF_PF_THREADS = 192;
+struct StFuseArgs {
+    const float *x = nullptr;
+    const float *norm_w = nullptr;
+    float eps = 1e-6f;
+    const bf16_t *Wqkv = nullptr;
+    int C = 0;
+    unsigned long long *g = nullptr;
+    int *ctl = nullptr;
+    int idx = 0;
+    unsigned long long *dbg = nullptr;
+};
+bool qtts_qkv_attn_o_covers(const StFuseArgs &f, const AttnArgs &a, const bf16_t *Wo, int R);
+int qtts_qkv_attn_o(const StFuseArgs &f, const AttnArgs &a, const bf16_t *Wo, int R, float *part, hipStream_t st);
+int qtts_stfuse_row(int NH, int KV, int HD, int b, int m);
+int qtts_qkv_attn_o_blocks_per_cu();
+int qtts_stfuse_epoch_bump(int *ctl, hipStream_t st);
+
 extern thread_local const char *qtts_last_kernel;
 inline bool qtts_attn_head_ok(int HD) { return HD == 8 || HD == 16 || HD == 32 || HD == 64 || HD == 128; }
 int qtts_attention(const AttnArgs &a, hipStream_t st);
@@ -228,6 +248,7 @@
     float *out = nullptr;
     int *kv_len = nullptr;
     int advance = 0;
+    int *epoch = nullptr;
 };
 int qtts_embed_sum(const EmbedSumArgs &a, hipStream_t st);
 
diff --git a/qwen3-tts-c_amd/csrc/hip/qtts_runtime.hip b/qwen3-tts-c_amd/csrc/hip/qtts_runtime.hip
--- a/qwen3-tts-c_amd/csrc/hip/qtts_runtime.hip
+++ b/qwen3-tts-c_amd/csrc/hip/qtts_runtime.hip
@@ -146,6 +146,11 @@
     bool attn_o = true;
     bool tab0b = true;
     bool st_pair = true;
+    bool st_fuse = true;
+    int st_fuse_cap = 0;
+    unsigned long long *st_g = nullptr;
+    int *st_ctl = nullptr;
+    bool gm_dbg_fused = false;
     int l2pf = 31;
     int l2pf_tk = 0;
     unsigned *pf_sink = nullptr;
@@ -449,6 +454,16 @@
     dv->tab0b = !(tb && !atoi(tb));
     const char *sp = getenv("QTTS_HIP_ST_PAIR");
     dv->st_pair = !(sp && !atoi(sp));
+    const char *sf = getenv("QTTS_HIP_ST_FUSE");
+    dv->st_fuse = !(sf && !atoi(sf)) && dims->HDs == 128 && dims->Hs == QTTS_SF_C && dims->NHs == 2 * dims->KVs &&
+                  dims->KVs >= 1 && dims->G * dims->Ls <= QTTS_SF_MAX_IDX;
+    if (dv->st_fuse) {
+        int dev = 0, ncu = 0;
+        if (hipGetDevice(&dev) == hipSuccess &&
+            hipDeviceGetAttribute(&ncu, hipDeviceAttributeMultiprocessorCount, dev) == hipSuccess)
+            dv->st_fuse_cap = qtts_qkv_attn_o_blocks_per_cu() * ncu;
+        if (dv->st_fuse_cap < 2 * (dims->HDs / 4) * dims->KVs) dv->st_fuse = false;
+    }
     const char *pf = getenv("QTTS_HIP_L2PF");
     if (pf) dv->l2pf = atoi(pf);
     const char *pft = getenv("QTTS_HIP_L2PF_TK");
@@ -735,6 +750,14 @@
             CK(hipMemsetAsync(dv->te_ctl, 0, 2 * sizeof(int), dv->st));
         }
         CK(hipMemsetAsync(dv->btick, 0, QTTS_GM_TICKS * sizeof(int), dv->st));
+        A(st_ctl, int, 4);
+        CK(hipMemsetAsync(dv->st_ctl, 0, 4 * sizeof(int), dv->st));
+        dv->st_g = nullptr;
+        if (dv->st_fuse) {
+            const size_t ng = (size_t)d.G * d.Ls * d.KVs * 4 * d.HDs;
+            A(st_g, unsigned long long, ng);
+            CK(hipMemsetAsync(dv->st_g, 0, ng * 8, dv->st));
+        }
         if (dv->gm_dbg_layer >= 0) {
             A(gm_dbg, unsigned long long, 4 * 2048 * 8);
             CK(hipMemsetAsync(dv->gm_dbg, 0, 4 * 2048 * 8 * 8, dv->st));
@@ -784,6 +807,8 @@
     CK(hipMemsetAsync(dv->stopped, 0, B * sizeof(int), st));
     CK(hipMemsetAsync(dv->cur_row, 0, B * sizeof(int), st));
     CK(hipMemsetAsync(dv->stop_step, 0, B * sizeof(int), st));
+    if (dv->st_ctl) CK(hipMemsetAsync(dv->st_ctl + 1, 0, sizeof(int), st));
+    if (dv->te_ctl) CK(hipMemsetAsync(dv->te_ctl + 1, 0, sizeof(int), st));
     std::vector<uint32_t> r(B, seed_bits(dv->par.seed));
     CK(hipMemcpyAsync(dv->rng, r.data(), B * 4, hipMemcpyHostToDevice, st));
     CK(hipMemcpyAsync(dv->st_rng, r.data(), B * 4, hipMemcpyHostToDevice, st));
@@ -995,6 +1020,37 @@
     p.chunks = RPW * cpr; p.lg = __builtin_ctz(cpr); p.ld = NH * HD * 2; p.sink = dv->pf_sink;
     p.nwg = (R / RPW) * (NH / 2);
     return p;
+}
+
+static L2Prefetch pf_stfuse_slices(int NH, int KV, int HD, int C) {
+    L2Prefetch p;
+    const long long rowb = (long long)C * 2;
+    const int cpr = (int)(8 * rowb / 64);
+    if ((cpr & (cpr - 1)) || cpr < 1 || 2 * cpr > 256 * QTTS_PF_LOADS || HD % 16) return p;
+    p.pm = KV; p.pa = 2 * HD * rowb; p.pb = 16 * rowb; p.ld = (int)(8 * rowb);
+    p.chunks = 2 * cpr; p.lg = __builtin_ctz(cpr);
+    p.nwg = (HD / 8) * KV;
+    return p;
+}
+static L2Prefetch pf_stfuse(const qtts_dev *dv, const bf16_t *Wqkv, int NH, int KV, int HD, int C) {
+    L2Prefetch p = pf_stfuse_slices(NH, KV, HD, C);
+    if (p.nwg) { p.base = reinterpret_cast<const unsigned char *>(Wqkv); p.sink = dv->pf_sink; }
+    return p;
+}
+extern "C" int qtts_hip_st_fuse_row(int NH, int KV, int HD, int b, int m) { return qtts_stfuse_row(NH, KV, HD, b, m); }
+extern "C" int qtts_hip_st_fuse_pf_rows(int NH, int KV, int HD, int C, int b, int *rows, int max) {
+    const L2Prefetch p = pf_stfuse_slices(NH, KV, HD, C);
+    if (!p.nwg || b < 0 || b >= p.nwg) return -1;
+    const long long so = (long long)(b % p.pm) * p.pa + (long long)(b / p.pm) * p.pb, ld = p.ld;
+    int n = 0, last = -1;
+    for (int c = 0; c < p.chunks; ++c) {
+        const long long off = so + (long long)(c >> p.lg) * ld + ((long long)(c & ((1 << p.lg) - 1)) << p.cs);
+        const int r = (int)(off / ((long long)C * 2));
+        if (r == last) continue;
+        if (n >= max) return -1;
+        rows[n++] = last = r;
+    }
+    return n;
 }
 
 static bool tengine_ok(qtts_dev *dv, int kzo, int kzd) {
@@ -1226,6 +1282,9 @@
     return 0;
 }
 
+static std::atomic<long long> g_st_fused_launches{0};
+extern "C" long long qtts_hip_st_fused_launches(void) { return g_st_fused_launches.load(); }
+
 static int subtalker(qtts_dev *dv) {
     const qtts_dims_t &d = dv->d;
     const int nb = dv->nrun, NBA = dv->nb, QKV = dv->QKVs(), AD = d.NHs * d.HDs, KVD = d.KVs * d.HDs;
@@ -1253,6 +1312,21 @@
         s.codes = dv->codes; s.codes_bstride = cstride; s.G = d.G; s.g = g; s.out_tok = dv->last_tok;
         return head_sample(dv, a, s, PK_GEMV_SUB);
     };
+    auto fuse_args = [&](int g, int l, const float *x) {
+        StFuseArgs f;
+        f.x = x; f.norm_w = dv->sl[l].in; f.eps = d.eps; f.Wqkv = dv->sl[l].wqkv; f.C = d.Hs;
+        f.idx = g * d.Ls + l;
+        f.g = dv->st_g ? dv->st_g + (size_t)f.idx * d.KVs * 4 * d.HDs : nullptr;
+        f.ctl = dv->st_ctl;
+        return f;
+    };
+    auto fuse_ok = [&](int g, int l, const AttnArgs *ta) {
+        if (!dv->st_fuse || !dv->st_g || nb != 1 || !dv->attn_o || l < 1 || l >= d.Ls) return false;
+        AttnArgs tt;
+        if (ta) tt = *ta;
+        else { tt.mode = 0; tt.NH = d.NHs; tt.KV = d.KVs; tt.HD = d.HDs; tt.S = d.G; tt.nrows = 1; tt.pos_const = g; }
+        return qtts_qkv_attn_o_covers(fuse_args(g, l, dv->x_st), tt, dv->sl[l].wo, d.Hs);
+    };
     int g0 = 0;
     if (st_pair_ok(dv)) {
         float *xfin = nullptr;
@@ -1293,7 +1367,7 @@
             GemvArgs a = gv(ly.wqkv, QKV, d.Hs, xa, d.Hs, dv->qkv_s, QKV, nb, EPI_STORE);
             a.norm_w = ly.in; a.eps = d.eps; a.nt = 0;
             const bool sdbg = dv->gm_dbg && dv->gm_dbg_layer == 99 && g == 5 && l == 2;
-            if (sdbg) { a.dbg = dv->gm_dbg; DBG_XFIRST(a); }
+            if (sdbg) { a.dbg = dv->gm_dbg; DBG_XFIRST(a); dv->gm_dbg_fused = false; }
             if (l == 0 && (!proj || ptab)) { set_src(a); a.xcopy = dv->x_st; a.ldxc = d.Hs; a.xcopy_normed = 0; }
             else if (pend) add_in(a, pend, npend, d.Hs, nb, xb);
             AttnArgs t;
@@ -1322,7 +1396,18 @@
 #ifdef QTTS_STAMPS
             if (sdbg) t.dbg = dv->gm_dbg + 2048 * 8;
 #endif
-            if (dv->attn_o && nb == 1) {
+            if (dv->attn_o && nb == 1 && !tab0 && !pend && !a.xcopy && !a.table && !a.table_f32 && !a.xadd &&
+                fuse_ok(g, l, &t)) {
+                StFuseArgs f = fuse_args(g, l, a.x);
+                if (sdbg) { f.dbg = dv->gm_dbg; dv->gm_dbg_fused = true; }
+                ProfScope ps(dv, PK_GEMV_SUB, ((double)QKV * d.Hs + (double)d.Hs * AD) * 2);
+                if (qtts_qkv_attn_o(f, t, ly.wo, d.Hs, dv->opart, st) != 0) {
+                    fprintf(stderr, "qtts: fused q|k|v + attention + O launch failed (pass %d layer %d)\n", g, l);
+                    return -1;
+                }
+                g_st_fused_launches.fetch_add(1);
+                fused_o = true;
+            } else if (dv->attn_o && nb == 1) {
                 if (!tab0) CKI(pgemv(dv, a, PK_GEMV_SUB));
                 if (pend) { std::swap(xa, xb); pend = nullptr; }
                 ProfScope ps(dv, PK_ATTN, (double)d.Hs * AD * 2);
@@ -1366,7 +1451,9 @@
             a = gv(ly.wdown, d.Hs, d.Is, dv->h_s, d.Is, xa, d.Hs, nb, EPI_RESID);
             a.nt = 0;
             if (pfm & 8) {
-                if (l + 1 < d.Ls) a.pf = pf_gemvw(dv, dv->sl[l + 1].wqkv, QKV, d.Hs);
+                if (l + 1 < d.Ls && fuse_ok(g, l + 1, nullptr))
+                    a.pf = pf_stfuse(dv, dv->sl[l + 1].wqkv, d.NHs, d.KVs, d.HDs, d.Hs);
+                else if (l + 1 < d.Ls) a.pf = pf_gemvw(dv, dv->sl[l + 1].wqkv, QKV, d.Hs);
                 else if (g >= 1) a.pf = pf_gemvw(dv, dv->lm + (size_t)(g - 1) * d.Vs * d.Hs, d.Vs, d.Hs);
             }
             if (sdbg) { a.dbg = dv->gm_dbg + 3 * 2048 * 8; DBG_XFIRST(a); }
@@ -1386,6 +1473,7 @@
     e.cur_row = dv->cur_row; e.stopped = dv->stopped; e.codec_emb = dv->codec_emb; e.st_emb = dv->st_emb;
     e.Vs = d.Vs; e.H = d.H; e.nb = dv->nrun; e.trailing = dv->trailing; e.tr_cap = dv->tr_cap;
     e.n_trailing = dv->n_trailing; e.pad = dv->pad_emb; e.out = dv->x_tk; e.kv_len = dv->kv_len; e.advance = advance;
+    e.epoch = dv->st_ctl;
     ProfScope ps(dv, PK_EMBED, 0);
     return qtts_embed_sum(e, dv->st);
 }
@@ -1794,6 +1882,14 @@
             return -1;
         }
     }
+    if (dv->st_ctl) {
+        int ctl[2] = {0, 0};
+        CK(hipMemcpy(ctl, dv->st_ctl, sizeof(ctl), hipMemcpyDeviceToHost));
+        if (ctl[1]) {
+            fprintf(stderr, "qtts: sub-talker q|k|v hand-off timed out (code %d, epoch %d)\n", ctl[1], ctl[0]);
+            return -1;
+        }
+    }
     if (dv->gm_dbg && dv->te_g) {
         std::vector<unsigned long long> h(2 * 256 * 16);
         CK(hipMemcpy(h.data(), dv->gm_dbg, h.size() * 8, hipMemcpyDeviceToHost));
@@ -1822,7 +1918,8 @@
         std::vector<unsigned long long> h(4 * 2048 * 8);
         CK(hipMemcpy(h.data(), dv->gm_dbg, h.size() * 8, hipMemcpyDeviceToHost));
         static const char *op[4] = {"q|k|v", "O / -", "gate|up", "down"};
-        static const char *ph[7] = {"start", "x staged", "dot done", "epilogue", "pf landed", "w issued", "merged"};
+        static const char *ph[8] = {"start", "x staged", "dot done", "epilogue", "pf landed", "w issued", "merged", "-"};
+        static const char *phf[8] = {"start", "x staged", "qkv dot", "published", "gathered", "attn done", "O dot", "end"};
         unsigned long long tq = 0;
         for (int g = 0; g < 4; ++g) {
             const unsigned long long *b = h.data() + (size_t)g * 2048 * 8;
@@ -1834,13 +1931,14 @@
                 fprintf(stderr, "[gm_dbg] %-8s launch at %7.2f us after the first, last stamp %6.2f us into it\n", op[g],
                         (t0 - tq) * 0.01, (tend - t0) * 0.01);
             }
-            for (int k = 0; k < 7; ++k) {
+            const bool fz = g == 0 && dv->gm_dbg_fused;
+            for (int k = 0; k < (fz ? 8 : 7); ++k) {
                 std::vector<double> v;
                 for (int i = 0; i < 2048; ++i) if (b[i * 8 + k]) v.push_back((b[i * 8 + k] - t0) * 0.01);
                 if (v.empty()) continue;
                 std::sort(v.begin(), v.end());
-                fprintf(stderr, "[gm_dbg] %-8s %-10s n %4zu  min %6.2f  med %6.2f  max %6.2f us\n", op[g], ph[k], v.size(),
-                        v[0], v[v.size() / 2], v.back());
+                fprintf(stderr, "[gm_dbg] %-8s %-10s n %4zu  min %6.2f  med %6.2f  max %6.2f us\n", fz ? "fused" : op[g],
+                        fz ? phf[k] : ph[k], v.size(), v[0], v[v.size() / 2], v.back());
             }
         }
         hipMemsetAsync(dv->gm_dbg, 0, h.size() * 8, dv->st);
@@ -2415,6 +2513,7 @@
     int rc = subtalker(dv);
     dv->nrun = dv->nb;
     CKI(rc);
+    if (dv->st_ctl) CKI(qtts_stfuse_epoch_bump(dv->st_ctl, dv->st));
     CK(hipMemcpyAsync(out_codes, dv->codes, (size_t)d.G * 4, hipMemcpyDeviceToHost, dv->st));
     CK(hipStreamSynchronize(dv->st));
     return 0;
@@ -2725,6 +2824,40 @@
     return rc;
 }
 
+extern "C" int qtts_hip_qkv_attn_o(float *part, const float *x, const float *in_w, const uint16_t *Wqkv, float *kc,
+                                   float *vc, const float *qn_w, const float *kn_w, const float *rope_cos,
+                                   const float *rope_sin, const int *skip, const uint16_t *Wo,
+                                   unsigned long long *g, int *ctl, int idx, int pos, int R, int C, int NH, int KV,
+                                   int HD, int S, float eps, int bump, int sync, void *stream) {
+    if (!part || !x || !in_w || !Wqkv || !kc || !vc || !qn_w || !kn_w || !rope_cos || !rope_sin || !Wo || !g || !ctl)
+        return -1;
+    if (!attn_dims_ok(NH, KV, HD, S, 1, 0) || R < 1 || pos < 0 || pos >= S) return -1;
+    AttnArgs t;
+    t.mode = 0; t.ld_qkv = (NH + 2 * KV) * HD; t.qn_w = qn_w; t.kn_w = kn_w; t.eps = eps;
+    t.rope_cos = rope_cos; t.rope_sin = rope_sin; t.kc = kc; t.vc = vc; t.S = S;
+    t.pos = nullptr; t.pos_const = pos; t.NH = NH; t.KV = KV; t.HD = HD; t.ld_out = NH * HD; t.nrows = 1; t.skip = skip;
+    StFuseArgs f;
+    f.x = x; f.norm_w = in_w; f.eps = eps; f.Wqkv = Wqkv; f.C = C; f.idx = idx; f.ctl = ctl;
+    f.g = g + (size_t)(idx < 0 ? 0 : idx) * KV * 4 * HD;
+    if (!qtts_qkv_attn_o_covers(f, t, Wo, R)) return 1;
+    hipStream_t st = (hipStream_t)stream;
+    int rc = qtts_qkv_attn_o(f, t, Wo, R, part, st);
+    if (!rc && bump) rc = qtts_stfuse_epoch_bump(ctl, st);
+    if (!rc) g_st_fused_launches.fetch_add(1);
+    if (sync && hipStreamSynchronize(st) != hipSuccess) rc = -1;
+    return rc;
+}
+
+extern "C" int qtts_dev_debug_set_handoff_err(qtts_dev_t *dv, int which, int code) {
+    if (!dv) return -1;
+    hipSetDevice(dv->device);
+    int *w = which == 0 ? dv->st_ctl : which == 1 ? dv->te_ctl : nullptr;
+    if (!w) return -1;
+    CK(hipStreamSynchronize(dv->st));
+    CK(hipMemcpy(w + 1, &code, sizeof(int), hipMemcpyHostToDevice));
+    return 0;
+}
+
 extern "C" int qtts_hip_resident_matvec_rows_bf16(float *out, const uint16_t *A, const float *x, const float *w,
                                                   float eps, int rows, int cols, int epi, const float *part,
                                                   int n_part, float *x_new, int nrows, void *stream) {
diff --git a/qwen3-tts-c_amd/qtts.py b/qwen3-tts-c_amd/qtts.py
--- a/qwen3-tts-c_amd/qtts.py
+++ b/qwen3-tts-c_amd/qtts.py
@@ -107,6 +107,8 @@
     "qwen_tts_codec_mstream_push_ragged", "qtts_dev_codec_mstream_push_host_ragged",
     "qtts_dev_codec_mstream_push_slots_ragged", "qtts_dev_codec_mstream_prime",
     "qwen_tts_generate_voice_clone_batch_stream", "qwen_tts_generate_voice_clone_audio_batch_stream",
+    "qtts_hip_qkv_attn_o", "qtts_hip_st_fuse_row", "qtts_hip_st_fuse_pf_rows", "qtts_hip_st_fused_launches",
+    "qtts_dev_debug_set_handoff_err",
 ]
 
 MAX_BATCH = 64
@@ -374,6 +376,16 @@
     L.qtts_hip_attn_cached.argtypes = [vp, vp, C.c_int] + [vp] * 8 + [C.c_int] * 6 + [C.c_float] + [C.c_int] * 3 + [vp]
     L.qtts_hip_attn_o.restype = C.c_int
     L.qtts_hip_attn_o.argtypes = [vp] * 10 + [C.c_int] * 6 + [C.c_float, vp]
+    if hasattr(L, "qtts_hip_st_fused_launches"):
+        L.qtts_hip_st_fused_launches.restype = C.c_longlong
+        L.qtts_hip_qkv_attn_o.restype = C.c_int
+        L.qtts_hip_qkv_attn_o.argtypes = [vp] * 14 + [C.c_int] * 8 + [C.c_float, C.c_int, C.c_int, vp]
+        L.qtts_hip_st_fuse_row.restype = C.c_int
+        L.qtts_hip_st_fuse_row.argtypes = [C.c_int] * 5
+        L.qtts_hip_st_fuse_pf_rows.restype = C.c_int
+        L.qtts_hip_st_fuse_pf_rows.argtypes = [C.c_int] * 5 + [C.POINTER(C.c_int), C.c_int]
+        L.qtts_dev_debug_set_handoff_err.restype = C.c_int
+        L.qtts_dev_debug_set_handoff_err.argtypes = [C.c_void_p, C.c_int, C.c_int]
     if hasattr(L, "qtts_hip_st_pair_passes"):
         L.qtts_hip_st_pair_passes.restype = C.c_longlong
         L.qtts_hip_attn_o_pair.restype = C.c_int
@@ -1043,6 +1055,18 @@
         return True
 
     @staticmethod
+    def qkv_attn_o(part, x, in_w, Wqkv_u16, kc, vc, qn_w, kn_w, rope_cos, rope_sin, Wo_u16, g_i64, ctl_i32, idx, pos,
+                   R, cols, NH, KV, HD, S, eps, skip_i32=None, bump=True, sync=True):
+        rc = lib().qtts_hip_qkv_attn_o(_ptr(part), _ptr(x), _ptr(in_w), _ptr(Wqkv_u16), _ptr(kc), _ptr(vc), _ptr(qn_w),
+                                       _ptr(kn_w), _ptr(rope_cos), _ptr(rope_sin), _ptr(skip_i32), _ptr(Wo_u16),
+                                       _ptr(g_i64), _ptr(ctl_i32), int(idx), int(pos), R, cols, NH, KV, HD, S, eps,
+                                       int(bool(bump)), int(bool(sync)), _stream())
+        if rc == 1:
+            return False
+        _ok(rc, "qkv_attn_o")
+        return True
+
+    @staticmethod
     def attn_o_pair(part, qkv, kc, vc, qn_w, kn_w, rope_cos, rope_sin, Wo_u16, R, NH, KV, HD, S, eps, skip_i32=None):
         rc = lib().qtts_hip_attn_o_pair(_ptr(part), _ptr(qkv), _ptr(kc), _ptr(vc), _ptr(qn_w), _ptr(kn_w),
                                         _ptr(rope_cos), _ptr(rope_sin), _ptr(skip_i32), _ptr(Wo_u16), R, NH, KV, HD,
```
